# neka-nat/probreg

Measured on AMD Instinct MI355X. Metric: EM iterations/sec (RigidCPD, N=M=100k fp32), higher is better.
Workload: dtype f32; 1 GPU; C1 RigidCPD fp32 synthetic N=M=100000 D=3 w=0; window=EM iterations 0..2332 of the registration (state reset after the warm-up steps), collective=none, m=100000, n_local=100000, n_global=100000

## Files before the change

include/probreg_hip.h:

```cpp
#ifndef PROBREG_HIP_H
#define PROBREG_HIP_H

#include <stdint.h>

#ifdef __cplusplus
extern "C" {
#endif

typedef enum prg_status {
    PRG_OK = 0,
    PRG_ERR_INVALID = -1,
    PRG_ERR_HIP = -2,
    PRG_ERR_STATE = -3,
    PRG_ERR_NOMEM = -4
} prg_status;

typedef enum prg_tf_kind {
    PRG_TF_RIGID = 0,
    PRG_TF_AFFINE = 1,
    PRG_TF_NONRIGID = 2
} prg_tf_kind;

const char* prg_last_error(void);
int prg_version(void);
int prg_device_count(int* count);

#define PRG_NMOMENTS 32
#define PRG_NPARAMS 32

typedef struct prg_cpd prg_cpd;

int prg_cpd_create(prg_cpd** out, int device, void* hip_stream);
int prg_cpd_destroy(prg_cpd* h);

int prg_spatial_order(const float* points_hd, int64_t n, int dim, int on_device, int* perm_host);
int prg_cpd_set_options(prg_cpd* h, int sort_source, int sort_target, int cull);

int prg_cpd_set_dense_engine(prg_cpd* h, int mode, double bound);
int prg_cpd_last_estep_engine(prg_cpd* h, int* engine);
int prg_cpd_engine_bounds(int64_t m, int64_t n_local, double* col_bound, double* row_bound);
int prg_cpd_set_sparse_engine(prg_cpd* h, int mode);
int prg_cpd_last_estep_engines(prg_cpd* h, int* col_engine, int* row_engine);
int prg_cpd_last_estep_lean(prg_cpd* h, int* lean);
int prg_cpd_set_lean_factor(prg_cpd* h, double factor);
int prg_cpd_set_stream_mode(prg_cpd* h, int on);

int prg_cpd_set_source(prg_cpd* h, const float* source_hd, int64_t m, int dim);

int prg_cpd_set_target(prg_cpd* h, const float* target_hd, int64_t n_local, int dim, int64_t n_global);

int prg_cpd_bind_moments(prg_cpd* h, double* moments_dev);
int prg_cpd_moments_ptr(prg_cpd* h, double** moments_dev);
int prg_cpd_params_ptr(prg_cpd* h, double** params_dev);

#define PRG_COMM_ID_BYTES 128
typedef struct prg_comm prg_comm;
int prg_comm_available(int* rccl_version);
int prg_comm_unique_id(unsigned char* id_out);
int prg_comm_create(prg_comm** out, const unsigned char* id, int rank, int nranks, int device);
int prg_comm_adopt(prg_comm** out, void* nccl_comm, int device);
int prg_comm_info(prg_comm* c, int* rank, int* nranks, int64_t* all_reduces_issued);
int prg_comm_destroy(prg_comm* c);
int prg_comm_all_reduce_f64(prg_comm* c, double* buf_dev, int64_t count, void* hip_stream);
int prg_cpd_set_comm(prg_cpd* h, prg_comm* comm);
int prg_cpd_iterate(prg_cpd* h, int kind, int update_scale, double w, int n_iter);
int prg_cpd_set_moments_only(prg_cpd* h, int mode);
int prg_cpd_last_estep_fused(prg_cpd* h, int* fused);
int prg_cpd_set_fused_factor(prg_cpd* h, double factor);
int prg_cpd_set_resid_sweep(prg_cpd* h, int on);

int prg_cpd_init_sums(prg_cpd* h);
int prg_cpd_init_params(prg_cpd* h, const double* init_params_host);

int prg_cpd_estep(prg_cpd* h, double w);

int prg_cpd_estep_timed(prg_cpd* h, double w, float* ms_out);

int prg_cpd_pair_counts(prg_cpd* h, double* col_pairs, double* row_pairs);

int prg_cpd_mstep(prg_cpd* h, int kind, int update_scale);

int prg_cpd_get_params(prg_cpd* h, double* params_host);
int prg_cpd_set_params(prg_cpd* h, const double* params_host);
int prg_cpd_get_moments(prg_cpd* h, double* moments_host);

int prg_cpd_get_estep(prg_cpd* h, double* pt1_hd, double* p1_hd, double* px_hd);
int prg_cpd_get_tsource(prg_cpd* h, float* tsource_hd);

int prg_cpd_moments_from_estep(prg_cpd* h, const double* pt1_hd, const double* p1_hd, const double* px_hd);

int prg_cpd_set_tuning(prg_cpd* h, int r_col, int seg_col, int r_row, int seg_row);

int prg_cpd_nonrigid_build_g(prg_cpd* h, double beta);
int prg_cpd_nonrigid_set_solver(prg_cpd* h, int mode, int max_rank, double tol);
int prg_cpd_nonrigid_rank(prg_cpd* h, int* rank);
int prg_cpd_nonrigid_get_g(prg_cpd* h, float* g_hd);
int prg_cpd_nonrigid_set_w(prg_cpd* h, const double* w_hd);
int prg_cpd_nonrigid_get_w(prg_cpd* h, double* w_hd);
int prg_cpd_nonrigid_apply(prg_cpd* h, double* t_hd);
int prg_cpd_nonrigid_set_priors(prg_cpd* h, const double* p1_tilde_hd, const double* px_tilde_hd, double alpha);
int prg_cpd_rowacc_ptr(prg_cpd* h, double** rowacc_dev, int64_t* count);
int prg_cpd_mstep_nonrigid(prg_cpd* h, double lmd);

int prg_cpd_set_source_weights(prg_cpd* h, const double* log_weights_hd, double uniform_ratio);
int prg_cpd_bcpd_build_g(prg_cpd* h, double c);
int prg_cpd_bcpd_solve(prg_cpd* h, double lmd, double cfac, const double* nu_hd, const double* resid_hd,
                       double* vhat_hd, double* sigma_diag_hd);

int prg_gauss_transform_direct(int device, void* hip_stream, const double* source_hd, int64_t s,
                               const double* target_hd, int64_t t, int dim, const double* weights_hd,
                               int n_weight_rows, double h, double* out_hd);
int prg_gauss_transform_direct_f64(int device, void* hip_stream, const double* source_hd, int64_t s,
                               const double* target_hd, int64_t t, int dim, const double* weights_hd,
                               int n_weight_rows, double h, double* out_hd);

int prg_squared_kernel_sum(int device, void* hip_stream, const float* x_hd, int64_t m,
                           const float* y_hd, int64_t n, int dim, double* out_host);
int prg_rbf_kernel(int device, void* hip_stream, const float* x_hd, int64_t m, const float* y_hd,
                   int64_t n, int dim, double beta, float* out_hd);
int prg_inverse_multiquadric_kernel(int device, void* hip_stream, const float* x_hd, int64_t m, const float* y_hd,
                                    int64_t n, int dim, double c, float* out_hd);
int prg_nn_mean_distance(int device, void* hip_stream, const float* a_hd, int64_t m, const float* b_hd, int64_t n,
                         int dim, double* out_host);

typedef struct prg_ph prg_ph;
int prg_lattice_set_splat_mode(int mode);
int prg_ph_create(prg_ph** out, int device, void* hip_stream);
int prg_ph_destroy(prg_ph* h);
int prg_ph_init(prg_ph* h, const float* points_hd, int64_t n, int dim, int with_blur);
int prg_ph_lattice_size(prg_ph* h, int* size);
int prg_ph_filter(prg_ph* h, const float* values_hd, int channels, float* out_hd);

typedef struct prg_filterreg prg_filterreg;
int prg_fr_create(prg_filterreg** out, int device, void* hip_stream);
int prg_fr_destroy(prg_filterreg* h);
int prg_fr_set_source(prg_filterreg* h, const double* source_hd, int64_t m, int dim);
int prg_fr_set_target(prg_filterreg* h, const double* target_hd, int64_t n, int dim);
int prg_fr_set_state(prg_filterreg* h, const double* rot9, const double* t3, double sigma2);
int prg_fr_estep(prg_filterreg* h, double alpha, int* lattice_size, int* with_blur);
int prg_fr_get_estep(prg_filterreg* h, float* m0_hd, float* m1_hd, float* m2_hd);
int prg_fr_mstep(prg_filterreg* h, double w, int update_sigma2, double min_sigma2, double* out_host);
int prg_fr_get_state(prg_filterreg* h, double* out_host);

int prg_fr_set_target_normals(prg_filterreg* h, const double* normals_hd);
int prg_fr_get_nx(prg_filterreg* h, float* nx_hd);
int prg_fr_mstep_pt2pl(prg_filterreg* h, double w, int update_sigma2, double min_sigma2, double* out_host);

int prg_fr_mstep_from_arrays(int device, void* hip_stream, const double* t_source_hd, int64_t m, int dim,
                             int64_t n_target, const float* m0_hd, const float* m1_hd, const float* m2_hd,
                             const float* nx_hd, const double* rot9, const double* t3, double sigma2, double w,
                             double* out_host);

int prg_kabsch_weighted(int device, void* hip_stream, const float* model_hd, const float* target_hd,
                        const float* weight_hd, int64_t n, int dim, double* rot_host, double* t_host);

typedef struct prg_gmmtree prg_gmmtree;
int prg_gmm_create(prg_gmmtree** out, int device, void* hip_stream);
int prg_gmm_destroy(prg_gmmtree* h);
int prg_gmm_build(prg_gmmtree* h, const double* points_hd, int64_t n, int tree_level, const int64_t* init_idx_host,
                  double lambda_s, double lambda_d, int max_iter, int* iters_host, double* q_host, double* dq_host);
int prg_gmm_set_nodes(prg_gmmtree* h, const double* nodes_host, int tree_level);
int prg_gmm_get_nodes(prg_gmmtree* h, double* nodes_host);
int prg_gmm_set_target(prg_gmmtree* h, const double* target_hd, int64_t n);
int prg_gmm_reg_estep(prg_gmmtree* h, const double* rot9, const double* t3, double scale, double lambda_c,
                      double* m01_host, double* m2_host);

typedef struct prg_gmmfit prg_gmmfit;
int prg_gmmfit_create(prg_gmmfit** out, int device, void* hip_stream);
int prg_gmmfit_destroy(prg_gmmfit* h);
int prg_gmmfit_set_data(prg_gmmfit* h, const double* data_hd, int64_t n, int dim);
int prg_gmmfit_seed(prg_gmmfit* h, int k, const double* uniforms_host, int n_trials);
int prg_gmmfit_get_seeds(prg_gmmfit* h, int* index_host);
int prg_gmmfit_lloyd(prg_gmmfit* h, int max_iter, double tol, int* n_iter_host);
int prg_gmmfit_init_from_labels(prg_gmmfit* h, double reg_covar);
int prg_gmmfit_set_params(prg_gmmfit* h, int k, const double* weights_host, const double* means_host,
                          const double* precisions_host);
int prg_gmmfit_em(prg_gmmfit* h, double tol, int max_iter, double reg_covar, int* n_iter_host, int* converged_host,
                  double* lower_bounds_host);
int prg_gmmfit_get_params(prg_gmmfit* h, double* weights_host, double* means_host, double* covariances_host);

#ifdef __cplusplus
}
#endif
#endif
```

probreg_amd/_lib.py:

```python
import ctypes
import os

_HERE = os.path.dirname(os.path.abspath(__file__))
LIB_PATH = os.environ.get("PROBREG_HIP_LIB") or os.path.join(_HERE, "csrc", "libprobreg_hip.so")

PRG_OK = 0
PRG_ERR_INVALID = -1
PRG_ERR_HIP = -2
PRG_ERR_STATE = -3
PRG_ERR_NOMEM = -4

PRG_TF_RIGID = 0
PRG_TF_AFFINE = 1
PRG_TF_NONRIGID = 2

PRG_NMOMENTS = 32
PRG_NPARAMS = 32
PRG_COMM_ID_BYTES = 128


class ProbregHipError(RuntimeError):
    """A libprobreg_hip call failed (HIP runtime error or call-order violation)."""


def _load():
    try:
        import torch
    except Exception:
        pass
    if not os.path.isfile(LIB_PATH):
        raise ImportError(
            "probreg_amd: %s not found. Build it with `python __graft_entry__.py build` "
            "(or `make -C probreg_amd/csrc`); there is no CPU fallback." % LIB_PATH
        )
    try:
        return ctypes.CDLL(LIB_PATH)
    except OSError as e:
        raise ImportError("probreg_amd: cannot load %s: %s" % (LIB_PATH, e))


lib = _load()

_c = ctypes
_vp, _i, _i64, _d = _c.c_void_p, _c.c_int, _c.c_int64, _c.c_double
_pp = _c.POINTER(_c.c_void_p)

SIGNATURES = {
    "prg_version": [],
    "prg_device_count": [_c.POINTER(_i)],
    "prg_cpd_create": [_pp, _i, _vp],
    "prg_cpd_destroy": [_vp],
    "prg_spatial_order": [_vp, _i64, _i, _i, _vp],
    "prg_cpd_set_options": [_vp, _i, _i, _i],
    "prg_cpd_set_dense_engine": [_vp, _i, _d],
    "prg_cpd_last_estep_engine": [_vp, _c.POINTER(_i)],
    "prg_cpd_set_sparse_engine": [_vp, _i],
    "prg_cpd_engine_bounds": [_i64, _i64, _c.POINTER(_d), _c.POINTER(_d)],
    "prg_cpd_last_estep_lean": [_vp, _c.POINTER(_i)],
    "prg_cpd_set_lean_factor": [_vp, _d],
    "prg_cpd_set_stream_mode": [_vp, _i],
    "prg_cpd_last_estep_engines": [_vp, _c.POINTER(_i), _c.POINTER(_i)],
    "prg_cpd_set_source": [_vp, _vp, _i64, _i],
    "prg_cpd_set_target": [_vp, _vp, _i64, _i, _i64],
    "prg_cpd_bind_moments": [_vp, _vp],
    "prg_cpd_moments_ptr": [_vp, _pp],
    "prg_cpd_params_ptr": [_vp, _pp],
    "prg_comm_available": [_c.POINTER(_i)],
    "prg_comm_unique_id": [_vp],
    "prg_comm_create": [_pp, _vp, _i, _i, _i],
    "prg_comm_adopt": [_pp, _vp, _i],
    "prg_comm_info": [_vp, _c.POINTER(_i), _c.POINTER(_i), _c.POINTER(_i64)],
    "prg_comm_destroy": [_vp],
    "prg_comm_all_reduce_f64": [_vp, _vp, _i64, _vp],
    "prg_cpd_set_comm": [_vp, _vp],
    "prg_cpd_iterate": [_vp, _i, _i, _d, _i],
    "prg_cpd_set_moments_only": [_vp, _i],
    "prg_cpd_last_estep_fused": [_vp, _c.POINTER(_i)],
    "prg_cpd_set_fused_factor": [_vp, _d],
    "prg_cpd_set_resid_sweep": [_vp, _i],
    "prg_cpd_init_sums": [_vp],
    "prg_cpd_init_params": [_vp, _vp],
    "prg_cpd_estep": [_vp, _d],
    "prg_cpd_estep_timed": [_vp, _d, _vp],
    "prg_cpd_pair_counts": [_vp, _c.POINTER(_d), _c.POINTER(_d)],
    "prg_cpd_mstep": [_vp, _i, _i],
    "prg_cpd_get_params": [_vp, _vp],
    "prg_cpd_set_params": [_vp, _vp],
    "prg_cpd_get_moments": [_vp, _vp],
    "prg_cpd_get_estep": [_vp, _vp, _vp, _vp],
    "prg_cpd_get_tsource": [_vp, _vp],
    "prg_cpd_moments_from_estep": [_vp, _vp, _vp, _vp],
    "prg_cpd_set_tuning": [_vp, _i, _i, _i, _i],
    "prg_cpd_nonrigid_build_g": [_vp, _d],
    "prg_cpd_nonrigid_set_solver": [_vp, _i, _i, _d],
    "prg_cpd_nonrigid_rank": [_vp, _c.POINTER(_i)],
    "prg_cpd_nonrigid_get_g": [_vp, _vp],
    "prg_cpd_nonrigid_set_w": [_vp, _vp],
    "prg_cpd_nonrigid_get_w": [_vp, _vp],
    "prg_cpd_nonrigid_apply": [_vp, _vp],
    "prg_cpd_nonrigid_set_priors": [_vp, _vp, _vp, _d],
    "prg_cpd_rowacc_ptr": [_vp, _pp, _c.POINTER(_i64)],
    "prg_cpd_mstep_nonrigid": [_vp, _d],
    "prg_cpd_set_source_weights": [_vp, _vp, _d],
    "prg_cpd_bcpd_build_g": [_vp, _d],
    "prg_cpd_bcpd_solve": [_vp, _d, _d, _vp, _vp, _vp, _vp],
    "prg_gauss_transform_direct": [_i, _vp, _vp, _i64, _vp, _i64, _i, _vp, _i, _d, _vp],
    "prg_gauss_transform_direct_f64": [_i, _vp, _vp, _i64, _vp, _i64, _i, _vp, _i, _d, _vp],
    "prg_squared_kernel_sum": [_i, _vp, _vp, _i64, _vp, _i64, _i, _c.POINTER(_d)],
    "prg_rbf_kernel": [_i, _vp, _vp, _i64, _vp, _i64, _i, _d, _vp],
    "prg_inverse_multiquadric_kernel": [_i, _vp, _vp, _i64, _vp, _i64, _i, _d, _vp],
    "prg_nn_mean_distance": [_i, _vp, _vp, _i64, _vp, _i64, _i, _c.POINTER(_d)],
    "prg_lattice_set_splat_mode": [_i],
    "prg_ph_create": [_pp, _i, _vp],
    "prg_ph_destroy": [_vp],
    "prg_ph_init": [_vp, _vp, _i64, _i, _i],
    "prg_ph_lattice_size": [_vp, _c.POINTER(_i)],
    "prg_ph_filter": [_vp, _vp, _i, _vp],
    "prg_fr_create": [_pp, _i, _vp],
    "prg_fr_destroy": [_vp],
    "prg_fr_set_source": [_vp, _vp, _i64, _i],
    "prg_fr_set_target": [_vp, _vp, _i64, _i],
    "prg_fr_set_state": [_vp, _vp, _vp, _d],
    "prg_fr_estep": [_vp, _d, _c.POINTER(_i), _c.POINTER(_i)],
    "prg_fr_get_estep": [_vp, _vp, _vp, _vp],
    "prg_fr_mstep": [_vp, _d, _i, _d, _vp],
    "prg_fr_get_state": [_vp, _vp],
    "prg_fr_set_target_normals": [_vp, _vp],
    "prg_fr_get_nx": [_vp, _vp],
    "prg_fr_mstep_pt2pl": [_vp, _d, _i, _d, _vp],
    "prg_fr_mstep_from_arrays": [_i, _vp, _vp, _i64, _i, _i64, _vp, _vp, _vp, _vp, _vp, _vp, _d, _d, _vp],
    "prg_kabsch_weighted": [_i, _vp, _vp, _vp, _vp, _i64, _i, _vp, _vp],
    "prg_gmm_create": [_pp, _i, _vp],
    "prg_gmm_destroy": [_vp],
    "prg_gmm_build": [_vp, _vp, _i64, _i, _vp, _d, _d, _i, _vp, _vp, _vp],
    "prg_gmm_set_nodes": [_vp, _vp, _i],
    "prg_gmm_get_nodes": [_vp, _vp],
    "prg_gmm_set_target": [_vp, _vp, _i64],
    "prg_gmm_reg_estep": [_vp, _vp, _vp, _d, _d, _vp, _vp],
    "prg_gmmfit_create": [_pp, _i, _vp],
    "prg_gmmfit_destroy": [_vp],
    "prg_gmmfit_set_data": [_vp, _vp, _i64, _i],
    "prg_gmmfit_seed": [_vp, _i, _vp, _i],
    "prg_gmmfit_get_seeds": [_vp, _vp],
    "prg_gmmfit_lloyd": [_vp, _i, _d, _c.POINTER(_i)],
    "prg_gmmfit_init_from_labels": [_vp, _d],
    "prg_gmmfit_set_params": [_vp, _i, _vp, _vp, _vp],
    "prg_gmmfit_em": [_vp, _d, _i, _d, _c.POINTER(_i), _c.POINTER(_i), _vp],
    "prg_gmmfit_get_params": [_vp, _vp, _vp, _vp],
}

for _name, _args in SIGNATURES.items():
    _fn = getattr(lib, _name)
    _fn.argtypes = _args
    _fn.restype = _i
lib.prg_last_error.argtypes = []
lib.prg_last_error.restype = _c.c_char_p


def last_error():
    msg = lib.prg_last_error()
    return msg.decode("utf-8", "replace") if msg else ""


def check(status):
    if status == PRG_OK:
        return
    msg = last_error()
    if status == PRG_ERR_INVALID:
        raise ValueError(msg)
    if status == PRG_ERR_NOMEM:
        raise MemoryError(msg)
    raise ProbregHipError("libprobreg_hip status %d: %s" % (status, msg))


def device_count():
    n = _i(0)
    st = lib.prg_device_count(_c.byref(n))
    if st != PRG_OK:
        return 0
    return int(n.value)


def require_gpu():
    n = device_count()
    if n <= 0:
        raise ProbregHipError(
            "probreg_amd needs an AMD GPU (gfx950): hipGetDeviceCount reported none (%s). "
            "There is no CPU fallback." % last_error()
        )
    return n


def ptr(a):
    if a is None:
        return None
    if hasattr(a, "data_ptr"):
        return _vp(a.data_ptr())
    return _vp(a.ctypes.data)
```

probreg_amd/csrc/cpd.hip:

```cpp
#include <math.h>

#include <algorithm>
#include <cmath>
#include <cstdlib>
#include <cstring>
#include <vector>

#include "cpd_estep.h"
#include "cpd_sweeps.h"
#include "morton.h"
#include "small_linalg.h"

namespace {
using prg::block_reduce_store;
using prg::ensure_mompart;
using prg::grid1;
using prg::kBlock;
using prg::kMomComp;
using prg::row_moment_terms;

constexpr double kEps32 = 1.1920928955078125e-07;

__global__ __launch_bounds__(kBlock) void k_pack_cloud(const float* __restrict__ in, int64_t n, int dim,
                                                       float4* __restrict__ out, int64_t cap, float pad,
// ... 98 lines not shown
                                                                const double* __restrict__ px, int dim, int64_t m,
                                                                int64_t n, const float4* __restrict__ src4,
                                                                const float4* __restrict__ tgt4,
                                                                const int* __restrict__ perm_src,
                                                                const int* __restrict__ perm_tgt,
                                                                double* __restrict__ mompart) {
    const int64_t i = (int64_t)blockIdx.x * kBlock + threadIdx.x;
    double a[kMomComp];
#pragma unroll
    for (int c = 0; c < kMomComp; ++c) a[c] = 0.0;
    if (i < m) {
        const float4 yf = src4[i];
        const double y[3] = {yf.x, yf.y, yf.z};
        const int64_t j = perm_src ? perm_src[i] : i;
        double pxi[3] = {px[j * dim], px[j * dim + 1], dim > 2 ? px[j * dim + 2] : 0.0};
        row_moment_terms(a, p1[j], pxi, y);
    }
    if (i < n) {
        const float4 xf = tgt4[i];
        const int64_t j = perm_tgt ? perm_tgt[i] : i;
        a[22] = pt1[j] * ((double)xf.x * xf.x + (double)xf.y * xf.y + (double)xf.z * xf.z);
    }
    block_reduce_store(a, mompart);
}

__global__ __launch_bounds__(kBlock) void k_rowacc_from_arrays(const double* __restrict__ pt1,
                                                               const double* __restrict__ p1,
                                                               const double* __restrict__ px, int dim, int64_t m,
                                                               int64_t n, int64_t mcap,
                                                               const int* __restrict__ perm_src,
                                                               const int* __restrict__ perm_tgt,
                                                               double* __restrict__ rowacc, float* __restrict__ pt1f) {
    const int64_t i = (int64_t)blockIdx.x * kBlock + threadIdx.x;
    if (i < n) pt1f[i] = (float)pt1[perm_tgt ? perm_tgt[i] : i];
    if (i >= m) return;
    const int64_t j = perm_src ? perm_src[i] : i;
    rowacc[i] = p1[j];
    rowacc[mcap + i] = px[j * dim];
    rowacc[2 * mcap + i] = px[j * dim + 1];
    rowacc[3 * mcap + i] = dim > 2 ? px[j * dim + 2] : 0.0;
}

__global__ void k_mstep(const double* __restrict__ mom, double* __restrict__ params, int kind, int update_scale,
                        int dim) {
    if (threadIdx.x != 0 || blockIdx.x != 0) return;
    const int d = dim;
    const double S0 = mom[0];
    double mu_x[3], mu_y[3], A[3][3], YPY[3][3];
#pragma unroll
    for (int i = 0; i < 3; ++i) {
        mu_x[i] = mom[1 + i] / S0;
        mu_y[i] = mom[4 + i] / S0;
    }
#pragma unroll
    for (int i = 0; i < 3; ++i)
#pragma unroll
        for (int j = 0; j < 3; ++j) A[i][j] = mom[7 + 3 * i + j] - mom[1 + i] * mu_y[j];
    const double syy[3][3] = {{mom[16], mom[17], mom[18]}, {mom[17], mom[19], mom[20]}, {mom[18], mom[20], mom[21]}};
    double tr_yp1y = 0.0, mux2 = 0.0;
#pragma unroll
    for (int i = 0; i < 3; ++i) {
#pragma unroll
        for (int j = 0; j < 3; ++j) YPY[i][j] = syy[i][j] - S0 * mu_y[i] * mu_y[j];
        tr_yp1y += YPY[i][i];
        mux2 += mu_x[i] * mu_x[i];
    }
    const double tr_xp1x = mom[22] - S0 * mux2;
    double L[3][3], t[3];
    double scale = 1.0, sigma2, q;
    if (kind == PRG_TF_RIGID) {
        double U[3][3], V[3][3], sv[3];
        prg::jacobi_svd(A, d, U, V, sv);
        const double dd = prg::det3(U, d) * prg::det3(V, d);
        double c[3];
#pragma unroll
        for (int k = 0; k < 3; ++k) {
            bool is_min = k < d;
#pragma unroll
            for (int j = 0; j < 3; ++j)
                if (j < d && j != k && (sv[j] < sv[k] || (sv[j] == sv[k] && j < k))) is_min = false;
            c[k] = is_min ? dd : 1.0;
        }
        double tr_atr = 0.0;
#pragma unroll
        for (int i = 0; i < 3; ++i)
#pragma unroll
            for (int j = 0; j < 3; ++j) {
                double r = 0;
#pragma unroll
                for (int k = 0; k < 3; ++k) r += c[k] * U[i][k] * V[j][k];
                L[i][j] = r;
                tr_atr += (i < d && j < d) ? A[i][j] * r : 0.0;
            }
        scale = update_scale ? tr_atr / tr_yp1y : 1.0;
#pragma unroll
        for (int i = 0; i < 3; ++i) {
            double r = 0;
#pragma unroll
            for (int j = 0; j < 3; ++j) r += L[i][j] * mu_y[j];
            t[i] = (i < d) ? mu_x[i] - scale * r : 0.0;
        }
        if (update_scale)
            sigma2 = (tr_xp1x - scale * tr_atr) / (S0 * d);
        else
            sigma2 = (tr_xp1x + tr_yp1y - scale * tr_atr) / (S0 * d);
        sigma2 = fmax(sigma2, kEps32);
        q = (tr_xp1x - 2.0 * scale * tr_atr + scale * scale * tr_yp1y) / (2.0 * sigma2);
        q += d * S0 * 0.5 * log(sigma2);
    } else {
        double Mx[3][6];
#pragma unroll
        for (int i = 0; i < 3; ++i)
#pragma unroll
            for (int j = 0; j < 3; ++j) {
                const bool in = i < d && j < d;
                Mx[i][j] = in ? YPY[j][i] : ((i == j) ? 1.0 : 0.0);
                Mx[i][3 + j] = in ? A[j][i] : 0.0;
            }
        double ypy_scale = 0.0;
#pragma unroll
        for (int i = 0; i < 3; ++i)
#pragma unroll
            for (int j = 0; j < 3; ++j) ypy_scale = fmax(ypy_scale, (i < d && j < d) ? fabs(YPY[i][j]) : 0.0);
#pragma unroll
        for (int c = 0; c < 3; ++c) {
#pragma unroll
            for (int r = c + 1; r < 3; ++r) {
                if (fabs(Mx[r][c]) > fabs(Mx[c][c])) {
#pragma unroll
                    for (int j = 0; j < 6; ++j) { const double tmp = Mx[c][j]; Mx[c][j] = Mx[r][j]; Mx[r][j] = tmp; }
                }
            }
            if (c < d && !(fabs(Mx[c][c]) > 1e-12 * ypy_scale)) Mx[c][c] = 0.0;
#pragma unroll
            for (int r = c + 1; r < 3; ++r) {
                const double f = Mx[r][c] / Mx[c][c];
#pragma unroll
                for (int j = 0; j < 6; ++j) Mx[r][j] -= (j >= c) ? f * Mx[c][j] : 0.0;
            }
        }
        double Xs[3][3];
#pragma unroll
        for (int col = 0; col < 3; ++col)
#pragma unroll
            for (int r = 2; r >= 0; --r) {
                double v = Mx[r][3 + col];
#pragma unroll
                for (int j = 0; j < 3; ++j) v -= (j > r) ? Mx[r][j] * Xs[j][col] : 0.0;
                Xs[r][col] = v / Mx[r][r];
            }
        double tr_ab = 0.0;
#pragma unroll
        for (int i = 0; i < 3; ++i) {
            double r = 0;
#pragma unroll
            for (int j = 0; j < 3; ++j) {
                const bool in = i < d && j < d;
                L[i][j] = in ? Xs[j][i] : ((i == j) ? 1.0 : 0.0);
                r += in ? L[i][j] * mu_y[j] : 0.0;
                tr_ab += in ? A[i][j] * L[i][j] : 0.0;
            }
            t[i] = (i < d) ? mu_x[i] - r : 0.0;
        }
        sigma2 = (tr_xp1x - tr_ab) / (S0 * d);
        sigma2 = fmax(sigma2, kEps32);
        q = (tr_xp1x - 2.0 * tr_ab + tr_ab) / (2.0 * sigma2) + d * S0 * 0.5 * log(sigma2);
    }
    for (int i = 0; i < 3; ++i) {
        for (int j = 0; j < 3; ++j) params[3 * i + j] = L[i][j];
        params[9 + i] = t[i];
    }
    params[12] = scale;
    params[13] = sigma2;
    params[14] = q;
    params[15] = S0;
    params[16] += 1.0;
}

__global__ __launch_bounds__(kBlock) void k_float_to_double(const float* __restrict__ in, double* __restrict__ out,
                                                            int64_t n, const int* __restrict__ perm) {
    int64_t i = (int64_t)blockIdx.x * kBlock + threadIdx.x;
    if (i < n) out[perm ? perm[i] : i] = in[i];
}
__global__ __launch_bounds__(kBlock) void k_scatter_double(const double* __restrict__ in, double* __restrict__ out,
                                                           int64_t n, const int* __restrict__ perm) {
    int64_t i = (int64_t)blockIdx.x * kBlock + threadIdx.x;
    if (i < n) out[perm ? perm[i] : i] = in[i];
}
__global__ __launch_bounds__(kBlock) void k_gather_weights(const double* __restrict__ lw, int64_t m,
                                                           const int* __restrict__ perm, float* __restrict__ out) {
    int64_t i = (int64_t)blockIdx.x * kBlock + threadIdx.x;
    if (i < m) out[i] = (float)lw[perm ? perm[i] : i];
}
__global__ __launch_bounds__(kBlock) void k_pack_px(const double* __restrict__ rowacc, int64_t mcap, int64_t m,
                                                    int dim, double* __restrict__ out, const int* __restrict__ perm) {
    int64_t i = (int64_t)blockIdx.x * kBlock + threadIdx.x;
    if (i >= m) return;
    const int64_t j = perm ? perm[i] : i;
    for (int k = 0; k < dim; ++k) out[j * dim + k] = rowacc[(int64_t)(1 + k) * mcap + i];
}
__global__ __launch_bounds__(kBlock) void k_unpack_points(const float4* __restrict__ in, int64_t m, int dim,
                                                          float* __restrict__ out, const int* __restrict__ perm) {
    int64_t i = (int64_t)blockIdx.x * kBlock + threadIdx.x;
    if (i >= m) return;
    const float4 v = in[i];
    const int64_t j = perm ? perm[i] : i;
    out[j * dim] = v.x;
    out[j * dim + 1] = v.y;
    if (dim > 2) out[j * dim + 2] = v.z;
}

static void free_queue(SweepQueue& q) {
    for (void* p : {(void*)q.masks, (void*)q.chunk, (void*)q.units, (void*)q.ctrl, (void*)q.ucount})
        if (p) (void)hipFree(p);
    q = SweepQueue();
}

int free_plan_buffers(prg_cpd* h) {
    free_queue(h->qcol);
    free_queue(h->qrow);
    void** const owned[] = {(void**)&h->src4, (void**)&h->z4, (void**)&h->tgt4, (void**)&h->pt1, (void**)&h->colpart, (void**)&h->rowpart,
                            (void**)&h->rowacc, (void**)&h->mompart, &h->stage, (void**)&h->perm_src, (void**)&h->perm_tgt, (void**)&h->zmeta,
                            (void**)&h->tmeta, (void**)&h->colmin, (void**)&h->motion, (void**)&h->srcw, (void**)&h->wgcount, (void**)&h->rorig,
                            (void**)&h->corig, (void**)&h->zchunk, (void**)&h->tchunk};
    for (void** p : owned) {
        if (*p) (void)hipFree(*p);
        *p = nullptr;
    }
    h->wg_cap = 0;
    h->stage_bytes = 0;
    return PRG_OK;
}

int cap_for(int64_t n) { return (int)prg::round_up(n + 64 * prg::kSuper + 1024, 1024); }

int morton_permutation(prg_cpd* h, const float* pts_hd, int64_t n, int dim, int** perm_dev, double* ext2 = nullptr,
                       float* box = nullptr) {
    std::vector<float> host((size_t)n * dim);
    PRG_HIP(hipMemcpy(host.data(), pts_hd, host.size() * sizeof(float), hipMemcpyDefault));
    if (ext2) {
        *ext2 = 0.0;
        for (int k = 0; k < 3; ++k) {
            float lo = INFINITY, hi = -INFINITY;
            for (int64_t i = 0; i < n && k < dim; ++i) {
                lo = std::min(lo, host[(size_t)i * dim + k]);
                hi = std::max(hi, host[(size_t)i * dim + k]);
            }
            if (k >= dim) lo = hi = 0.f;
            *ext2 += (double)(hi - lo) * (double)(hi - lo);
            if (box) {
                box[k] = lo;
                box[3 + k] = hi;
            }
        }
    }
    if (*perm_dev) (void)hipFree(*perm_dev);
    *perm_dev = nullptr;
    PRG_HIP(hipMalloc((void**)perm_dev, (size_t)n * sizeof(int)));
    const std::string& order = prg::cpd_env().spatial_order;
    if (order != "morton" && order != "kd_host") {
        PRG_TRY(prg::ensure_stage(h, (size_t)n * dim * sizeof(float)));
        PRG_HIP(hipMemcpyAsync(h->stage, host.data(), host.size() * sizeof(float), hipMemcpyHostToDevice, h->stream));
        return prg::device_kd_order((const float*)h->stage, n, dim, *perm_dev, h->stream);
    }
    const std::vector<int> perm = order == "morton" ? prg::morton_order(host.data(), n, dim) : prg::kd_order(host.data(), n, dim);
    PRG_HIP(hipMemcpy(*perm_dev, perm.data(), (size_t)n * sizeof(int), hipMemcpyHostToDevice));
    return PRG_OK;
}

template <typename T>
int ensure_exact(T** p, size_t count) {
    if (*p) (void)hipFree(*p);
    *p = nullptr;
    PRG_HIP(hipMalloc((void**)p, count * sizeof(T)));
    return PRG_OK;
}

}

namespace prg {
int ensure_stage(prg_cpd* h, size_t bytes) {
    if (h->stage && h->stage_bytes >= bytes) return PRG_OK;
    if (h->stage) {
        PRG_HIP(hipStreamSynchronize(h->stream));
        (void)hipFree(h->stage);
    }
    h->stage = nullptr;
    h->stage_bytes = 0;
    PRG_HIP(hipMalloc(&h->stage, bytes));
    h->stage_bytes = bytes;
    return PRG_OK;
}

const CpdEnv& cpd_env() {
    static const CpdEnv env = [] {
        CpdEnv e;
        auto num = [](const char* name, double absent) { const char* v = getenv(name); return v ? atof(v) : absent; };
        auto is_zero = [](const char* name) { const char* v = getenv(name); return v && atoi(v) == 0; };
        e.mfma_seg = getenv("PRG_MFMA_SEG") ? atoi(getenv("PRG_MFMA_SEG")) : 0;
        e.fine_grid_off = is_zero("PRG_MFMA_FINE_GRID");
        e.r_col = num("PRG_ENGINE_RCOL", 0.0);
        e.r_row = num("PRG_ENGINE_RROW", 0.0);
        e.fused_rcol_scale = num("PRG_FUSED_RCOL_SCALE", -1.0);
        e.lean_factor = num("PRG_LEAN_FACTOR", -1.0);
        e.fused_factor = num("PRG_FUSED_FACTOR", -1.0);
        e.owner_off = is_zero("PRG_OWNER_SWEEP");
        e.debug_engine = getenv("PRG_DEBUG_ENGINE") != nullptr;
        if (const char* v = getenv("PRG_SPATIAL_ORDER")) e.spatial_order = v;
        return e;
    }();
    return env;
}

int ensure_engine_state(prg_cpd* h) {
    if (h->eng_host) return PRG_OK;
    PRG_HIP(hipHostMalloc((void**)&h->eng_host, sizeof(EngineDecision), hipHostMallocMapped | hipHostMallocCoherent));
    memset(h->eng_host, 0, sizeof(EngineDecision));
    PRG_HIP(hipHostGetDevicePointer((void**)&h->eng_host_dev, h->eng_host, 0));
    const size_t bytes = sizeof(EngineDecision) + 2 * sizeof(unsigned long long) + 4 * sizeof(double);
    PRG_HIP(hipMalloc((void**)&h->eng_dev, bytes));
    PRG_HIP(hipMemsetAsync(h->eng_dev, 0, bytes, h->stream));
    h->eng_work = reinterpret_cast<unsigned long long*>(h->eng_dev + 1);
    h->tsum_local = reinterpret_cast<double*>(h->eng_work + 2);
    return PRG_OK;
}
}

extern "C" {

int prg_cpd_create(prg_cpd** out, int device, void* hip_stream) {
    PRG_REQUIRE(out != nullptr, PRG_ERR_INVALID, "prg_cpd_create: out is NULL");
    int count = 0;
    PRG_HIP(hipGetDeviceCount(&count));
    PRG_REQUIRE(device >= 0 && device < count, PRG_ERR_INVALID, "prg_cpd_create: device %d out of range (%d devices)",
                device, count);
    prg::DeviceGuard g(device);
    PRG_REQUIRE(g.ok, PRG_ERR_HIP, "prg_cpd_create: hipSetDevice(%d) failed", device);
    prg_cpd* h = new (std::nothrow) prg_cpd();
    PRG_REQUIRE(h != nullptr, PRG_ERR_NOMEM, "prg_cpd_create: out of host memory");
    h->device = device;
    h->stream = (hipStream_t)hip_stream;
    if (const char* eng = getenv("PRG_DENSE_ENGINE")) h->dense_engine = std::max(0, std::min(2, atoi(eng)));
    if (const char* eng = getenv("PRG_SPARSE_ENGINE")) h->sparse_engine = std::max(0, std::min(2, atoi(eng)));
    if (const char* eng = getenv("PRG_RESID_SWEEP")) h->resid_sweep = atoi(eng) != 0;
    hipError_t e = hipMalloc((void**)&h->state, (PRG_NMOMENTS + PRG_NPARAMS) * sizeof(double));
    if (e != hipSuccess) {
        delete h;
        prg::set_error("prg_cpd_create: hipMalloc failed: %s", hipGetErrorString(e));
        return PRG_ERR_HIP;
    }
    h->moments = h->state;
    h->params = h->state + PRG_NMOMENTS;
    k_zero_doubles<<<1, 64, 0, h->stream>>>(h->state, PRG_NMOMENTS + PRG_NPARAMS);
    *out = h;
    return PRG_OK;
}

int prg_cpd_destroy(prg_cpd* h) {
    if (!h) return PRG_OK;
    prg::DeviceGuard g(h->device);
    (void)hipStreamSynchronize(h->stream);
    free_plan_buffers(h);
    prg::nonrigid_free(h);
    if (h->state) (void)hipFree(h->state);
    if (h->pinned) (void)hipHostFree(h->pinned);
    if (h->eng_host) (void)hipHostFree(h->eng_host);
    if (h->eng_dev) (void)hipFree(h->eng_dev);
    delete h;
    return PRG_OK;
}

int prg_cpd_set_source(prg_cpd* h, const float* source_hd, int64_t m, int dim) {
    PRG_REQUIRE(h && source_hd, PRG_ERR_INVALID, "prg_cpd_set_source: NULL argument");
    PRG_REQUIRE(m > 0 && (dim == 2 || dim == 3), PRG_ERR_INVALID,
                "prg_cpd_set_source: need m > 0 and dim in {2,3} (got m=%lld dim=%d)", (long long)m, dim);
    PRG_REQUIRE(!h->have_target || h->D == dim, PRG_ERR_INVALID,
                "prg_cpd_set_source: dim %d does not match target dim %d", dim, h->D);
    prg::DeviceGuard g(h->device);
    PRG_HIP(hipStreamSynchronize(h->stream));
    const int64_t cap = cap_for(m);
    if (cap != h->Mcap) {
        if (h->src4) (void)hipFree(h->src4);
        if (h->z4) (void)hipFree(h->z4);
        if (h->rowacc) (void)hipFree(h->rowacc);
        h->src4 = h->z4 = nullptr;
        h->rowacc = nullptr;
        PRG_HIP(hipMalloc((void**)&h->src4, cap * sizeof(float4)));
        PRG_HIP(hipMalloc((void**)&h->z4, cap * sizeof(float4)));
        PRG_HIP(hipMalloc((void**)&h->rowacc, 4 * cap * sizeof(double)));
    }
    if (cap != h->Mcap || !h->zmeta) {
        PRG_TRY(ensure_exact(&h->zmeta, (size_t)(cap / prg::kGroup) * 8));
        if (!h->motion) {
            PRG_TRY(ensure_exact(&h->motion, 16));
            PRG_HIP(hipMemsetAsync(h->motion, 0, 16 * sizeof(unsigned), h->stream));
        }
        PRG_TRY(ensure_exact(&h->rorig, (size_t)(cap / prg::kMfmaWgPoints) + 4));
        PRG_TRY(ensure_exact(&h->zchunk, (size_t)(cap / prg::kSuper) * 8));
    }
    h->M = m;
    h->D = dim;
    h->Mcap = cap;
    if (h->opt_sort_src) {
        PRG_TRY(morton_permutation(h, source_hd, m, dim, &h->perm_src, &h->sext2));
    } else if (h->perm_src) {
        (void)hipFree(h->perm_src);
        h->perm_src = nullptr;
    }
    PRG_TRY(prg::ensure_stage(h, (size_t)m * dim * sizeof(float)));
    PRG_HIP(hipMemcpyAsync(h->stage, source_hd, (size_t)m * dim * sizeof(float), hipMemcpyDefault, h->stream));
    k_pack_cloud<<<grid1(cap), kBlock, 0, h->stream>>>((const float*)h->stage, m, dim, h->src4, cap, prg::kSrcPad,
                                                       0.f, h->perm_src);
    k_pack_cloud<<<grid1(cap), kBlock, 0, h->stream>>>((const float*)h->stage, m, dim, h->z4, cap, prg::kSrcPad, 0.f,
                                                       h->perm_src);
    k_group_meta<<<grid1(cap / prg::kGroup), kBlock, 0, h->stream>>>(h->z4, cap / prg::kGroup, h->zmeta);
    PRG_HIP(hipGetLastError());
    PRG_HIP(hipStreamSynchronize(h->stream));
    h->have_colmin = false;
    h->have_source = true;
    h->have_estep = false;
    prg::nonrigid_free(h);
    if (h->srcw) (void)hipFree(h->srcw);
    h->srcw = nullptr;
    h->uniform_ratio = 0.0;
    return PRG_OK;
}

int prg_cpd_set_source_weights(prg_cpd* h, const double* log_weights_hd, double uniform_ratio) {
    PRG_REQUIRE(h && h->have_source, PRG_ERR_STATE, "prg_cpd_set_source_weights: source not set");
    PRG_REQUIRE(uniform_ratio >= 0.0, PRG_ERR_INVALID, "prg_cpd_set_source_weights: uniform_ratio must be >= 0");
    prg::DeviceGuard g(h->device);
    h->uniform_ratio = uniform_ratio;
    if (!log_weights_hd) {
        PRG_HIP(hipStreamSynchronize(h->stream));
        if (h->srcw) (void)hipFree(h->srcw);
        h->srcw = nullptr;
        return PRG_OK;
    }
    hipPointerAttribute_t attr;
    const bool on_host = hipPointerGetAttributes(&attr, log_weights_hd) != hipSuccess || attr.type != hipMemoryTypeDevice;
    (void)hipGetLastError();
    if (on_host)
        for (int64_t i = 0; i < h->M; ++i)
            PRG_REQUIRE(log_weights_hd[i] <= 0.0, PRG_ERR_INVALID,
                        "prg_cpd_set_source_weights: log-weight %lld is %g, must be <= 0 (and not NaN)", (long long)i,
                        log_weights_hd[i]);
    if (!h->srcw) PRG_HIP(hipMalloc((void**)&h->srcw, (size_t)h->Mcap * sizeof(float)));
    PRG_TRY(prg::ensure_stage(h, (size_t)h->M * sizeof(double)));
    PRG_HIP(hipMemcpyAsync(h->stage, log_weights_hd, (size_t)h->M * sizeof(double), hipMemcpyDefault, h->stream));
    k_gather_weights<<<grid1(h->M), kBlock, 0, h->stream>>>((const double*)h->stage, h->M, h->perm_src, h->srcw);
    PRG_HIP(hipGetLastError());
    PRG_HIP(hipStreamSynchronize(h->stream));
    h->have_colmin = false;
    return PRG_OK;
}

int prg_cpd_set_target(prg_cpd* h, const float* target_hd, int64_t n_local, int dim, int64_t n_global) {
    PRG_REQUIRE(h && target_hd, PRG_ERR_INVALID, "prg_cpd_set_target: NULL argument");
    PRG_REQUIRE(n_local > 0 && n_global >= n_local && (dim == 2 || dim == 3), PRG_ERR_INVALID,
                "prg_cpd_set_target: need 0 < n_local <= n_global and dim in {2,3}");
    PRG_REQUIRE(!h->have_source || h->D == dim, PRG_ERR_INVALID,
                "prg_cpd_set_target: dim %d does not match source dim %d", dim, h->D);
    prg::DeviceGuard g(h->device);
    PRG_HIP(hipStreamSynchronize(h->stream));
    if (h->tsum_local) PRG_HIP(hipMemsetAsync(h->tsum_local, 0, 4 * sizeof(double), h->stream));
    const int64_t cap = cap_for(n_local);
    if (cap != h->Ncap) {
        if (h->tgt4) (void)hipFree(h->tgt4);
        if (h->pt1) (void)hipFree(h->pt1);
        h->tgt4 = nullptr;
        h->pt1 = nullptr;
        PRG_HIP(hipMalloc((void**)&h->tgt4, cap * sizeof(float4)));
        PRG_HIP(hipMalloc((void**)&h->pt1, cap * sizeof(float)));
    }
    if (cap != h->Ncap || !h->tmeta) {
        PRG_TRY(ensure_exact(&h->tmeta, (size_t)(cap / prg::kGroup) * 8));
        PRG_TRY(ensure_exact(&h->tchunk, (size_t)(cap / prg::kSuper) * 8));
        PRG_TRY(ensure_exact(&h->corig, (size_t)(cap / prg::kMfmaWgPoints) + 4));
        PRG_TRY(ensure_exact(&h->colmin, (size_t)cap + (size_t)cap / prg::kGroup));
        PRG_HIP(hipMemsetAsync(h->colmin, 0, ((size_t)cap + (size_t)cap / prg::kGroup) * sizeof(float), h->stream));
    }
    if (!h->motion) {
        PRG_TRY(ensure_exact(&h->motion, 16));
        PRG_HIP(hipMemsetAsync(h->motion, 0, 16 * sizeof(unsigned), h->stream));
    }
    h->N = n_local;
    h->Nglobal = n_global;
    h->D = dim;
    h->Ncap = cap;
    if (h->opt_sort_tgt) {
        PRG_TRY(morton_permutation(h, target_hd, n_local, dim, &h->perm_tgt, &h->text2, h->tbox));
    } else if (h->perm_tgt) {
        (void)hipFree(h->perm_tgt);
        h->perm_tgt = nullptr;
    }
    PRG_TRY(prg::ensure_stage(h, (size_t)n_local * dim * sizeof(float)));
    PRG_HIP(hipMemcpyAsync(h->stage, target_hd, (size_t)n_local * dim * sizeof(float), hipMemcpyDefault, h->stream));
    k_pack_cloud<<<grid1(cap), kBlock, 0, h->stream>>>((const float*)h->stage, n_local, dim, h->tgt4, cap,
                                                       prg::kTgtPad, 0.f, h->perm_tgt);
    k_group_meta<<<grid1(cap / prg::kGroup), kBlock, 0, h->stream>>>(h->tgt4, cap / prg::kGroup, h->tmeta);
    PRG_HIP(hipGetLastError());
    PRG_HIP(hipStreamSynchronize(h->stream));
    h->have_colmin = false;
    h->have_target = true;
    h->have_estep = false;
    return PRG_OK;
}

int prg_cpd_bind_moments(prg_cpd* h, double* moments_dev) {
    PRG_REQUIRE(h, PRG_ERR_INVALID, "prg_cpd_bind_moments: NULL handle");
    h->moments = moments_dev ? moments_dev : h->state;
    return PRG_OK;
}

int prg_cpd_moments_ptr(prg_cpd* h, double** moments_dev) {
    PRG_REQUIRE(h && moments_dev, PRG_ERR_INVALID, "prg_cpd_moments_ptr: NULL argument");
    *moments_dev = h->moments;
    return PRG_OK;
}

int prg_cpd_params_ptr(prg_cpd* h, double** params_dev) {
    PRG_REQUIRE(h && params_dev, PRG_ERR_INVALID, "prg_cpd_params_ptr: NULL argument");
    *params_dev = h->params;
    return PRG_OK;
}

int prg_cpd_set_tuning(prg_cpd* h, int r_col, int seg_col, int r_row, int seg_row) {
    PRG_REQUIRE(h, PRG_ERR_INVALID, "prg_cpd_set_tuning: NULL handle");
    auto ok_r = [](int r) { return r == 0 || r == 2 || r == 4 || r == -2 || r == -4; };
    PRG_REQUIRE(ok_r(r_col) && ok_r(r_row), PRG_ERR_INVALID,
                "prg_cpd_set_tuning: points per lane must be 0 (auto), 2, 4 (packed) or -2, -4 (scalar form)");
    PRG_REQUIRE(seg_col >= 0 && seg_col <= 1024 && seg_row >= 0 && seg_row <= 256, PRG_ERR_INVALID,
                "prg_cpd_set_tuning: segment counts must be in [0, 1024] (column pass) / [0, 256] (row pass)");
    h->r_col = r_col;
    h->seg_col = seg_col;
    h->r_row = r_row;
    h->seg_row = seg_row;
    return PRG_OK;
}

int prg_cpd_set_dense_engine(prg_cpd* h, int mode, double bound) {
    PRG_REQUIRE(h, PRG_ERR_INVALID, "prg_cpd_set_dense_engine: NULL handle");
    PRG_REQUIRE(mode >= 0 && mode <= 2, PRG_ERR_INVALID, "prg_cpd_set_dense_engine: mode must be 0, 1 or 2");
    PRG_REQUIRE(bound >= 0.0, PRG_ERR_INVALID, "prg_cpd_set_dense_engine: bound must be >= 0 (0 keeps the default)");
    h->dense_engine = mode;
    if (bound > 0.0) h->dense_bound = bound;
    EngineSwitch fresh;
    fresh.pred_fused = h->eng.pred_fused;
    fresh.grid_fine = h->eng.grid_fine;
    h->eng = fresh;
    return PRG_OK;
}

int prg_cpd_last_estep_engine(prg_cpd* h, int* engine) {
    PRG_REQUIRE(h && engine, PRG_ERR_INVALID, "prg_cpd_last_estep_engine: NULL argument");
    *engine = h->last_estep_mfma ? 1 : 0;
    return PRG_OK;
}

int prg_cpd_set_sparse_engine(prg_cpd* h, int mode) {
    PRG_REQUIRE(h, PRG_ERR_INVALID, "prg_cpd_set_sparse_engine: NULL handle");
    PRG_REQUIRE(mode >= 0 && mode <= 3, PRG_ERR_INVALID, "prg_cpd_set_sparse_engine: mode must be 0 (grid of culled waves), 1 (default: owner sweep for single-sweep "
                "iterations, work queue for the two-sweep E-steps of large clouds), 2 (work queue always) or 3 (round 5's default: queue for large clouds, no owner sweep)");
    h->sparse_engine = mode;
    return PRG_OK;
}

int prg_cpd_last_estep_engines(prg_cpd* h, int* col_engine, int* row_engine) {
    PRG_REQUIRE(h && col_engine && row_engine, PRG_ERR_INVALID, "prg_cpd_last_estep_engines: NULL argument");
    *col_engine = h->last_estep_mfma ? 1 : 0;
    *row_engine = h->last_estep_row_mfma ? 1 : 0;
    return PRG_OK;
}

int prg_cpd_last_estep_lean(prg_cpd* h, int* lean) {
    PRG_REQUIRE(h && lean, PRG_ERR_INVALID, "prg_cpd_last_estep_lean: NULL argument");
    *lean = h->last_estep_row_lean ? 1 : 0;
    return PRG_OK;
}

int prg_cpd_set_moments_only(prg_cpd* h, int mode) {
    PRG_REQUIRE(h, PRG_ERR_INVALID, "prg_cpd_set_moments_only: NULL handle");
    PRG_REQUIRE(mode >= 0 && mode <= 2, PRG_ERR_INVALID, "prg_cpd_set_moments_only: mode must be 0, 1 or 2");
    h->moments_only = mode == 1;
    h->fused_in_iterate = mode != 2;
    return PRG_OK;
}

int prg_cpd_set_resid_sweep(prg_cpd* h, int on) {
    PRG_REQUIRE(h, PRG_ERR_INVALID, "prg_cpd_set_resid_sweep: NULL handle");
    h->resid_sweep = on != 0;
    return PRG_OK;
}

int prg_cpd_set_fused_factor(prg_cpd* h, double factor) {
    PRG_REQUIRE(h && factor >= 0.0, PRG_ERR_INVALID, "prg_cpd_set_fused_factor: need a handle and a factor >= 0");
    h->fused_factor = factor;
    return PRG_OK;
}

int prg_cpd_last_estep_fused(prg_cpd* h, int* fused) {
    PRG_REQUIRE(h && fused, PRG_ERR_INVALID, "prg_cpd_last_estep_fused: NULL argument");
    *fused = h->last_estep_fused ? 1 : 0;
    return PRG_OK;
}

int prg_cpd_set_stream_mode(prg_cpd* h, int on) {
    PRG_REQUIRE(h, PRG_ERR_INVALID, "prg_cpd_set_stream_mode: NULL handle");
    h->mfma_stream = on != 0;
    return PRG_OK;
}

int prg_cpd_set_lean_factor(prg_cpd* h, double factor) {
    PRG_REQUIRE(h, PRG_ERR_INVALID, "prg_cpd_set_lean_factor: NULL handle");
    h->lean_factor = factor;
    return PRG_OK;
}

int prg_cpd_set_options(prg_cpd* h, int sort_source, int sort_target, int cull) {
    PRG_REQUIRE(h, PRG_ERR_INVALID, "prg_cpd_set_options: NULL handle");
    PRG_REQUIRE(!h->have_source && !h->have_target, PRG_ERR_STATE,
                "prg_cpd_set_options: must be called before the clouds are uploaded");
    h->opt_sort_src = sort_source != 0;
    h->opt_sort_tgt = sort_target != 0;
    h->opt_cull = cull != 0;
    return PRG_OK;
}

int prg_cpd_init_sums(prg_cpd* h) {
    PRG_REQUIRE(h && h->have_target, PRG_ERR_STATE, "prg_cpd_init_sums: target not set");
    prg::DeviceGuard g(h->device);
    PRG_TRY(ensure_mompart(h));
    const int nblk = (int)prg::ceil_div(h->N, kBlock);
    k_zero_doubles<<<1, 64, 0, h->stream>>>(h->moments, PRG_NMOMENTS);
    k_cloud_sums<<<nblk, kBlock, 0, h->stream>>>(h->tgt4, h->N, h->mompart);
    prg::reduce_partials(h, h->mompart, nblk, 4, h->moments, 24);
    PRG_HIP(hipGetLastError());
    PRG_TRY(prg::ensure_engine_state(h));
    PRG_HIP(hipMemcpyAsync(h->tsum_local, h->moments + 24, 4 * sizeof(double), hipMemcpyDeviceToDevice, h->stream));
    if (h->comm) PRG_TRY(prg::comm_all_reduce_f64(h->comm, h->moments, PRG_NMOMENTS, h->stream));
    return PRG_OK;
}

int prg_cpd_set_comm(prg_cpd* h, prg_comm* comm) {
    PRG_REQUIRE(h, PRG_ERR_INVALID, "prg_cpd_set_comm: NULL handle");
    PRG_REQUIRE(!comm || comm->device == h->device, PRG_ERR_INVALID, "prg_cpd_set_comm: the communicator lives on device %d, the plan on %d",
                comm ? comm->device : -1, h->device);
    h->comm = comm;
    return PRG_OK;
}

static bool is_rotation(const double* lin) {
    for (int i = 0; i < 3; ++i)
        for (int j = 0; j < 3; ++j) {
            double d = 0.0;
            for (int k = 0; k < 3; ++k) d += lin[3 * k + i] * lin[3 * k + j];
            if (!(fabs(d - (i == j ? 1.0 : 0.0)) <= 1.0e-12)) return false;
        }
    return true;
}

int prg_cpd_init_params(prg_cpd* h, const double* init_params_host) {
    PRG_REQUIRE(h && h->have_source && h->have_target, PRG_ERR_STATE, "prg_cpd_init_params: clouds not set");
    prg::DeviceGuard g(h->device);
    PRG_TRY(ensure_mompart(h));
    const int nblk = (int)prg::ceil_div(h->M, kBlock);
    double* srcsum = h->mompart + (h->mompart_elems - 64);
    double* init_dev = nullptr;
    if (init_params_host) {
        init_dev = srcsum + 8;
        PRG_HIP(hipMemcpyAsync(init_dev, init_params_host, 16 * sizeof(double), hipMemcpyHostToDevice, h->stream));
    }
    k_cloud_sums<<<nblk, kBlock, 0, h->stream>>>(h->src4, h->M, h->mompart);
    prg::reduce_partials(h, h->mompart, nblk, 4, srcsum, 0);
    k_init_params<<<1, 64, 0, h->stream>>>(h->moments, srcsum, h->params, (double)h->M, (double)h->Nglobal, h->D,
                                           init_dev);
    PRG_HIP(hipGetLastError());
    if (init_params_host) PRG_HIP(hipStreamSynchronize(h->stream));
    h->have_colmin = false;
    h->eng = EngineSwitch();
    h->init_rot_orthonormal = !init_params_host || is_rotation(init_params_host);
    return PRG_OK;
}


int prg_cpd_engine_bounds(int64_t m, int64_t n_local, double* col_bound, double* row_bound) {
    PRG_REQUIRE(m > 0 && n_local > 0 && col_bound && row_bound, PRG_ERR_INVALID, "prg_cpd_engine_bounds: need m, n_local > 0 and two outputs");
    *col_bound = prg::engine_col_bound(m, n_local);
    *row_bound = prg::engine_row_bound(m, n_local);
    return PRG_OK;
}

int prg_cpd_estep(prg_cpd* h, double w) { return prg::estep_impl(h, w, nullptr); }

int prg_cpd_estep_timed(prg_cpd* h, double w, float* ms_out) {
    PRG_REQUIRE(h && ms_out, PRG_ERR_INVALID, "prg_cpd_estep_timed: NULL argument");
    prg::DeviceGuard g(h->device);
    hipEvent_t ev[6];
    for (int i = 0; i < 6; ++i) PRG_HIP(hipEventCreate(&ev[i]));
    int st = prg::estep_impl(h, w, ev);
    if (st == PRG_OK) {
        hipError_t e = hipEventSynchronize(ev[5]);
        if (e != hipSuccess) {
            prg::set_error("prg_cpd_estep_timed: hipEventSynchronize failed: %s", hipGetErrorString(e));
            st = PRG_ERR_HIP;
        }
    }
    if (st == PRG_OK) {
        for (int i = 0; i < 5; ++i) (void)hipEventElapsedTime(&ms_out[i], ev[i], ev[i + 1]);
        (void)hipEventElapsedTime(&ms_out[5], ev[0], ev[5]);
    }
    for (int i = 0; i < 6; ++i) (void)hipEventDestroy(ev[i]);
    return st;
}

int prg_cpd_pair_counts(prg_cpd* h, double* col_pairs, double* row_pairs) {
    PRG_REQUIRE(h && h->have_estep && col_pairs && row_pairs, PRG_ERR_STATE, "prg_cpd_pair_counts: no E-step has been run");
    prg::DeviceGuard g(h->device);
    *col_pairs = h->dense_pairs_col;
    *row_pairs = h->dense_pairs_row;
    for (int pass = 0; pass < 2; ++pass) {
        const SweepQueue& q = pass ? h->qrow : h->qcol;
        if ((pass ? h->wg_row : h->wg_col) != -1) continue;
        int nu[2] = {0, 0};
        PRG_HIP(hipMemcpyAsync(nu, q.ctrl + 8, 2 * sizeof(int), hipMemcpyDeviceToHost, h->stream));
        PRG_HIP(hipStreamSynchronize(h->stream));
        double sum = 0.0;
        for (int part = 0; part < 2; ++part) {
            if (nu[part] <= 0) continue;
            std::vector<unsigned> host((size_t)nu[part]);
            PRG_HIP(hipMemcpyAsync(host.data(), q.ucount + (part ? q.cap_soft : 0), (size_t)nu[part] * sizeof(unsigned),
                                   hipMemcpyDeviceToHost, h->stream));
            PRG_HIP(hipStreamSynchronize(h->stream));
            for (int i = 0; i < nu[part]; ++i) sum += host[(size_t)i];
        }
        *(pass ? row_pairs : col_pairs) = sum * 128.0 * prg::kGroup;
    }
    if (h->wg_col > 0 || h->wg_row > 0) {
        std::vector<unsigned> host((size_t)h->wg_cap * 2);
        PRG_HIP(hipMemcpyAsync(host.data(), h->wgcount, host.size() * sizeof(unsigned), hipMemcpyDeviceToHost, h->stream));
        PRG_HIP(hipStreamSynchronize(h->stream));
        if (h->wg_col > 0) {
            double s = 0.0;
            for (int64_t i = 0; i < h->wg_col; ++i) s += host[(size_t)i];
            *col_pairs = s * h->wg_col_pairs;
        }
        if (h->wg_row > 0) {
            double s = 0.0;
            for (int64_t i = 0; i < h->wg_row; ++i) s += host[(size_t)(h->wg_cap + i)];
            *row_pairs = s * h->wg_row_pairs;
        }
    }
    const double all_pairs = (double)h->M * (double)h->N;
    *col_pairs = std::min(*col_pairs, all_pairs);
    *row_pairs = std::min(*row_pairs, all_pairs);
    return PRG_OK;
}

int prg_cpd_mstep(prg_cpd* h, int kind, int update_scale) {
    PRG_REQUIRE(h && h->have_source, PRG_ERR_STATE, "prg_cpd_mstep: source not set");
    PRG_REQUIRE(kind == PRG_TF_RIGID || kind == PRG_TF_AFFINE, PRG_ERR_INVALID,
                "prg_cpd_mstep: kind must be PRG_TF_RIGID or PRG_TF_AFFINE (use prg_cpd_mstep_nonrigid)");
    PRG_REQUIRE(kind == PRG_TF_RIGID || !(h->have_estep && h->last_estep_fused), PRG_ERR_STATE,
                "prg_cpd_mstep: the last E-step ran as the single sweep of a rigid iteration (prg_cpd_set_moments_only(1)): its "
                "moments do not hold Y^T diag(p1) Y, which the affine M-step needs");
    prg::DeviceGuard g(h->device);
    k_mstep<<<1, 64, 0, h->stream>>>(h->moments, h->params, kind, update_scale, h->D);
    PRG_HIP(hipGetLastError());
    h->init_rot_orthonormal = kind == PRG_TF_RIGID;
    return PRG_OK;
}

int prg_cpd_iterate(prg_cpd* h, int kind, int update_scale, double w, int n_iter) {
    PRG_REQUIRE(h && h->have_source && h->have_target, PRG_ERR_STATE, "prg_cpd_iterate: clouds not set");
    PRG_REQUIRE(kind == PRG_TF_RIGID || kind == PRG_TF_AFFINE, PRG_ERR_INVALID,
                "prg_cpd_iterate: kind must be PRG_TF_RIGID or PRG_TF_AFFINE");
    PRG_REQUIRE(n_iter >= 0, PRG_ERR_INVALID, "prg_cpd_iterate: n_iter must be >= 0");
    prg::DeviceGuard g(h->device);
    const bool keep = h->moments_only;
    if (kind == PRG_TF_RIGID && h->fused_in_iterate) h->moments_only = true;
    if (kind != PRG_TF_RIGID) h->moments_only = false;
    int st = PRG_OK;
    for (int it = 0; it < n_iter && st == PRG_OK; ++it) {
        st = prg::estep_impl(h, w, nullptr);
        if (st == PRG_OK) {
            k_mstep<<<1, 64, 0, h->stream>>>(h->moments, h->params, kind, update_scale, h->D);
            h->init_rot_orthonormal = kind == PRG_TF_RIGID;
        }
    }
    h->moments_only = keep;
    PRG_TRY(st);
    PRG_HIP(hipGetLastError());
    return PRG_OK;
}

int prg_cpd_get_params(prg_cpd* h, double* params_host) {
    PRG_REQUIRE(h && params_host, PRG_ERR_INVALID, "prg_cpd_get_params: NULL argument");
    prg::DeviceGuard g(h->device);
    if (!h->pinned) PRG_HIP(hipHostMalloc((void**)&h->pinned, 64 * sizeof(double), hipHostMallocDefault));
    PRG_HIP(hipMemcpyAsync(h->pinned, h->params, PRG_NPARAMS * sizeof(double), hipMemcpyDeviceToHost, h->stream));
    int* host_info = reinterpret_cast<int*>(h->pinned + 48);
    *host_info = 0;
    if (h->nr_info) PRG_HIP(hipMemcpyAsync(host_info, h->nr_info, sizeof(int), hipMemcpyDeviceToHost, h->stream));
    PRG_HIP(hipStreamSynchronize(h->stream));
    for (int i = 0; i < PRG_NPARAMS; ++i) params_host[i] = h->pinned[i];
    if (*host_info != 0) {
        const int pivot = *host_info - 1;
        PRG_HIP(hipMemsetAsync(h->nr_info, 0, sizeof(int), h->stream));
        prg::set_error("prg_cpd_mstep_nonrigid: the reduced system is not positive definite at pivot %d (sigma2 or lmd <= 0?)", pivot);
        return PRG_ERR_STATE;
    }
    return PRG_OK;
}

int prg_cpd_set_params(prg_cpd* h, const double* params_host) {
    PRG_REQUIRE(h && params_host, PRG_ERR_INVALID, "prg_cpd_set_params: NULL argument");
    prg::DeviceGuard g(h->device);
    PRG_HIP(hipMemcpyAsync(h->params, params_host, PRG_NPARAMS * sizeof(double), hipMemcpyHostToDevice, h->stream));
    PRG_HIP(hipStreamSynchronize(h->stream));
    h->init_rot_orthonormal = is_rotation(params_host);
    return PRG_OK;
}

int prg_cpd_get_moments(prg_cpd* h, double* moments_host) {
    PRG_REQUIRE(h && moments_host, PRG_ERR_INVALID, "prg_cpd_get_moments: NULL argument");
    prg::DeviceGuard g(h->device);
    PRG_HIP(hipMemcpyAsync(moments_host, h->moments, PRG_NMOMENTS * sizeof(double), hipMemcpyDeviceToHost,
                           h->stream));
    PRG_HIP(hipStreamSynchronize(h->stream));
    return PRG_OK;
}

int prg_cpd_get_estep(prg_cpd* h, double* pt1_hd, double* p1_hd, double* px_hd) {
    PRG_REQUIRE(h && h->have_estep, PRG_ERR_STATE, "prg_cpd_get_estep: no E-step has been run");
    PRG_REQUIRE(h->rowacc_valid || (!p1_hd && !px_hd), PRG_ERR_STATE,
                "prg_cpd_get_estep: the last E-step ran as the fused single sweep of a rigid iteration (prg_cpd_iterate / "
                "prg_cpd_set_moments_only): it leaves MOMENTS and pt1, no per-point p1 / px");
    prg::DeviceGuard g(h->device);
    const size_t need = (size_t)(h->N > h->M * h->D ? h->N : h->M * h->D) * sizeof(double);
    PRG_TRY(prg::ensure_stage(h, need));
    if (pt1_hd) {
        k_float_to_double<<<grid1(h->N), kBlock, 0, h->stream>>>(h->pt1, (double*)h->stage, h->N, h->perm_tgt);
        PRG_HIP(hipMemcpyAsync(pt1_hd, h->stage, h->N * sizeof(double), hipMemcpyDefault, h->stream));
        PRG_HIP(hipStreamSynchronize(h->stream));
    }
    if (p1_hd) {
        k_scatter_double<<<grid1(h->M), kBlock, 0, h->stream>>>(h->rowacc, (double*)h->stage, h->M, h->perm_src);
        PRG_HIP(hipMemcpyAsync(p1_hd, h->stage, h->M * sizeof(double), hipMemcpyDefault, h->stream));
        PRG_HIP(hipStreamSynchronize(h->stream));
    }
    if (px_hd) {
        k_pack_px<<<grid1(h->M), kBlock, 0, h->stream>>>(h->rowacc, h->Mcap, h->M, h->D, (double*)h->stage, h->perm_src);
        PRG_HIP(hipMemcpyAsync(px_hd, h->stage, h->M * h->D * sizeof(double), hipMemcpyDefault, h->stream));
        PRG_HIP(hipStreamSynchronize(h->stream));
    }
    PRG_HIP(hipGetLastError());
    return PRG_OK;
}

int prg_cpd_get_tsource(prg_cpd* h, float* tsource_hd) {
    PRG_REQUIRE(h && h->have_source && tsource_hd, PRG_ERR_STATE, "prg_cpd_get_tsource: source not set");
    prg::DeviceGuard g(h->device);
    PRG_TRY(prg::ensure_stage(h, (size_t)h->M * h->D * sizeof(float)));
    k_unpack_points<<<grid1(h->M), kBlock, 0, h->stream>>>(h->z4, h->M, h->D, (float*)h->stage, h->perm_src);
    PRG_HIP(hipMemcpyAsync(tsource_hd, h->stage, h->M * h->D * sizeof(float), hipMemcpyDefault, h->stream));
    PRG_HIP(hipStreamSynchronize(h->stream));
    return PRG_OK;
}

int prg_cpd_moments_from_estep(prg_cpd* h, const double* pt1_hd, const double* p1_hd, const double* px_hd) {
    PRG_REQUIRE(h && h->have_source && h->have_target, PRG_ERR_STATE, "prg_cpd_moments_from_estep: clouds not set");
    PRG_REQUIRE(pt1_hd && p1_hd && px_hd, PRG_ERR_INVALID, "prg_cpd_moments_from_estep: NULL array");
    prg::DeviceGuard g(h->device);
    const size_t nb_pt1 = (size_t)h->N * sizeof(double), nb_p1 = (size_t)h->M * sizeof(double),
                 nb_px = (size_t)h->M * h->D * sizeof(double);
    PRG_TRY(prg::ensure_stage(h, nb_pt1 + nb_p1 + nb_px));
    PRG_TRY(ensure_mompart(h));
    double* d_pt1 = (double*)h->stage;
    double* d_p1 = d_pt1 + h->N;
    double* d_px = d_p1 + h->M;
    PRG_HIP(hipMemcpyAsync(d_pt1, pt1_hd, nb_pt1, hipMemcpyDefault, h->stream));
    PRG_HIP(hipMemcpyAsync(d_p1, p1_hd, nb_p1, hipMemcpyDefault, h->stream));
    PRG_HIP(hipMemcpyAsync(d_px, px_hd, nb_px, hipMemcpyDefault, h->stream));
    const int nblk = prg::mom_blocks(*h);
    k_moments_from_arrays<<<nblk, kBlock, 0, h->stream>>>(d_pt1, d_p1, d_px, h->D, h->M, h->N, h->src4, h->tgt4,
                                                          h->perm_src, h->perm_tgt, h->mompart);
    prg::reduce_partials(h, h->mompart, nblk, kMomComp, h->moments, 0);
    k_rowacc_from_arrays<<<nblk, kBlock, 0, h->stream>>>(d_pt1, d_p1, d_px, h->D, h->M, h->N, h->Mcap, h->perm_src,
                                                         h->perm_tgt, h->rowacc, h->pt1);
    PRG_HIP(hipGetLastError());
    PRG_HIP(hipStreamSynchronize(h->stream));
    h->have_estep = true;
    h->last_estep_fused = false;
    h->rowacc_valid = true;
    return PRG_OK;
}

}
```

probreg_amd/csrc/cpd_estep.h:

```cpp
#pragma once
#include <algorithm>

#include "cpd_plan.h"
#include "prg_device.h"

struct EstepLayout {
    int ra, rb, RA, RB;
    bool use_cull;
    int SA, segA, PA;
    int SB, segB, PB;
    bool mfma_possible;
    int seg_col_fine, seg_row_fine;
    int PAm, PBm;
    bool use_queue;
    bool allow_fused;
    bool allow_resid;
    bool use_owner;
    int PO;
    int64_t colpart_elems, rowpart_elems, wgcount_elems, mompart_elems;
};

namespace prg {
constexpr int kBlock = 256;
constexpr int kMomComp = 24;
inline dim3 grid1(int64_t n) { return dim3((unsigned)ceil_div(n, kBlock)); }

int estep_layout(const prg_cpd& h, EstepLayout* L);
int estep_impl(prg_cpd* h, double w, hipEvent_t* ev);
double engine_col_bound(int64_t m, int64_t n_local);
double engine_row_bound(int64_t m, int64_t n_local, bool lean = true);
int ensure_engine_state(prg_cpd* h);

inline int mom_blocks(const prg_cpd& h) { return (int)ceil_div(std::max(h.M, h.N), kBlock); }
inline int64_t mompart_elems(const prg_cpd& h) { return (int64_t)mom_blocks(h) * (kMomComp + 2) + 64; }
int ensure_mompart(prg_cpd* h);
void reduce_partials(prg_cpd* h, const double* part, int nblk, int ncomp, double* out, int off);

__device__ __forceinline__ void block_reduce_store(double (&a)[kMomComp], double* __restrict__ mompart) {
    __shared__ double sh[4][kMomComp];
    const int lane = threadIdx.x & 63, wv = threadIdx.x >> 6;
#pragma unroll
    for (int c = 0; c < kMomComp; ++c) {
        const double s = wave_sum(a[c]);
        if (lane == 0) sh[wv][c] = s;
    }
    __syncthreads();
    if (threadIdx.x < kMomComp)
        mompart[(int64_t)blockIdx.x * kMomComp + threadIdx.x] =
            sh[0][threadIdx.x] + sh[1][threadIdx.x] + sh[2][threadIdx.x] + sh[3][threadIdx.x];
}

__device__ __forceinline__ void row_moment_terms(double (&a)[kMomComp], double p1, const double (&px)[3],
                                                 const double (&y)[3]) {
    a[0] = p1;
#pragma unroll
    for (int i = 0; i < 3; ++i) {
        a[1 + i] = px[i];
        a[4 + i] = p1 * y[i];
#pragma unroll
        for (int j = 0; j < 3; ++j) a[7 + 3 * i + j] = px[i] * y[j];
    }
    a[16] = p1 * y[0] * y[0];
    a[17] = p1 * y[0] * y[1];
    a[18] = p1 * y[0] * y[2];
    a[19] = p1 * y[1] * y[1];
    a[20] = p1 * y[1] * y[2];
    a[21] = p1 * y[2] * y[2];
}
}
```

probreg_amd/csrc/cpd_estep.hip:

```cpp
#include <math.h>

#include <algorithm>
#include <cmath>

#include "cpd_estep.h"
#include "cpd_sweeps.h"

namespace {
using prg::block_reduce_store;
using prg::grid1;
using prg::kBlock;
using prg::kMomComp;
using prg::row_moment_terms;

constexpr double kLog2e = 1.4426950408889634;

constexpr int kRedBlock = 1024;
__global__ __launch_bounds__(kRedBlock) void k_reduce_partials(const double* __restrict__ part, int nblk, int ncomp,
                                                               double* __restrict__ out, int off) {
    __shared__ double sh[32][33];
    const int c = threadIdx.x & 31, slice = threadIdx.x >> 5;
    double s = 0.0;
    if (c < ncomp)
        for (int b = slice; b < nblk; b += 32) s += part[(int64_t)b * ncomp + c];
// ... 445 lines not shown
    } else {
        const double tot = den + c;
        b = (float)(-log2(tot));
        pd = den / tot;
        p = (float)pd;
        qn = pd / A;
    }
    float cmin = 0.f;
    double a[kMomComp];
#pragma unroll
    for (int k = 0; k < kMomComp; ++k) a[k] = 0.0;
    if (valid) {
        reinterpret_cast<float*>(tgt4 + i)[3] = b;
        pt1[i] = p;
        colmin[i] = gmin;
        cmin = gmin;
        const float4 xf = tgt4[i];
        const double x[3] = {xf.x, xf.y, xf.z};
        double pz[3], xu = 0.0, xx = 0.0;
#pragma unroll
        for (int k = 0; k < 3; ++k) {
            pz[k] = pd * x[k] - qn * U[k];
            xu += x[k] * U[k];
            xx += x[k] * x[k];
        }
        a[0] = pd;
#pragma unroll
        for (int r = 0; r < 3; ++r) {
            a[1 + r] = pd * x[r];
            a[4 + r] = pz[r];
#pragma unroll
            for (int k = 0; k < 3; ++k) a[7 + 3 * r + k] = x[r] * pz[k];
        }
        a[16] = pd * xx + qn * (R - 2.0 * xu);
        a[22] = pd * xx;
    } else {
        b = 0.f;
    }
    block_reduce_store(a, mompart);
    {
        const float gm = half_max(cmin);
        if ((threadIdx.x & 31) == 0) colmin_g[(int64_t)blockIdx.x * (kBlock / 32) + (threadIdx.x >> 5)] = gm;
        __shared__ float wg_max[kBlock / 32];
        if ((threadIdx.x & 31) == 0) wg_max[threadIdx.x >> 5] = gm;
        __syncthreads();
        if (threadIdx.x == 0) {
            float mx = wg_max[0];
#pragma unroll
            for (int k = 1; k < kBlock / 32; ++k) mx = fmaxf(mx, wg_max[k]);
            if (mx > 0.f) atomicMax(stat + 4 + slot, __float_as_uint(mx));
        }
    }
    if (gmeta) block_group_meta(0.f, 0.f, 0.f, b, b, false, gmeta);
}

__global__ __launch_bounds__(kRedBlock) void k_fused_final(const double* __restrict__ part, int nblk,
                                                           const double* __restrict__ params, double* __restrict__ moments) {
    __shared__ double sh[32][33];
    __shared__ double m[32];
    const int c = threadIdx.x & 31, slice = threadIdx.x >> 5;
    double sum = 0.0;
    if (c < kMomComp)
        for (int b = slice; b < nblk; b += 32) sum += part[(int64_t)b * kMomComp + c];
    sh[slice][c] = sum;
    __syncthreads();
    if (threadIdx.x < 32) {
        double t = 0.0;
#pragma unroll
        for (int k = 0; k < 32; ++k) t += sh[k][threadIdx.x];
        m[threadIdx.x] = t;
    }
    __syncthreads();
    if (threadIdx.x != 0) return;
    const double S0 = m[0], s = params[12];
    const double t[3] = {params[9], params[10], params[11]};
    double tsz = 0.0, tt = 0.0;
    moments[0] = S0;
#pragma unroll
    for (int i = 0; i < 3; ++i) {
        moments[1 + i] = m[1 + i];
        tsz += t[i] * m[4 + i];
        tt += t[i] * t[i];
    }
#pragma unroll
    for (int j = 0; j < 3; ++j) {
        double sy = 0.0;
#pragma unroll
        for (int k = 0; k < 3; ++k) sy += params[3 * k + j] * (m[4 + k] - S0 * t[k]);
        moments[4 + j] = sy / s;
    }
#pragma unroll
    for (int i = 0; i < 3; ++i)
#pragma unroll
        for (int j = 0; j < 3; ++j) {
            double v = 0.0;
#pragma unroll
            for (int k = 0; k < 3; ++k) v += (m[7 + 3 * i + k] - m[1 + i] * t[k]) * params[3 * k + j];
            moments[7 + 3 * i + j] = v / s;
        }
    moments[16] = (m[16] - 2.0 * tsz + S0 * tt) / (s * s);
#pragma unroll
    for (int k = 17; k < 22; ++k) moments[k] = 0.0;
    moments[22] = m[22];
    moments[23] = 0.0;
}

__global__ __launch_bounds__(kBlock) void k_row_moments(const float* __restrict__ rowpart, int nseg, int64_t mcap,
                                                        int64_t m, const float4* __restrict__ src4,
                                                        const float4* __restrict__ z4, double* __restrict__ rowacc,
                                                        double* __restrict__ mompart,
                                                        const unsigned char* __restrict__ rowflag,
                                                        const float4* __restrict__ rorig, const QueueView qv, int lean) {
    if (qv.chunk) queue_reset(qv);
    const bool has_e = !lean;
    double a[kMomComp];
#pragma unroll
    for (int c = 0; c < kMomComp; ++c) a[c] = 0.0;
    const int lane = threadIdx.x & 63;
    for (int64_t i = (int64_t)blockIdx.x * kBlock + threadIdx.x; i - lane < m; i += (int64_t)gridDim.x * kBlock) {
        const bool valid = i < m;
        double p1 = 0, u[3] = {0, 0, 0}, e = 0;
        if (qv.chunk) {
            const int2* __restrict__ cb = qv.chunk + (i >> 7) * qv.nchunk;
            for (int c0 = 0; c0 < qv.nchunk; c0 += 64) {
                const int2 mine = c0 + lane < qv.nchunk ? cb[c0 + lane] : make_int2(0, 0);
                const int lim = qv.nchunk - c0 < 64 ? qv.nchunk - c0 : 64;
                int c = -1, left = 0, next = 0;
                auto next_slot = [&]() -> int {
                    while (left == 0) {
                        if (++c >= lim) return -1;
                        next = __builtin_amdgcn_readlane(mine.x, c);
                        left = __builtin_amdgcn_readlane(mine.y, c);
                    }
                    --left;
                    return next++;
                };
                for (;;) {
                    int sl[4];
#pragma unroll
                    for (int q = 0; q < 4; ++q) sl[q] = next_slot();
                    if (sl[0] < 0) break;
                    float v[4][5];
#pragma unroll
                    for (int q = 0; q < 4; ++q) {
                        const float* __restrict__ o = rowpart + (int64_t)(sl[q] < 0 ? sl[0] : sl[q]) * 640 + (i & 127);
#pragma unroll
                        for (int k = 0; k < 5; ++k) v[q][k] = o[128 * k];
                    }
#pragma unroll
                    for (int q = 0; q < 4; ++q) {
                        if (sl[q] < 0) continue;
                        p1 += (double)v[q][0];
                        u[0] += (double)v[q][1];
                        u[1] += (double)v[q][2];
                        u[2] += (double)v[q][3];
                        e += (double)v[q][4];
                    }
                    if (sl[3] < 0) break;
                }
            }
        }
        uint64_t live = qv.chunk ? 0ull : (nseg >= 64 ? ~0ull : ((1ull << nseg) - 1ull));
        if (rowflag && !qv.chunk) {
            const int wb = __builtin_amdgcn_readfirstlane((int)(i >> 7));
            const uint4* __restrict__ f = reinterpret_cast<const uint4*>(rowflag + (int64_t)wb * 64);
            uint64_t bits = 0;
#pragma unroll
            for (int q = 0; q < 4; ++q) {
                const uint4 v = f[q];
                const uint32_t w4[4] = {v.x, v.y, v.z, v.w};
#pragma unroll
                for (int k = 0; k < 4; ++k)
#pragma unroll
                    for (int bb = 0; bb < 4; ++bb)
                        bits |= (uint64_t)((w4[k] >> (8 * bb)) & 1u) << (q * 16 + k * 4 + bb);
            }
            live &= bits;
        }
        while (live) {
            const int s = __builtin_ctzll(live);
            live &= live - 1;
            const int s2 = live ? __builtin_ctzll(live) : s;
            const double k2 = live ? 1.0 : 0.0;
            live &= live - 1;
            const float* __restrict__ o = rowpart + (int64_t)s * 5 * mcap + i;
            const float* __restrict__ o2 = rowpart + (int64_t)s2 * 5 * mcap + i;
            const float v0 = o[0], v1 = o[mcap], v2 = o[2 * mcap], v3 = o[3 * mcap], v4 = has_e ? o[4 * mcap] : 0.f;
            const float w0 = o2[0], w1 = o2[mcap], w2 = o2[2 * mcap], w3 = o2[3 * mcap], w4 = has_e ? o2[4 * mcap] : 0.f;
            p1 += (double)v0 + k2 * (double)w0;
            u[0] += (double)v1 + k2 * (double)w1;
            u[1] += (double)v2 + k2 * (double)w2;
            u[2] += (double)v3 + k2 * (double)w3;
            e += (double)v4 + k2 * (double)w4;
        }
        const float4 zf = rorig ? rorig[i / prg::kMfmaWgPoints] : z4[i], yf = src4[i];
        const double z[3] = {zf.x, zf.y, zf.z};
        const double y[3] = {yf.x, yf.y, yf.z};
        double px[3];
#pragma unroll
        for (int k = 0; k < 3; ++k) px[k] = u[k] + p1 * z[k];
        double t[kMomComp];
#pragma unroll
        for (int c = 0; c < kMomComp; ++c) t[c] = 0.0;
        row_moment_terms(t, p1, px, y);
        t[22] = has_e ? p1 * (z[0] * z[0] + z[1] * z[1] + z[2] * z[2]) + 2.0 * (z[0] * u[0] + z[1] * u[1] + z[2] * u[2]) + e : 0.0;
        if (valid) {
#pragma unroll
            for (int c = 0; c < kMomComp; ++c) a[c] += t[c];
            rowacc[i] = p1;
            rowacc[mcap + i] = px[0];
            rowacc[2 * mcap + i] = px[1];
            rowacc[3 * mcap + i] = px[2];
        }
    }
    block_reduce_store(a, mompart);
}

__global__ __launch_bounds__(kBlock) void k_xpx_columns(const double* __restrict__ xpart, int nblk, double* __restrict__ moments) {
    __shared__ double sh[kBlock / 64][2];
    double x = 0.0, p = 0.0;
    for (int b = threadIdx.x; b < nblk; b += kBlock) {
        x += xpart[2 * (int64_t)b];
        p += xpart[2 * (int64_t)b + 1];
    }
    const double wx = wave_sum(x), wp = wave_sum(p);
    if ((threadIdx.x & 63) == 0) {
        sh[threadIdx.x >> 6][0] = wx;
        sh[threadIdx.x >> 6][1] = wp;
    }
    __syncthreads();
    if (threadIdx.x == 0) {
        double tx = 0.0, tp = 0.0;
#pragma unroll
        for (int k = 0; k < kBlock / 64; ++k) {
            tx += sh[k][0];
            tp += sh[k][1];
        }
        moments[22] = tp > 0.0 ? tx * (moments[0] / tp) : tx;
    }
}

static QueueView queue_view(const SweepQueue& q, bool active) {
    QueueView v;
    v.chunk = active ? q.chunk : nullptr;
    v.nchunk = q.nchunk;
    v.ctrl = q.ctrl;
    v.pop_start = prg::kQueueWorkgroups * (prg::kSweepBlock / 64);
    v.cap_soft = q.cap_soft;
    return v;
}

template <typename T>
int ensure_buffer(T** p, int64_t* have, int64_t need) {
    if (*p && *have >= need) return PRG_OK;
    if (*p) (void)hipFree(*p);
    *p = nullptr;
    *have = 0;
    PRG_HIP(hipMalloc((void**)p, (size_t)need * sizeof(T)));
    *have = need;
    return PRG_OK;
}

int auto_segments(int64_t nblk_x, int64_t stream_len, int quantum, int cap) {
    int64_t target = std::max<int64_t>(prg::ceil_div(12544, std::max<int64_t>(nblk_x, 1)),
                                       std::min<int64_t>(stream_len / 2048, 64));
    target = std::min<int64_t>(std::max<int64_t>(target, 1), cap);
    const int64_t seg = prg::round_up(prg::ceil_div(stream_len, target), quantum);
    return (int)prg::ceil_div(stream_len, seg);
}

int cull_segments(int64_t lane_points, int64_t stream_len, int64_t cap) {
    int64_t s = std::min<int64_t>(prg::ceil_div(stream_len, 512), cap);
    if (s * prg::ceil_div(lane_points, 128) < 65536) s = std::min<int64_t>(prg::ceil_div(stream_len, 256), cap);
    return (int)std::max<int64_t>(s, 1);
}

int mfma_fine_segments(int64_t owned, int64_t streamed, int max_planes) {
    const CpdEnv& env = prg::cpd_env();
    if (env.mfma_seg || env.fine_grid_off) return env.mfma_seg;
    const int64_t blocks = prg::ceil_div(owned, prg::kMfmaWgPoints), chunks = prg::ceil_div(streamed, 256);
    int64_t want = prg::ceil_div(3 * 768 + 256, blocks);
    want = std::min<int64_t>(std::min<int64_t>(want, chunks / 4), max_planes);
    return want > prg::mfma_planes(owned, streamed, 0) ? (int)want : 0;
}

int64_t resid_plane_elems(const prg_cpd& h, int planes, int block_cols) {
    return (int64_t)3 * planes * h.Ncap + (prg::ceil_div(h.N, block_cols) * planes + 64) / 8 + 8;
}

double engine_leave_below(int64_t owned, int64_t streamed, double tau, double delta, double c_v) {
    const int seg = prg::cpd_env().mfma_seg;
    const int cps_i = seg ? prg::mfma_chunks_per_seg(owned, streamed, seg) : prg::mfma_chunks_per_seg_model(owned, streamed);
    const double cps = (double)cps_i;
    const double wgs = (double)prg::ceil_div(owned, prg::kMfmaWgPoints) * (double)prg::ceil_div(prg::ceil_div(streamed, 256), cps_i);
    const double late = std::max(0.0, 1.0 - 768.0 / wgs) * tau / (768.0 * 512.0 * 256.0);
    return std::max(0.0, cps * tau + delta) / (c_v - late) / (double)owned;
}

double fused_lower_bound_scale(bool allow_resid) {
    const double env = prg::cpd_env().fused_rcol_scale;
    return env > 0.0 ? env : allow_resid ? 1.0 : 0.5;
}

constexpr double kLeanFactor = 64.0;

int first_queue_unit(double bound, int64_t owned, int64_t streamed) {
    const double groups = std::min(bound, (double)streamed) * (double)owned / (128.0 * prg::kGroup);
    int q = 32;
    while (groups / q > 0.75 * prg::kQueueMaxUnits && q < 256) q *= 2;
    return q;
}

double m_over_n(const prg_cpd* h) { return h->uniform_ratio > 0.0 ? h->uniform_ratio : (double)h->M / (double)h->Nglobal; }

}

namespace prg {
double engine_col_bound(int64_t m, int64_t n_local) { return engine_leave_below(n_local, m, 12.0e-6, -15.0e-6, 0.200e-12); }
double engine_row_bound(int64_t m, int64_t n_local, bool lean) {
    return lean ? engine_leave_below(m, n_local, 14.5e-6, -20.0e-6, 0.250e-12) : engine_leave_below(m, n_local, 19.2e-6, 8.0e-6, 0.233e-12);
}

int ensure_mompart(prg_cpd* h) { return ensure_buffer(&h->mompart, &h->mompart_elems, mompart_elems(*h)); }

void reduce_partials(prg_cpd* h, const double* part, int nblk, int ncomp, double* out, int off) {
    k_reduce_partials<<<1, kRedBlock, 0, h->stream>>>(part, nblk, ncomp, out, off);
}

int estep_layout(const prg_cpd& h, EstepLayout* out) {
    const CpdEnv& env = cpd_env();
    EstepLayout L;
    L.ra = h.r_col ? h.r_col : 2;
    L.rb = h.r_row ? h.r_row : 2;
    L.RA = L.ra < 0 ? -L.ra : L.ra;
    L.RB = L.rb < 0 ? -L.rb : L.rb;
    L.use_cull = h.opt_cull && h.perm_src && h.perm_tgt && h.r_col == 0 && h.r_row == 0;
    const int quantum = L.use_cull ? kSuper : 8;
    if (L.use_cull) {
        L.SA = h.seg_col ? h.seg_col : cull_segments(h.N, h.M, 1024);
        L.SB = h.seg_row ? h.seg_row : cull_segments(h.M, h.N, 256);
    } else {
        L.SA = h.seg_col ? h.seg_col : auto_segments(ceil_div(h.N, kBlock * L.RA), h.M, quantum, 256);
        L.SB = h.seg_row ? h.seg_row : auto_segments(ceil_div(h.M, kBlock * L.RB), h.N, quantum, 64);
    }
    auto seg_of = [quantum](int64_t len, int s) { return (int)round_up(ceil_div(len, s), quantum); };
    L.segA = seg_of(h.M, L.SA);
    L.segB = seg_of(h.N, L.SB);
    L.SA = (int)ceil_div(h.M, L.segA);
    L.SB = (int)ceil_div(h.N, L.segB);
    while (L.SA > 1 && (int64_t)L.SA * L.segA + kOverRead > h.Mcap) --L.SA, L.segA = seg_of(h.M, L.SA);
    while (L.SB > 1 && (int64_t)L.SB * L.segB + kOverRead > h.Ncap) --L.SB, L.segB = seg_of(h.N, L.SB);
    PRG_REQUIRE((int64_t)L.SA * L.segA + kOverRead <= h.Mcap && (int64_t)L.SB * L.segB + kOverRead <= h.Ncap,
                PRG_ERR_STATE, "prg_cpd_estep: internal segmenting failure");
    L.PA = L.use_cull ? (int)ceil_div(L.SA, 4) : L.SA;
    L.PB = L.use_cull ? (int)ceil_div(L.SB, 4) : L.SB;
    PRG_REQUIRE(!L.use_cull || L.PB <= 64, PRG_ERR_INVALID, "prg_cpd_estep: at most 256 row-pass segments with culling");

    L.mfma_possible = L.use_cull && h.dense_engine > 0 && !h.srcw && (h.dense_engine >= 2 || (h.M >= 8192 && h.N >= 8192));
    L.seg_col_fine = L.mfma_possible ? mfma_fine_segments(h.N, h.M, 256) : 0;
    L.seg_row_fine = L.mfma_possible ? mfma_fine_segments(h.M, h.N, 64) : 0;
    const int col_grid_planes = L.mfma_possible ? std::max(mfma_planes(h.N, h.M, env.mfma_seg), mfma_planes(h.N, h.M, L.seg_col_fine)) : 0;
    const int row_grid_planes = L.mfma_possible ? std::max(mfma_planes(h.M, h.N, env.mfma_seg), mfma_planes(h.M, h.N, L.seg_row_fine)) : 0;
    L.PAm = L.mfma_possible ? std::max(col_grid_planes, mfma_stream_planes(h.N, h.M)) : 0;
    L.PBm = L.mfma_possible ? std::max(row_grid_planes, mfma_stream_planes(h.M, h.N)) : 0;
    L.use_queue = L.use_cull && (h.sparse_engine == 2 || ((h.sparse_engine == 1 || h.sparse_engine == 3) && h.M >= 32768 && h.N >= 32768));
    const bool single_ok = h.moments_only && !h.nonrigid && !h.bcpd && h.init_rot_orthonormal;
    L.allow_fused = L.mfma_possible && single_ok;
    L.allow_resid = L.use_cull && h.resid_sweep && single_ok && !h.srcw;
    L.use_owner = L.allow_resid && h.sparse_engine == 1 && !env.owner_off;
    L.PO = L.use_owner ? owner_planes(h.N, h.M) : 0;

    const int64_t col_grid = (int64_t)L.PA * h.Ncap;
    const int64_t col_mfma = (int64_t)L.PAm * h.Ncap;
    const int64_t col_queue = L.use_queue ? queue_max_units(h.N, h.M) * 128 : 0;
    const int64_t col_fused = L.allow_fused ? (int64_t)3 * col_grid_planes * h.Ncap : 0;
    const int64_t col_resid = !L.allow_resid ? 0 : L.use_owner ? resid_plane_elems(h, L.PO, 64)
                              : L.use_queue ? 3 * col_queue : resid_plane_elems(h, L.PA, 128);
    L.colpart_elems = std::max({col_grid, col_mfma, col_queue, col_fused, col_resid});
    const int64_t row_planes = (int64_t)std::max(L.PB, L.PBm) * 5 * h.Mcap + (h.Mcap >> 7) * 16;
    const int64_t row_queue = L.use_queue ? queue_max_units(h.M, h.N) * 640 : 0;
    L.rowpart_elems = std::max(row_planes, row_queue);
    L.wgcount_elems = !L.use_cull ? 0 : std::max({ceil_div(h.N, 128) * L.PA, ceil_div(h.N, 64) * L.PO, ceil_div(h.M, 128) * L.PB,
                                                  ceil_div(h.N, kMfmaWgPoints) * L.PAm, ceil_div(h.M, kMfmaWgPoints) * L.PBm});
    L.mompart_elems = mompart_elems(h);
    *out = L;
    return PRG_OK;
}
}

namespace {
int ensure_estep_buffers(prg_cpd* h, const EstepLayout& L) {
    PRG_TRY(ensure_buffer(&h->colpart, &h->colpart_elems, L.colpart_elems));
    PRG_TRY(ensure_buffer(&h->rowpart, &h->rowpart_elems, L.rowpart_elems));
    PRG_TRY(ensure_buffer(&h->mompart, &h->mompart_elems, L.mompart_elems));
    if (L.use_queue) PRG_TRY(prg::prepare_queues(h));
    if (L.wgcount_elems > h->wg_cap) {
        if (h->wgcount) {
            PRG_HIP(hipStreamSynchronize(h->stream));
            (void)hipFree(h->wgcount);
        }
        h->wgcount = nullptr;
        h->wg_cap = 0;
        PRG_HIP(hipMalloc((void**)&h->wgcount, (size_t)L.wgcount_elems * 2 * sizeof(unsigned)));
        h->wg_cap = L.wgcount_elems;
    }
    return PRG_OK;
}

int transform_source(prg_cpd* h, int slot) {
    const double* disp = h->bcpd ? h->W : nullptr;
    if (h->nonrigid) PRG_TRY(prg::nonrigid_displacement(h, &disp));
    k_transform_linear<<<(unsigned)prg::ceil_div(h->M, kBlock), kBlock, 0, h->stream>>>(
        h->src4, h->z4, h->M, h->params, h->motion, slot, h->zmeta, h->srcw, disp, h->zchunk);
    return PRG_OK;
}

struct EstepEngines {
    bool use_mfma = false, row_mfma = false;
    bool first = false;
    bool fine = false;
    bool row_lean = false;
    bool fused = false;
    bool col_launched = false;
};

void fill_engine_args(prg_cpd* h, const EstepLayout& L, int slot, EngineArgs* out) {
    const CpdEnv& env = prg::cpd_env();
    EngineArgs ea;
    ea.ext2 = std::max(h->sext2, h->text2);
    ea.r_col_bound = env.r_col > 0.0 ? env.r_col : h->dense_bound > 0.0 ? h->dense_bound : prg::engine_col_bound(h->M, h->N);
    ea.r_col_bound_fused = ea.r_col_bound * fused_lower_bound_scale(L.allow_resid);
    ea.r_row_bound = env.r_row > 0.0 ? env.r_row : prg::engine_row_bound(h->M, h->N, true);
    ea.r_row_bound_full = env.r_row > 0.0 ? env.r_row : prg::engine_row_bound(h->M, h->N, false);
    ea.streamed_col = (double)h->M;
    ea.streamed_row = (double)h->N;
    h->q_first_col = first_queue_unit(ea.r_col_bound, h->N, h->M);
    h->q_first_row = first_queue_unit(ea.r_row_bound, h->M, h->N);
    ea.owned_col = (double)h->N;
    ea.owned_row = (double)h->M;
    ea.work = h->eng_work;
    ea.tsum = h->tsum_local;
    ea.dim = h->D;
    ea.lean_factor = h->lean_factor >= 0.0 ? h->lean_factor : env.lean_factor >= 0.0 ? env.lean_factor : kLeanFactor;
    ea.fused_allowed = L.allow_fused ? 1 : 0;
    ea.resid_allowed = L.allow_resid ? 1 : 0;
    ea.fused_factor = env.fused_factor >= 0.0 ? env.fused_factor : h->fused_factor;
    ea.reset = h->eng.reset ? 1 : 0;
    for (int k = 0; k < 6; ++k) ea.tbox[k] = h->tbox[k];
    ea.slot = slot;
    ea.have_colmin = h->have_colmin ? 1 : 0;
    ea.forced = h->dense_engine >= 2 ? 1 : 0;
    ea.seq = (unsigned)h->estep_count;
    ea.dev = h->eng_dev;
    ea.host = h->eng_host_dev;
    *out = ea;
}

int decide_engines(prg_cpd* h, const EstepLayout& L, int slot, bool cull_seed, hipEvent_t* ev, EstepEngines* out) {
    EstepEngines d;
    *out = d;
    if (!L.mfma_possible || h->eng.mfma_off) {
        if (ev) PRG_HIP(hipEventRecord(ev[1], h->stream));
        return PRG_OK;
    }
    PRG_TRY(prg::ensure_engine_state(h));
    EngineArgs ea;
    fill_engine_args(h, L, slot, &ea);
    h->eng.reset = false;
    prg::launch_chunk_meta_bbox(h, &ea);
    if (ev) PRG_HIP(hipEventRecord(ev[1], h->stream));
    auto seg_col = [&]() { return h->eng.grid_fine && L.seg_col_fine ? L.seg_col_fine : prg::cpd_env().mfma_seg; };
    const bool pred = h->eng.pred_col != 0, pred_fused = L.allow_fused && h->eng.pred_fused != 0;
    const bool vector_grid = !L.use_queue && !L.use_owner;
    if (pred_fused)
        prg::launch_fused_mfma(h, seg_col(), !h->have_colmin, false, h->eng_dev);
    else if (pred)
        prg::launch_colpass_mfma(h, seg_col(), !h->have_colmin, false, h->eng_dev, h->mfma_stream && h->eng.pred_fine == 0 && !h->eng.grid_fine);
    else if (vector_grid)
        prg::launch_colpass_cull(h, L.SA, L.segA, cull_seed, h->eng_dev, L.allow_resid);
    PRG_HIP(hipGetLastError());
    volatile EngineDecision* mb = h->eng_host;
    hipError_t werr;
    const bool got = prg::wait_mailbox(&mb->seq, ea.seq, h->stream, &werr);
    PRG_HIP(werr);
    PRG_REQUIRE(got, PRG_ERR_HIP, "prg_cpd_estep: the engine decision never reached the host");
    d.use_mfma = mb->col != 0;
    d.first = mb->first != 0;
    d.row_mfma = mb->row != 0;
    d.fine = mb->fine != 0;
    d.row_lean = d.row_mfma && mb->lean != 0;
    d.fused = L.allow_fused && mb->fused != 0;
    if (!mb->dense) h->eng.mfma_off = true;
    h->eng.grid_fine = !d.first && (double)mb->r_col < 0.9 * (double)h->M;
    if (prg::cpd_env().debug_engine)
        fprintf(stderr, "[engine] sigma2 %.4e nk*ext2 %.1f pairs per owned point col %.0f (bound %.0f) row %.0f (bound %.0f) motion %.3e cmax %.3e nk*width %.1f "
                        "nk*far2 %.1f have_colmin %d -> col %d (first %d, launched ahead: %s) row %d fine %d\n",
                (double)mb->sigma2, (double)mb->nk_ext2, (double)mb->r_col, ea.r_col_bound, (double)mb->r_row, ea.r_row_bound,
                (double)mb->motion, (double)mb->cmax,
                (double)mb->nk_width, (double)mb->nk_far2, (int)h->have_colmin, (int)d.use_mfma, (int)d.first,
                pred == d.use_mfma ? "yes" : "NO", (int)d.row_mfma, (int)d.fine);
    if (pred_fused)
        d.col_launched = d.fused;
    else if (pred)
        d.col_launched = d.use_mfma && !d.fused;
    else
        d.col_launched = !d.use_mfma && vector_grid;
    h->eng.pred_col = d.use_mfma ? 1 : 0;
    h->eng.pred_fine = d.fine ? 1 : 0;
    h->eng.pred_fused = d.fused ? 1 : 0;
    if (!d.col_launched && d.fused) {
        prg::launch_fused_mfma(h, seg_col(), d.first, d.fine, h->eng_dev);
        d.col_launched = true;
    } else if (!d.col_launched && d.use_mfma) {
        prg::launch_colpass_mfma(h, seg_col(), d.first, d.fine, h->eng_dev, h->mfma_stream && !d.fine && !h->eng.grid_fine);
        d.col_launched = true;
    }
    *out = d;
    return PRG_OK;
}

struct ColumnPass {
    bool owner = false, queue = false;
};
int column_pass(prg_cpd* h, const EstepLayout& L, const EstepEngines& d, bool resid, bool cull_seed, ColumnPass* out) {
    ColumnPass cp;
    cp.owner = !d.col_launched && resid && L.use_owner;
    cp.queue = !d.col_launched && L.use_queue && !cp.owner;
    if (d.col_launched) {
    } else if (cp.owner)
        prg::launch_colpass_owner(h, cull_seed, L.PO);
    else if (cp.queue)
        PRG_TRY(prg::launch_colpass_queue(h, cull_seed, h->qcol_live ? 0 : h->q_first_col, resid));
    else if (L.use_cull)
        prg::launch_colpass_cull(h, L.SA, L.segA, cull_seed, nullptr, resid);
    else if (L.ra < 0)
        prg::launch_colpass_scalar(h, L.RA, L.SA, L.segA);
    else
        prg::launch_colpass_packed(h, L.RA, L.SA, L.segA);
    *out = cp;
    return PRG_OK;
}

int finish_estep(prg_cpd* h, double w, bool col_queue, bool row_queue, bool rowacc_valid) {
    PRG_HIP(hipGetLastError());
    if (h->comm) {
        PRG_TRY(prg::comm_all_reduce_f64(h->comm, h->moments, kMomComp, h->stream));
        if (h->nonrigid && rowacc_valid) PRG_TRY(prg::comm_all_reduce_f64(h->comm, h->rowacc, 4 * h->Mcap, h->stream));
    }
    h->qcol_live = col_queue;
    h->qrow_live = row_queue;
    h->have_estep = true;
    h->rowacc_valid = rowacc_valid;
    h->have_colmin = true;
    h->last_w = w;
    return PRG_OK;
}

int single_sweep_tail(prg_cpd* h, const EstepLayout& L, const EstepEngines& d, const ColumnPass& cp, bool resid, double w, int slot,
                      hipEvent_t* ev) {
    const int nblk = (int)prg::ceil_div(h->N, kBlock);
    float* const colmin_g = h->colmin + h->Ncap;
    const float* part = reinterpret_cast<const float*>(h->colpart);
    if (!resid) {
        k_colfinal_fused<<<nblk, kBlock, 0, h->stream>>>(h->tgt4, part, h->mfma_col_planes, h->Ncap, h->N, h->pt1, h->params, w, m_over_n(h),
                                                         h->D, h->colmin, colmin_g, h->tmeta, d.first ? 2 : 1, h->motion, slot, h->corig,
                                                         h->mompart);
    } else if (cp.queue) {
        k_colfinal_resid<true><<<nblk, kBlock, 0, h->stream>>>(h->tgt4, part, 0, h->Ncap, h->N, h->pt1, h->params, w, m_over_n(h), h->D,
                                                               h->colmin, colmin_g, h->tmeta, h->motion, slot, nullptr,
                                                               queue_view(h->qcol, true), h->mompart, 7);
    } else {
        const int planes = cp.owner ? L.PO : L.PA;
        k_colfinal_resid<false><<<nblk, kBlock, 0, h->stream>>>(h->tgt4, part, planes, h->Ncap, h->N, h->pt1, h->params, w, m_over_n(h), h->D,
                                                                h->colmin, colmin_g, h->tmeta, h->motion, slot, prg::resid_flags(h, planes),
                                                                queue_view(h->qcol, false), h->mompart,
                                                                cp.owner && prg::owner_cols_per_lane() == 1 ? 6 : 7);
    }
    if (ev) {
        PRG_HIP(hipEventRecord(ev[3], h->stream));
        PRG_HIP(hipEventRecord(ev[4], h->stream));
    }
    k_fused_final<<<1, kRedBlock, 0, h->stream>>>(h->mompart, nblk, h->params, h->moments);
    if (ev) PRG_HIP(hipEventRecord(ev[5], h->stream));
    h->wg_row = 0;
    h->dense_pairs_row = 0.0;
    return finish_estep(h, w, cp.queue, false, false);
}

int two_sweep_tail(prg_cpd* h, const EstepLayout& L, const EstepEngines& d, const ColumnPass& cp, double w, int slot, hipEvent_t* ev) {
    const int mfma_seg = prg::cpd_env().mfma_seg;
    double* xpart = h->mompart + (int64_t)prg::mom_blocks(*h) * kMomComp;
    k_colfinal<<<grid1(h->N), kBlock, 0, h->stream>>>(h->tgt4, h->colpart, d.use_mfma ? h->mfma_col_planes : L.PA, h->Ncap, h->N, h->pt1, h->params, w,
                                                      m_over_n(h), h->D, h->colmin, h->colmin + h->Ncap,
                                                      L.use_cull ? h->tmeta : nullptr, d.use_mfma ? (d.first ? 2 : 1) : 0, h->motion, slot,
                                                      queue_view(h->qcol, cp.queue), d.row_lean ? xpart : nullptr);
    if (ev) PRG_HIP(hipEventRecord(ev[3], h->stream));
    const bool row_queue = !d.row_mfma && L.use_queue;
    if (d.row_mfma)
        prg::launch_rowpass_mfma(h, h->eng.grid_fine && L.seg_row_fine ? L.seg_row_fine : mfma_seg, d.fine, d.row_lean, h->mfma_stream && !d.fine && !h->eng.grid_fine);
    else if (row_queue)
        PRG_TRY(prg::launch_rowpass_queue(h, h->qrow_live ? 0 : h->q_first_row));
    else if (L.use_cull)
        prg::launch_rowpass_cull(h, L.SB, L.segB);
    else if (L.rb < 0)
        prg::launch_rowpass_scalar(h, L.RB, L.SB, L.segB);
    else
        prg::launch_rowpass_packed(h, L.RB, L.SB, L.segB);
    if (ev) PRG_HIP(hipEventRecord(ev[4], h->stream));
    const int nblk = (int)std::min<int64_t>(prg::ceil_div(h->M, kBlock), 1024);
    const int row_planes = d.row_mfma ? h->mfma_row_planes : L.PB;
    k_row_moments<<<nblk, kBlock, 0, h->stream>>>(h->rowpart, row_planes, h->Mcap, h->M, h->src4, h->z4, h->rowacc,
                                                  h->mompart,
                                                  L.use_cull ? reinterpret_cast<const unsigned char*>(h->rowpart + (int64_t)row_planes * 5 * h->Mcap)
                                                             : nullptr,
                                                  d.row_mfma ? h->rorig : nullptr, queue_view(h->qrow, row_queue), d.row_lean ? 1 : 0);
    k_reduce_partials<<<1, kRedBlock, 0, h->stream>>>(h->mompart, nblk, kMomComp, h->moments, 0);
    if (d.row_lean) k_xpx_columns<<<1, kBlock, 0, h->stream>>>(xpart, (int)prg::ceil_div(h->N, kBlock), h->moments);
    if (ev) PRG_HIP(hipEventRecord(ev[5], h->stream));
    return finish_estep(h, w, cp.queue, row_queue, true);
}

}

int prg::estep_impl(prg_cpd* h, double w, hipEvent_t* ev) {
    PRG_REQUIRE(h && h->have_source && h->have_target, PRG_ERR_STATE, "prg_cpd_estep: clouds not set");
    PRG_REQUIRE(w >= 0.0 && w < 1.0, PRG_ERR_INVALID, "prg_cpd_estep: w must be in [0, 1) (got %g)", w);
    prg::DeviceGuard g(h->device);
    EstepLayout L;
    PRG_TRY(estep_layout(*h, &L));
    PRG_TRY(ensure_estep_buffers(h, L));

    if (ev) PRG_HIP(hipEventRecord(ev[0], h->stream));
    const int slot = (int)(h->estep_count & 1);
    ++h->estep_count;
    PRG_TRY(transform_source(h, slot));
    const bool cull_seed = h->have_colmin && !h->srcw;
    h->wg_col_pairs = h->wg_row_pairs = 128.0 * prg::kGroup;
    EstepEngines d;
    PRG_TRY(decide_engines(h, L, slot, cull_seed, ev, &d));
    const bool resid = L.allow_resid && !d.use_mfma;
    const bool single = d.fused || resid;
    h->last_estep_mfma = d.use_mfma;
    h->last_estep_fused = single;
    h->last_estep_row_mfma = d.row_mfma && !single;
    h->last_estep_row_lean = d.row_lean && !single;
    ColumnPass cp;
    PRG_TRY(column_pass(h, L, d, resid, cull_seed, &cp));
    if (ev) PRG_HIP(hipEventRecord(ev[2], h->stream));
    return single ? single_sweep_tail(h, L, d, cp, resid, w, slot, ev) : two_sweep_tail(h, L, d, cp, w, slot, ev);
}
```

probreg_amd/csrc/cpd_plan.h:

```cpp
#pragma once
#include <vector>

#include "prg_common.h"

struct EngineDecision {
    unsigned seq;
    int col;
    int first;
    int row;
    int fine;
    int dense;
    float sigma2, motion, cmax, nk_ext2, nk_width, nk_far2;
    float r_col, r_row;
    int row_off;
    int lean;
    int fused;
    int pad_;
};
static_assert(sizeof(EngineDecision) % 8 == 0, "the engine state behind EngineDecision needs 8-byte alignment");
struct EngineArgs {
    double ext2;
    double r_col_bound, r_row_bound;
    double r_col_bound_fused;
    double r_row_bound_full;
    double owned_col, owned_row;
    double streamed_col, streamed_row;
    const double* tsum;
    double lean_factor;
    double fused_factor;
    int dim;
    unsigned long long* work;
    float tbox[6];
    int slot, have_colmin, forced, reset;
    int fused_allowed;
    int resid_allowed;
    unsigned seq;
    EngineDecision* dev;
    EngineDecision* host;
};

struct EngineSwitch {
    bool reset = true;
    bool mfma_off = false;
    int pred_col = 1;
    int pred_fine = 0;
    int pred_fused = 0;
    bool grid_fine = false;
};

struct CpdEnv {
    int mfma_seg = 0;
    bool fine_grid_off = false;
    double r_col = 0.0, r_row = 0.0;
    double fused_rcol_scale = -1.0;
    double lean_factor = -1.0, fused_factor = -1.0;
    bool owner_off = false;
    bool debug_engine = false;
    std::string spatial_order;
};

struct SweepQueue {
    unsigned long long* masks = nullptr;
    int2* chunk = nullptr;
    int2* units = nullptr;
    int* ctrl = nullptr;
    unsigned* ucount = nullptr;
    int64_t cap_blocks = 0, cap_units = 0;
    int cap_chunk = 0;
    int64_t nblocks = 0;
    int nchunk = 0, cap_soft = 0;
};

struct prg_comm {
    void* nccl = nullptr;
    int rank = 0, nranks = 1, device = 0;
    bool owned = true;
    int64_t calls = 0;
};

struct prg_cpd {
    int device = 0;
    hipStream_t stream = nullptr;

    int64_t M = 0, N = 0, Nglobal = 0;
    int D = 0;
    int64_t Mcap = 0, Ncap = 0;

    float4* src4 = nullptr;
    float4* z4 = nullptr;
    float4* tgt4 = nullptr;
    float* pt1 = nullptr;

    float2* colpart = nullptr;
    int64_t colpart_elems = 0;
    float* rowpart = nullptr;
    int64_t rowpart_elems = 0;
    double* rowacc = nullptr;
    double* mompart = nullptr;
    int64_t mompart_elems = 0;

    double* state = nullptr;
    double* moments = nullptr;
    double* params = nullptr;

    int r_col = 0, seg_col = 0, r_row = 0, seg_row = 0;

    bool opt_sort_src = true, opt_sort_tgt = true, opt_cull = true;
    int* perm_src = nullptr;
    int* perm_tgt = nullptr;
    float* zmeta = nullptr;
    float* tmeta = nullptr;
    float* colmin = nullptr;
    unsigned* motion = nullptr;
    bool have_colmin = false;
    float4* rorig = nullptr;
    float4* corig = nullptr;
    bool fused_in_iterate = true;
    bool moments_only = false;
    bool init_rot_orthonormal = true;
    bool resid_sweep = true;
    bool last_estep_fused = false;
    bool rowacc_valid = false;
    float* zchunk = nullptr;
    float* tchunk = nullptr;
    int dense_engine = 1;
    double dense_bound = 0.0;
    double* tsum_local = nullptr;
    unsigned long long* eng_work = nullptr;
    int q_first_col = 32, q_first_row = 32;
    EngineSwitch eng;
    EngineDecision* eng_dev = nullptr;
    EngineDecision* eng_host = nullptr;
    EngineDecision* eng_host_dev = nullptr;
    bool mfma_stream = true;
    int mfma_col_planes = 0, mfma_row_planes = 0;
    bool last_estep_row_lean = false;
    double fused_factor = 256.0;
    double lean_factor = -1.0;
    bool last_estep_mfma = false, last_estep_row_mfma = false;
    double text2 = 0.0, sext2 = 0.0;
    float tbox[6] = {0, 0, 0, 0, 0, 0};
    SweepQueue qcol, qrow;
    int sparse_engine = 1;
    bool qcol_live = false, qrow_live = false;
    unsigned* wgcount = nullptr;
    int64_t wg_cap = 0, wg_col = 0, wg_row = 0;
    double wg_col_pairs = 128.0 * 32.0, wg_row_pairs = 128.0 * 32.0;
    double dense_pairs_col = 0.0, dense_pairs_row = 0.0;
    uint64_t estep_count = 0;

    void* stage = nullptr;
    size_t stage_bytes = 0;

    float* G = nullptr;
    double* W = nullptr;
    double* F = nullptr;
    int64_t f_ld = 0;
    int f_rank = 0, f_cap = 0;
    int nr_solver = 1;
    int nr_max_rank = 0;
    double nr_tol = 1.0e-11;
    double beta = 0.0;
    bool nonrigid = false;
    double* nr_work = nullptr;
    bool gw_valid = false;
    size_t nr_work_bytes = 0;
    double* nr_solve = nullptr;
    size_t nr_solve_bytes = 0;
    int* nr_info = nullptr;
    double* nr_prior = nullptr;
    double nr_alpha = 0.0;
    hipStream_t nr_stream2 = nullptr;
    std::vector<hipEvent_t> nr_events;

    float* srcw = nullptr;
    double uniform_ratio = 0.0;
    bool bcpd = false;

    double* pinned = nullptr;

    bool have_source = false, have_target = false, have_estep = false;
    double last_w = 0.0;

    prg_comm* comm = nullptr;
};

namespace prg {
struct UniqueId { char bytes[PRG_COMM_ID_BYTES]; };
int comm_all_reduce_f64(prg_comm* c, double* buf_dev, int64_t count, hipStream_t st);
int ensure_stage(prg_cpd* h, size_t bytes);
const CpdEnv& cpd_env();
int device_kd_order(const float* pts_dev, int64_t n, int dim, int* perm_dev, hipStream_t st, int leaf = 32);
int nonrigid_displacement(prg_cpd* h, const double** gw_out);
int nonrigid_gw(prg_cpd* h, const double* w3, double* out3);
int nonrigid_free(prg_cpd* h);
int build_kernel_matrix(prg_cpd* h, int kind, double param);
int lowrank_ft3(prg_cpd* h, const double* x3, double* out);
int lowrank_apply(prg_cpd* h, const double* v, double* out3);
}
```

probreg_amd/csrc/cpd_sweeps.h:

```cpp
#pragma once
#include "cpd_plan.h"

namespace prg {
constexpr int kSweepBlock = 256;
constexpr int kColChunk = 8;
constexpr int kRowChunk = 4;
constexpr int kOverRead = 8;

__device__ __forceinline__ float col_offset(float kk, float dmin) {
    const float p = -(kk * dmin);
    return p > 0.f ? __uint_as_float(__float_as_uint(p) - 1u) : 0.f;
}

constexpr int kMfmaOwn = 8;
constexpr int kMfmaWgPoints = 4 * 16 * kMfmaOwn;
__device__ __forceinline__ float col_seed_offset(float kk, float cm, float mo) {
    const float r = __fsqrt_rn(cm);
    const float rl = fmaxf(__fsub_rn(r, mo), 0.f), rh = __fadd_rn(r, mo);
    const float lo = __fmul_rn(rl, rl), hi = __fmul_rn(rh, rh);
    const float nk = -kk;
    const float g = __fmul_rn(nk, __fsub_rn(hi, lo));
    return __fadd_rn(__fmul_rn(nk, lo), fmaxf(__fsub_rn(g, 80.f), 0.f));
}
void launch_colpass_mfma(prg_cpd* h, int S, bool first, bool fine, const EngineDecision* guard, bool stream);
int mfma_stream_planes(int64_t owned_points, int64_t streamed_points);
void launch_chunk_meta_bbox(prg_cpd* h, const EngineArgs* eng);
void launch_fused_mfma(prg_cpd* h, int S, bool first, bool fine, const EngineDecision* guard);
void launch_rowpass_mfma(prg_cpd* h, int S, bool fine, bool lean, bool stream);
int mfma_planes(int64_t owned_points, int64_t streamed_points, int S);
int mfma_chunks_per_seg(int64_t owned_points, int64_t streamed_points, int S);
int mfma_chunks_per_seg_model(int64_t owned_points, int64_t streamed_points);

constexpr int kOwnerWaves = 8;
constexpr int kOwnerMaxPlanes = 32;
constexpr int kOwnerColsPerLane = 1;
int owner_cols_per_lane();
int owner_planes(int64_t owned_points, int64_t streamed_points);
void launch_colpass_owner(prg_cpd* h, bool use_seed, int planes);

constexpr int kQueueChunkGroups = 512;
constexpr int kQueueTargetUnits = 16384;
constexpr int kQueueMaxUnits = 98304;
constexpr int kQueueWorkgroups = 2048;
int launch_colpass_queue(prg_cpd* h, bool use_seed, int q_init, bool resid = false);
int launch_rowpass_queue(prg_cpd* h, int q_init);
int64_t queue_max_units(int64_t owned_points, int64_t streamed_points);
int prepare_queues(prg_cpd* h);

#ifndef PRG_CULL_EXP
#define PRG_CULL_EXP 48
#endif
constexpr float kCullExp = (float)PRG_CULL_EXP;
constexpr int kGroup = 32;
constexpr int kSuper = 256;
void launch_colpass_cull(prg_cpd* h, int S, int seg_len, bool use_seed, const EngineDecision* guard = nullptr, bool resid = false);
inline unsigned char* resid_flags(const prg_cpd* h, int planes) {
    return reinterpret_cast<unsigned char*>(reinterpret_cast<float*>(h->colpart) + (int64_t)planes * 6 * h->Ncap);
}
void launch_rowpass_cull(prg_cpd* h, int S, int seg_len);
void launch_colpass_packed(prg_cpd* h, int R, int S, int seg_len);
void launch_rowpass_packed(prg_cpd* h, int R, int S, int seg_len);
void launch_colpass_scalar(prg_cpd* h, int R, int S, int seg_len);
void launch_rowpass_scalar(prg_cpd* h, int R, int S, int seg_len);
}
```

probreg_amd/csrc/cpd_sweeps_mfma.hip:

```cpp
#include <math.h>

#include <algorithm>
#include <map>
#include <mutex>
#include <vector>

#include "cpd_sweeps.h"

namespace {

typedef float f32x4 __attribute__((ext_vector_type(4)));
typedef float f32x2 __attribute__((ext_vector_type(2)));
typedef __bf16 bf16x8 __attribute__((ext_vector_type(8)));

constexpr double kLog2e = 1.4426950408889634;
constexpr int kBlock = prg::kSweepBlock;
constexpr int kOwn = prg::kMfmaOwn;
constexpr int kWgPoints = 4 * 16 * kOwn;
constexpr int kChunk = 256;
constexpr int kChunkTiles = kChunk / 16;
constexpr int kTileBytes = 1024 + 5 * 64;
constexpr int kTileFloats = kTileBytes / 4;

__device__ __forceinline__ float exp2r(float a) { return __builtin_amdgcn_exp2f(a); }
__device__ __forceinline__ float xor_sum(float v) {
    v += __shfl_xor(v, 16, 64);
    v += __shfl_xor(v, 32, 64);
    return v;
}
__device__ __forceinline__ float xor_max(float v) {
    v = fmaxf(v, __shfl_xor(v, 16, 64));
    v = fmaxf(v, __shfl_xor(v, 32, 64));
    return v;
}

struct alignas(32) BoxMeta { float lo[3]; float hi[3]; float aux; float pad; };

__device__ __forceinline__ float box_gap2(const float (&alo)[3], const float (&ahi)[3], const BoxMeta& g) {
    float d2 = 0.f;
#pragma unroll
    for (int k = 0; k < 3; ++k) {
        const float gap = fmaxf(fmaxf(alo[k] - g.hi[k], g.lo[k] - ahi[k]), 0.f);
        d2 = fmaf(gap, gap, d2);
    }
    return d2;
}

__device__ __forceinline__ bool wg_box(const BoxMeta* __restrict__ gmeta, int64_t first_point, int64_t n_points, int lane,
                                       float (&lo)[3], float (&hi)[3]) {
    const int64_t g = first_point / 32 + (lane & 15);
    const bool valid = (g + 1) * 32 <= n_points;
    const BoxMeta m = gmeta[g];
#pragma unroll
    for (int k = 0; k < 3; ++k) {
        lo[k] = valid ? m.lo[k] : INFINITY;
        hi[k] = valid ? m.hi[k] : -INFINITY;
#pragma unroll
        for (int sh = 1; sh < 16; sh <<= 1) {
            lo[k] = fminf(lo[k], __shfl_xor(lo[k], sh, 64));
            hi[k] = fmaxf(hi[k], __shfl_xor(hi[k], sh, 64));
        }
    }
    return hi[0] >= lo[0];
}

struct WaveBox { float lo[3]; float hi[3]; };
__device__ __forceinline__ bool wave_box(const BoxMeta* __restrict__ gmeta, int64_t first_point, int64_t n_points, int lane,
                                         WaveBox& w) {
    const BoxMeta m = gmeta[first_point / 32 + (lane & 3)];
#pragma unroll
    for (int k = 0; k < 3; ++k) {
        float l = m.lo[k], h = m.hi[k];
        l = fminf(l, __shfl_xor(l, 1, 64));
        l = fminf(l, __shfl_xor(l, 2, 64));
        h = fmaxf(h, __shfl_xor(h, 1, 64));
        h = fmaxf(h, __shfl_xor(h, 2, 64));
        w.lo[k] = __uint_as_float(__builtin_amdgcn_readfirstlane(__float_as_uint(l)));
        w.hi[k] = __uint_as_float(__builtin_amdgcn_readfirstlane(__float_as_uint(h)));
    }
    return first_point + 16 * kOwn <= n_points;
}

__device__ __forceinline__ unsigned tiles_of_groups(unsigned g) {
    g = (g | (g << 4)) & 0x0F0Fu;
    g = (g | (g << 2)) & 0x3333u;
    g = (g | (g << 1)) & 0x5555u;
    return g | (g << 1);
}

struct Split3 { __bf16 h, m, l; };
__device__ __forceinline__ Split3 split3(float a) {
    Split3 s;
    s.h = (__bf16)a;
    const float r1 = a - (float)s.h;
    s.m = (__bf16)r1;
    s.l = (__bf16)(r1 - (float)s.m);
    return s;
}
__device__ __forceinline__ bf16x8 slots_streamed(const Split3 s) {
    const __bf16 z = (__bf16)0.f;
    return (bf16x8){s.h, s.h, s.m, s.h, s.l, s.m, z, z};
}
__device__ __forceinline__ bf16x8 slots_owned(const Split3 s) {
    const __bf16 z = (__bf16)0.f;
    return (bf16x8){s.h, s.m, s.h, s.l, s.h, s.m, z, z};
}

__device__ __forceinline__ void stage_point(float* __restrict__ buf, int p, const float4 v, const float4 o, float kk,
                                            bool lean = false) {
    const float dx = v.x - o.x, dy = v.y - o.y, dz = v.z - o.z;
    const float sq = fmaf(dz, dz, fmaf(dy, dy, dx * dx));
    float* tile = buf + (p >> 4) * kTileFloats;
    bf16x8* a = reinterpret_cast<bf16x8*>(tile);
    const int j = p & 15;
    const __bf16 one = (__bf16)1.f, z = (__bf16)0.f;
    a[0 * 16 + j] = slots_streamed(split3(dx));
    a[1 * 16 + j] = slots_streamed(split3(dy));
    a[2 * 16 + j] = slots_streamed(split3(dz));
    a[3 * 16 + j] = (bf16x8){one, one, one, z, z, z, z, z};
    float* f = tile + 256;
    f[j] = fmaf(kk, sq, v.w);
    *reinterpret_cast<float2*>(f + 16 + 2 * j) = make_float2(dx, dy);
    *reinterpret_cast<float2*>(f + 48 + 2 * j) = make_float2(dz, lean ? 1.f : sq);
}

__device__ __forceinline__ bf16x8 owned_operand(int k, float kk, float dx, float dy, float dz, float cst) {
    const float m2 = -2.f * kk;
    if (k == 0) return slots_owned(split3(m2 * dx));
    if (k == 1) return slots_owned(split3(m2 * dy));
    if (k == 2) return slots_owned(split3(m2 * dz));
    const Split3 c = split3(cst);
    const __bf16 z = (__bf16)0.f;
    return (bf16x8){c.h, c.m, c.l, z, z, z, z, z};
}

struct WorkItem { int blk; int c0; int nc; int plane; bool ends_block; };
struct StreamCut { int g; int pmax; unsigned base; unsigned rem; };
__device__ __forceinline__ unsigned sk_start(unsigned w, const StreamCut sc) { return w * sc.base + (w < sc.rem ? w : sc.rem); }
__device__ __forceinline__ WorkItem sk_item(unsigned u, unsigned u_end, unsigned w, unsigned nchunks, const StreamCut sc) {
    WorkItem it;
    const unsigned blk = u / nchunks, c0 = u - blk * nchunks;
    const unsigned left = nchunks - c0, want = u_end - u;
    it.blk = (int)blk;
    it.c0 = (int)c0;
    it.nc = (int)(want < left ? want : left);
    it.ends_block = c0 + (unsigned)it.nc == nchunks;
    const unsigned x = blk * nchunks, big = sc.rem * (sc.base + 1u);
    const unsigned wf = x < big ? x / (sc.base + 1u) : sc.rem + (x - big) / sc.base;
    it.plane = (int)(w - wf);
    return it;
}

template <bool FUSED>
__global__ __launch_bounds__(kBlock) __attribute__((amdgpu_waves_per_eu(3, FUSED ? 3 : 10))) void k_colpass_mfma(
                                                         const float4* __restrict__ tgt4, const float4* __restrict__ z4,
                                                         const BoxMeta* __restrict__ tmeta,
                                                         const BoxMeta* __restrict__ zmeta,
                                                         const BoxMeta* __restrict__ zchunk,
                                                         const float* __restrict__ colmin_prev,
                                                         const float* __restrict__ colmin_g,
                                                         const unsigned* __restrict__ motion, int chunks_per_seg,
                                                         int64_t m_total, int64_t n_total,
                                                         const double* __restrict__ params,
                                                         float2* __restrict__ colpart, int64_t ncap,
                                                         unsigned* __restrict__ wgcount, unsigned long long* __restrict__ work,
                                                         int first, int fine,
                                                         const EngineDecision* __restrict__ guard, const StreamCut sk,
                                                         float4* __restrict__ corig) {
    __shared__ __attribute__((aligned(16))) float stage[2][kChunkTiles * kTileFloats];
    __shared__ unsigned wave_tiles[kBlock / 64];
    if (guard) {
        const bool fused_wanted = guard->col == 1 && guard->fused == 1;
        if (FUSED ? !fused_wanted : (guard->col != 1 || fused_wanted)) return;
        fine = guard->fine;
    }
    const int lane = threadIdx.x & 63, wv = __builtin_amdgcn_readfirstlane((int)(threadIdx.x >> 6));
    const float kk = (float)(-kLog2e / (2.0 * params[13]));
    const float mo = __uint_as_float(*motion);
    const int nchunks = (int)((m_total + kChunk - 1) / kChunk), nblocks = (int)((n_total + kWgPoints - 1) / kWgPoints);
    const int sk_g = FUSED ? 0 : sk.g, sk_pmax = sk.pmax;
    unsigned unit = sk_g ? sk_start(blockIdx.x, sk) : 0u;
    const unsigned unit_end = sk_g ? sk_start(blockIdx.x + 1u, sk) : 0u;
    for (;;) {
    WorkItem item;
    if (sk_g) {
        item = sk_item(unit, unit_end, blockIdx.x, (unsigned)nchunks, sk);
    } else {
        item.blk = (int)blockIdx.x;
        item.c0 = (int)blockIdx.y * chunks_per_seg;
        item.nc = (item.c0 + chunks_per_seg < nchunks ? item.c0 + chunks_per_seg : nchunks) - item.c0;
        item.plane = blockIdx.y;
        item.ends_block = false;
    }
    const int64_t n0wg = (int64_t)item.blk * kWgPoints, n0 = n0wg + wv * (16 * kOwn);
    float lo[3], hi[3];
    float4 o;
    float thr = INFINITY;
    float thr_w = INFINITY;
    WaveBox wb;
    bool wave_cull = wave_box(tmeta, n0, n_total, lane, wb) && !first && fine;
    if (n0wg + kWgPoints <= n_total && wg_box(tmeta, n0wg, n_total, lane, lo, hi)) {
        o = make_float4(0.5f * (lo[0] + hi[0]), 0.5f * (lo[1] + hi[1]), 0.5f * (lo[2] + hi[2]), 0.f);
        if (!first) {
            float cm = colmin_g[n0wg / 32 + (lane & 15)];
            float cw = __shfl(cm, 4 * wv + (lane & 3), 64);
            cw = fmaxf(cw, __shfl_xor(cw, 1, 64));
            cw = fmaxf(cw, __shfl_xor(cw, 2, 64));
#pragma unroll
            for (int sh = 1; sh < 16; sh <<= 1) cm = fmaxf(cm, __shfl_xor(cm, sh, 64));
            const float r = sqrtf(cm) + mo, rw = sqrtf(cw) + mo;
            thr = r * r * 1.00001f + (-prg::kCullExp) / kk;
            thr_w = rw * rw * 1.00001f + (-prg::kCullExp) / kk;
        }
    } else {
        o = tgt4[n0wg];
        o.w = 0.f;
        wave_cull = false;
#pragma unroll
        for (int q = 0; q < 3; ++q) { lo[q] = -INFINITY; hi[q] = INFINITY; }
    }
    const int k = lane >> 4, j = lane & 15;
    bf16x8 bx[kOwn];
    float s[kOwn], tm[kOwn], off[FUSED ? 1 : kOwn];
    f32x2 uxy[FUSED ? kOwn : 1], uze[FUSED ? kOwn : 1];
#pragma unroll
    for (int t = 0; t < kOwn; ++t) {
        const float4 x = tgt4[n0 + 16 * t + j];
        const float xx = x.x - o.x, xy = x.y - o.y, xz = x.z - o.z;
        const float xsq = fmaf(xz, xz, fmaf(xy, xy, xx * xx));
        const float offt = first ? 0.f : prg::col_seed_offset(kk, colmin_prev[n0 + 16 * t + j], mo);
        if (!FUSED) off[t] = offt;
        bx[t] = owned_operand(k, kk, xx, xy, xz, fmaf(kk, xsq, offt));
        s[t] = 0.f;
        tm[t] = -INFINITY;
        if (FUSED) uxy[t] = uze[t] = (f32x2){0.f, 0.f};
    }
    unsigned tiles_done = 0;
    const int64_t c0 = item.c0;
    const int nc = item.nc;
    const BoxMeta cm = zchunk[c0 + (lane < nc ? lane : nc - 1)];
    unsigned long long mask = __ballot(lane < nc && !(box_gap2(lo, hi, cm) > thr));
    if (mask) {
        int cur = __builtin_ctzll(mask);
        mask &= mask - 1;
        float4 ra = z4[(c0 + cur) * kChunk + threadIdx.x];
        ra.w = 0.f;
        BoxMeta gm = zmeta[wave_cull ? (c0 + cur) * 8 + (lane & 7) : 0];
        stage_point(stage[0], threadIdx.x, ra, o, kk);
        __syncthreads();
        for (int bsel = 0;; bsel ^= 1) {
            const float* __restrict__ buf = stage[bsel];
            unsigned tmask = 0xFFFFu;
            if (wave_cull)
                tmask = tiles_of_groups((unsigned)__ballot(lane < 8 && !(box_gap2(wb.lo, wb.hi, gm) > thr_w)) & 0xFFu);
            const int nxt = mask ? __builtin_ctzll(mask) : -1;
            mask &= mask - 1;
            if (nxt >= 0) {
                ra = z4[(c0 + nxt) * kChunk + threadIdx.x];
                ra.w = 0.f;
                if (wave_cull) gm = zmeta[(c0 + nxt) * 8 + (lane & 7)];
            }
            tiles_done += __popc(tmask);
            auto tile_step = [&](f32x4& d, const float* __restrict__ tb, const bf16x8 a1, const f32x4 cz, const bf16x8 a1n,
                                 const f32x4 czn) {
                f32x2 xy0, xy1, xy2, xy3, zs0, zs1, zs2, zs3;
                if (FUSED) {
                    const f32x4 a01 = *reinterpret_cast<const f32x4*>(tb + 272 + 8 * k), a23 = *reinterpret_cast<const f32x4*>(tb + 276 + 8 * k),
                                b01 = *reinterpret_cast<const f32x4*>(tb + 304 + 8 * k), b23 = *reinterpret_cast<const f32x4*>(tb + 308 + 8 * k);
                    xy0 = (f32x2){a01[0], a01[1]}; xy1 = (f32x2){a01[2], a01[3]}; xy2 = (f32x2){a23[0], a23[1]}; xy3 = (f32x2){a23[2], a23[3]};
                    zs0 = (f32x2){b01[0], b01[1]}; zs1 = (f32x2){b01[2], b01[3]}; zs2 = (f32x2){b23[0], b23[1]}; zs3 = (f32x2){b23[2], b23[3]};
                }
#pragma unroll
                for (int u = 0; u < kOwn; ++u) {
                    const f32x4 dn = u + 1 < kOwn ? __builtin_amdgcn_mfma_f32_16x16x32_bf16(a1, bx[u + 1], cz, 0, 0, 0)
                                                  : __builtin_amdgcn_mfma_f32_16x16x32_bf16(a1n, bx[0], czn, 0, 0, 0);
                    tm[u] = fmaxf(fmaxf(tm[u], d[0]), d[1]);
                    tm[u] = fmaxf(fmaxf(tm[u], d[2]), d[3]);
                    const float q0 = exp2r(d[0]), q1 = exp2r(d[1]), q2 = exp2r(d[2]), q3 = exp2r(d[3]);
                    s[u] += (q0 + q1) + (q2 + q3);
                    if (FUSED) {
                        const f32x2 s0 = {q0, q0}, s1 = {q1, q1}, s2 = {q2, q2}, s3 = {q3, q3};
                        uxy[u] = __builtin_elementwise_fma(s3, xy3, __builtin_elementwise_fma(s2, xy2, __builtin_elementwise_fma(s1, xy1, __builtin_elementwise_fma(s0, xy0, uxy[u]))));
                        uze[u] = __builtin_elementwise_fma(s3, zs3, __builtin_elementwise_fma(s2, zs2, __builtin_elementwise_fma(s1, zs1, __builtin_elementwise_fma(s0, zs0, uze[u]))));
                    }
                    d = dn;
                }
            };
            if (tmask == 0xFFFFu) {
                bf16x8 a1 = reinterpret_cast<const bf16x8*>(buf)[lane];
                f32x4 cz = *reinterpret_cast<const f32x4*>(buf + 256 + 4 * k);
                f32x4 d = __builtin_amdgcn_mfma_f32_16x16x32_bf16(a1, bx[0], cz, 0, 0, 0);
                for (int t = 0; t < kChunkTiles; ++t) {
                    const float* __restrict__ tn = buf + (t + 1 < kChunkTiles ? t + 1 : t) * kTileFloats;
                    const bf16x8 a1n = reinterpret_cast<const bf16x8*>(tn)[lane];
                    const f32x4 czn = *reinterpret_cast<const f32x4*>(tn + 256 + 4 * k);
                    tile_step(d, buf + t * kTileFloats, a1, cz, a1n, czn);
                    a1 = a1n;
                    cz = czn;
                }
            } else if (tmask) {
                int t = __builtin_ctz(tmask);
                tmask &= tmask - 1;
                bf16x8 a1 = reinterpret_cast<const bf16x8*>(buf + t * kTileFloats)[lane];
                f32x4 cz = *reinterpret_cast<const f32x4*>(buf + t * kTileFloats + 256 + 4 * k);
                f32x4 d = __builtin_amdgcn_mfma_f32_16x16x32_bf16(a1, bx[0], cz, 0, 0, 0);
                for (;;) {
                    const bool more = tmask != 0;
                    const int t2 = more ? __builtin_ctz(tmask) : t;
                    tmask &= tmask - 1;
                    const float* __restrict__ tn = buf + t2 * kTileFloats;
                    const bf16x8 a1n = reinterpret_cast<const bf16x8*>(tn)[lane];
                    const f32x4 czn = *reinterpret_cast<const f32x4*>(tn + 256 + 4 * k);
                    tile_step(d, buf + t * kTileFloats, a1, cz, a1n, czn);
                    if (!more) break;
                    t = t2;
                    a1 = a1n;
                    cz = czn;
                }
            }
            if (nxt >= 0) stage_point(stage[bsel ^ 1], threadIdx.x, ra, o, kk);
            __syncthreads();
            if (nxt < 0) break;
        }
    }
    if (lane == 0) wave_tiles[wv] = tiles_done;
    __syncthreads();
    if (threadIdx.x == 0) {
        const unsigned tiles = wave_tiles[0] + wave_tiles[1] + wave_tiles[2] + wave_tiles[3];
        wgcount[(int64_t)item.plane * nblocks + item.blk] = tiles;
        if (tiles) atomicAdd(work, (unsigned long long)tiles);
    }
    if (FUSED) {
        float* __restrict__ fout = reinterpret_cast<float*>(colpart) + (int64_t)item.plane * 6 * ncap + n0;
#pragma unroll
        for (int u2 = 0; u2 < kOwn; ++u2) {
            const float st = xor_sum(s[u2]), tt = xor_max(tm[u2]);
            const float bxs = xor_sum(uxy[u2][0]), bys = xor_sum(uxy[u2][1]), bzs = xor_sum(uze[u2][0]), es = xor_sum(uze[u2][1]);
            if (lane < 16) {
                const float offt = first ? 0.f : prg::col_seed_offset(kk, colmin_prev[n0 + 16 * u2 + lane], mo);
                float dmin = fmaxf((tt - offt) / kk, 0.f);
                dmin = fmaf(dmin, 2.0e-4f, dmin) + 1.0e-12f;
                fout[16 * u2 + lane] = tt == -INFINITY ? INFINITY : dmin;
                fout[ncap + 16 * u2 + lane] = st;
                fout[2 * ncap + 16 * u2 + lane] = bxs;
                fout[3 * ncap + 16 * u2 + lane] = bys;
                fout[4 * ncap + 16 * u2 + lane] = bzs;
                fout[5 * ncap + 16 * u2 + lane] = es;
            }
        }
        if (item.plane == 0 && threadIdx.x == 0) corig[item.blk] = o;
        break;
    }
    float2* __restrict__ out = colpart + (int64_t)item.plane * ncap + n0;
#pragma unroll
    for (int u2 = 0; u2 < kOwn; ++u2) {
        const float st = xor_sum(s[u2]);
        const float tt = xor_max(tm[u2]);
        if (lane < 16) {
            float dmin = fmaxf((tt - off[u2]) / kk, 0.f);
            dmin = fmaf(dmin, 2.0e-4f, dmin) + 1.0e-12f;
            out[16 * u2 + lane] = make_float2(tt == -INFINITY ? INFINITY : dmin, st);
        }
    }
    if (!sk_g) break;
    if (item.ends_block) {
        for (int q = item.plane + 1; q < sk_pmax; ++q) {
            colpart[(int64_t)q * ncap + n0wg + threadIdx.x] = make_float2(INFINITY, 0.f);
            colpart[(int64_t)q * ncap + n0wg + kBlock + threadIdx.x] = make_float2(INFINITY, 0.f);
            if (threadIdx.x == 0) wgcount[(int64_t)q * nblocks + item.blk] = 0u;
        }
    }
    unit += item.nc;
    if (unit >= unit_end) break;
    __syncthreads();
    }
}

template <bool LEAN, bool STREAM>
__global__ __launch_bounds__(kBlock) __attribute__((amdgpu_waves_per_eu(3, STREAM ? 3 : 10))) void k_rowpass_mfma(const float4* __restrict__ z4, const float4* __restrict__ tgt4,
                                                         const BoxMeta* __restrict__ zmeta,
                                                         const BoxMeta* __restrict__ tmeta,
                                                         const BoxMeta* __restrict__ tchunk, int chunks_per_seg,
                                                         int64_t n_total, int64_t m_total,
                                                         const double* __restrict__ params, float* __restrict__ rowpart,
                                                         int64_t mcap, float4* __restrict__ rorig,
                                                         unsigned char* __restrict__ rowflag,
                                                         unsigned* __restrict__ wgcount, unsigned long long* __restrict__ work,
                                                         int fine, const StreamCut sk) {
    __shared__ __attribute__((aligned(16))) float stage[2][kChunkTiles * kTileFloats];
    __shared__ unsigned wave_tiles[kBlock / 64];
    const int lane = threadIdx.x & 63, wv = __builtin_amdgcn_readfirstlane((int)(threadIdx.x >> 6));
    const float kk = (float)(-kLog2e / (2.0 * params[13]));
    const int nchunks = (int)((n_total + kChunk - 1) / kChunk), nblocks = (int)((m_total + kWgPoints - 1) / kWgPoints);
    const int sk_pmax = sk.pmax;
    unsigned unit = STREAM ? sk_start(blockIdx.x, sk) : 0u;
    const unsigned unit_end = STREAM ? sk_start(blockIdx.x + 1u, sk) : 0u;
    for (;;) {
    WorkItem item;
    if (STREAM) {
        item = sk_item(unit, unit_end, blockIdx.x, (unsigned)nchunks, sk);
    } else {
        item.blk = (int)blockIdx.x;
        item.c0 = (int)blockIdx.y * chunks_per_seg;
        item.nc = (item.c0 + chunks_per_seg < nchunks ? item.c0 + chunks_per_seg : nchunks) - item.c0;
        item.plane = blockIdx.y;
        item.ends_block = false;
    }
    const int64_t m0wg = (int64_t)item.blk * kWgPoints, m0 = m0wg + wv * (16 * kOwn);
    float lo[3], hi[3];
    float4 o;
    WaveBox wb;
    bool wave_cull = wave_box(zmeta, m0, m_total, lane, wb) && fine;
    if (m0wg + kWgPoints <= m_total && wg_box(zmeta, m0wg, m_total, lane, lo, hi)) {
        o = make_float4(0.5f * (lo[0] + hi[0]), 0.5f * (lo[1] + hi[1]), 0.5f * (lo[2] + hi[2]), 0.f);
    } else {
        o = z4[m0wg];
        o.w = 0.f;
        wave_cull = false;
#pragma unroll
        for (int q = 0; q < 3; ++q) { lo[q] = -INFINITY; hi[q] = INFINITY; }
    }
    const int k = lane >> 4, j = lane & 15;
    bf16x8 bz[kOwn];
    f32x2 uxy[kOwn], uze[kOwn], pp[LEAN ? 1 : kOwn];
#pragma unroll
    for (int t = 0; t < kOwn; ++t) {
        const float4 z = z4[m0 + 16 * t + j];
        const float zx = z.x - o.x, zy = z.y - o.y, zz = z.z - o.z;
        bz[t] = owned_operand(k, kk, zx, zy, zz, kk * fmaf(zz, zz, fmaf(zy, zy, zx * zx)));
        uxy[t] = uze[t] = (f32x2){0.f, 0.f};
        if (!LEAN) pp[t] = (f32x2){0.f, 0.f};
    }
    unsigned tiles_done = 0;
    const int64_t c0 = item.c0;
    const int nc = item.nc;
    const BoxMeta cm = tchunk[c0 + (lane < nc ? lane : nc - 1)];
    unsigned long long mask = __ballot(lane < nc && !(fmaf(box_gap2(lo, hi, cm), kk, cm.aux) < -prg::kCullExp));
    if (mask) {
        int cur = __builtin_ctzll(mask);
        mask &= mask - 1;
        float4 ra = tgt4[(c0 + cur) * kChunk + threadIdx.x];
        BoxMeta gm = tmeta[wave_cull ? (c0 + cur) * 8 + (lane & 7) : 0];
        stage_point(stage[0], threadIdx.x, ra, o, kk, LEAN);
        __syncthreads();
        for (int bsel = 0;; bsel ^= 1) {
            const float* __restrict__ buf = stage[bsel];
            unsigned tmask = 0xFFFFu;
            if (wave_cull)
                tmask = tiles_of_groups(
                    (unsigned)__ballot(lane < 8 && !(fmaf(box_gap2(wb.lo, wb.hi, gm), kk, gm.aux) < -prg::kCullExp)) & 0xFFu);
            const int nxt = mask ? __builtin_ctzll(mask) : -1;
            mask &= mask - 1;
            if (nxt >= 0) {
                ra = tgt4[(c0 + nxt) * kChunk + threadIdx.x];
                if (wave_cull) gm = tmeta[(c0 + nxt) * 8 + (lane & 7)];
            }
            tiles_done += __popc(tmask);
            auto tile_step = [&](f32x4& d, const float* __restrict__ tb, const bf16x8 a1, const f32x4 cx, const bf16x8 a1n,
                                 const f32x4 cxn) {
                const f32x4 a01 = *reinterpret_cast<const f32x4*>(tb + 272 + 8 * k), a23 = *reinterpret_cast<const f32x4*>(tb + 276 + 8 * k),
                            b01 = *reinterpret_cast<const f32x4*>(tb + 304 + 8 * k), b23 = *reinterpret_cast<const f32x4*>(tb + 308 + 8 * k);
                const f32x2 xy0 = {a01[0], a01[1]}, xy1 = {a01[2], a01[3]}, xy2 = {a23[0], a23[1]}, xy3 = {a23[2], a23[3]};
                const f32x2 zs0 = {b01[0], b01[1]}, zs1 = {b01[2], b01[3]}, zs2 = {b23[0], b23[1]}, zs3 = {b23[2], b23[3]};
#pragma unroll
                for (int u = 0; u < kOwn; ++u) {
                    const f32x4 dn = u + 1 < kOwn ? __builtin_amdgcn_mfma_f32_16x16x32_bf16(a1, bz[u + 1], cx, 0, 0, 0)
                                                  : __builtin_amdgcn_mfma_f32_16x16x32_bf16(a1n, bz[0], cxn, 0, 0, 0);
                    const float q0 = exp2r(d[0]), q1 = exp2r(d[1]), q2 = exp2r(d[2]), q3 = exp2r(d[3]);
                    const f32x2 s0 = {q0, q0}, s1 = {q1, q1}, s2 = {q2, q2}, s3 = {q3, q3};
                    if (!LEAN) {
                        pp[u] += (f32x2){q0, q1};
                        pp[u] += (f32x2){q2, q3};
                    }
                    uxy[u] = __builtin_elementwise_fma(s3, xy3, __builtin_elementwise_fma(s2, xy2, __builtin_elementwise_fma(s1, xy1, __builtin_elementwise_fma(s0, xy0, uxy[u]))));
                    uze[u] = __builtin_elementwise_fma(s3, zs3, __builtin_elementwise_fma(s2, zs2, __builtin_elementwise_fma(s1, zs1, __builtin_elementwise_fma(s0, zs0, uze[u]))));
                    d = dn;
                }
            };
            if (tmask == 0xFFFFu) {
                bf16x8 a1 = reinterpret_cast<const bf16x8*>(buf)[lane];
                f32x4 cx = *reinterpret_cast<const f32x4*>(buf + 256 + 4 * k);
                f32x4 d = __builtin_amdgcn_mfma_f32_16x16x32_bf16(a1, bz[0], cx, 0, 0, 0);
                for (int t = 0; t < kChunkTiles; ++t) {
                    const float* __restrict__ tn = buf + (t + 1 < kChunkTiles ? t + 1 : t) * kTileFloats;
                    const bf16x8 a1n = reinterpret_cast<const bf16x8*>(tn)[lane];
                    const f32x4 cxn = *reinterpret_cast<const f32x4*>(tn + 256 + 4 * k);
                    tile_step(d, buf + t * kTileFloats, a1, cx, a1n, cxn);
                    a1 = a1n;
                    cx = cxn;
                }
            } else if (tmask) {
                int t = __builtin_ctz(tmask);
                tmask &= tmask - 1;
                bf16x8 a1 = reinterpret_cast<const bf16x8*>(buf + t * kTileFloats)[lane];
                f32x4 cx = *reinterpret_cast<const f32x4*>(buf + t * kTileFloats + 256 + 4 * k);
                f32x4 d = __builtin_amdgcn_mfma_f32_16x16x32_bf16(a1, bz[0], cx, 0, 0, 0);
                for (;;) {
                    const bool more = tmask != 0;
                    const int t2 = more ? __builtin_ctz(tmask) : t;
                    tmask &= tmask - 1;
                    const float* __restrict__ tn = buf + t2 * kTileFloats;
                    const bf16x8 a1n = reinterpret_cast<const bf16x8*>(tn)[lane];
                    const f32x4 cxn = *reinterpret_cast<const f32x4*>(tn + 256 + 4 * k);
                    tile_step(d, buf + t * kTileFloats, a1, cx, a1n, cxn);
                    if (!more) break;
                    t = t2;
                    a1 = a1n;
                    cx = cxn;
                }
            }
            if (nxt >= 0) stage_point(stage[bsel ^ 1], threadIdx.x, ra, o, kk, LEAN);
            __syncthreads();
            if (nxt < 0) break;
        }
    }
    if (lane == 0) wave_tiles[wv] = tiles_done;
    __syncthreads();
    if (threadIdx.x == 0) {
        const unsigned tiles = wave_tiles[0] + wave_tiles[1] + wave_tiles[2] + wave_tiles[3];
        wgcount[(int64_t)item.plane * nblocks + item.blk] = tiles;
        if (tiles) atomicAdd(work, (unsigned long long)tiles);
    }
    const bool touched = tiles_done != 0;
    if (lane == 0) rowflag[((int64_t)item.blk * 4 + wv) * 64 + item.plane] = touched ? 1 : 0;
    if (touched) {
        float* __restrict__ out = rowpart + (int64_t)item.plane * 5 * mcap + m0;
#pragma unroll
        for (int u = 0; u < kOwn; ++u) {
            const float a0 = xor_sum(LEAN ? uze[u][1] : pp[LEAN ? 0 : u][0] + pp[LEAN ? 0 : u][1]), a1s = xor_sum(uxy[u][0]),
                        a2 = xor_sum(uxy[u][1]), a3 = xor_sum(uze[u][0]);
            if (!LEAN) {
                const float a4 = xor_sum(uze[u][1]);
                if (lane < 16) out[4 * mcap + 16 * u + lane] = a4;
            }
            if (lane < 16) {
                out[16 * u + lane] = a0;
                out[mcap + 16 * u + lane] = a1s;
                out[2 * mcap + 16 * u + lane] = a2;
                out[3 * mcap + 16 * u + lane] = a3;
            }
        }
    }
    if (item.c0 == 0 && threadIdx.x == 0) rorig[item.blk] = o;
    if (!STREAM) break;
    if (item.ends_block) {
        for (int q = item.plane + 1 + lane; q < sk_pmax; q += 64) rowflag[((int64_t)item.blk * 4 + wv) * 64 + q] = 0;
        if (threadIdx.x == 0)
            for (int q = item.plane + 1; q < sk_pmax; ++q) wgcount[(int64_t)q * nblocks + item.blk] = 0u;
    }
    unit += item.nc;
    if (unit >= unit_end) break;
    __syncthreads();
    }
}

__global__ __launch_bounds__(kBlock) void k_chunk_meta(const BoxMeta* __restrict__ gmeta, int64_t nchunk,
                                                       BoxMeta* __restrict__ cmeta) {
    const int64_t c = (int64_t)blockIdx.x * kBlock + threadIdx.x;
    if (c >= nchunk) return;
    BoxMeta o = gmeta[c * 8];
#pragma unroll
    for (int g = 1; g < 8; ++g) {
        const BoxMeta m = gmeta[c * 8 + g];
#pragma unroll
        for (int k = 0; k < 3; ++k) {
            o.lo[k] = fminf(o.lo[k], m.lo[k]);
            o.hi[k] = fmaxf(o.hi[k], m.hi[k]);
        }
        o.aux = fmaxf(o.aux, m.aux);
    }
    cmeta[c] = o;
}

__global__ __launch_bounds__(kBlock) void k_chunk_meta_bbox(const BoxMeta* __restrict__ gmeta, int64_t nchunk,
                                                            BoxMeta* __restrict__ cmeta, const float4* __restrict__ pts,
                                                            int64_t m, unsigned* __restrict__ stat,
                                                            const double* __restrict__ params, const EngineArgs eng) {
    __shared__ float sh[kBlock / 64][6];
    float lo[3] = {INFINITY, INFINITY, INFINITY}, hi[3] = {-INFINITY, -INFINITY, -INFINITY};
    for (int64_t c = threadIdx.x; c < nchunk; c += kBlock) {
        BoxMeta o = gmeta[c * 8];
#pragma unroll
        for (int g = 0; g < 8; ++g) {
            const BoxMeta q = gmeta[c * 8 + g];
#pragma unroll
            for (int k = 0; k < 3; ++k) {
                o.lo[k] = fminf(o.lo[k], q.lo[k]);
                o.hi[k] = fmaxf(o.hi[k], q.hi[k]);
            }
            o.aux = fmaxf(o.aux, q.aux);
            if ((c * 8 + g + 1) * 32 <= m) {
#pragma unroll
                for (int k = 0; k < 3; ++k) {
                    lo[k] = fminf(lo[k], q.lo[k]);
                    hi[k] = fmaxf(hi[k], q.hi[k]);
                }
            }
        }
        cmeta[c] = o;
    }
    const int64_t tail = (m / 32) * 32 + threadIdx.x;
    if (threadIdx.x < 32 && tail < m) {
        const float4 p = pts[tail];
        lo[0] = fminf(lo[0], p.x); hi[0] = fmaxf(hi[0], p.x);
        lo[1] = fminf(lo[1], p.y); hi[1] = fmaxf(hi[1], p.y);
        lo[2] = fminf(lo[2], p.z); hi[2] = fmaxf(hi[2], p.z);
    }
#pragma unroll
    for (int k = 0; k < 3; ++k) {
#pragma unroll
        for (int sft = 1; sft <= 32; sft <<= 1) {
            lo[k] = fminf(lo[k], __shfl_xor(lo[k], sft, 64));
            hi[k] = fmaxf(hi[k], __shfl_xor(hi[k], sft, 64));
        }
    }
    if ((threadIdx.x & 63) == 0)
#pragma unroll
        for (int k = 0; k < 3; ++k) {
            sh[threadIdx.x >> 6][k] = lo[k];
            sh[threadIdx.x >> 6][3 + k] = hi[k];
        }
    __syncthreads();
    if (threadIdx.x != 0) return;
    float box[6];
#pragma unroll
    for (int q = 0; q < 6; ++q) {
        float v = sh[0][q];
        for (int w = 1; w < kBlock / 64; ++w) v = q < 3 ? fminf(v, sh[w][q]) : fmaxf(v, sh[w][q]);
        box[q] = v;
        stat[8 + q] = __float_as_uint(v);
    }
    if (!eng.dev) return;
    const double sigma2 = params[13], nk = kLog2e / (2.0 * sigma2);
    const double mo = __uint_as_float(stat[eng.slot]), cmax = __uint_as_float(stat[4 + (eng.slot ^ 1)]), r = sqrt(cmax);
    const double width = r >= mo ? 4.0 * r * mo : (r + mo) * (r + mo);
    const bool ok = sigma2 > 0.0 && isfinite(sigma2);
    const EngineDecision prev = *eng.dev;
    float r_col = eng.reset ? (float)eng.streamed_col : prev.r_col, r_row = eng.reset ? (float)eng.streamed_row : prev.r_row;
    int row_off = eng.reset ? 0 : prev.row_off;
    const unsigned long long tc = eng.work[0], tr = eng.work[1];
    eng.work[0] = 0ull;
    eng.work[1] = 0ull;
    if (tc && !eng.reset) r_col = (float)((double)tc * 2048.0 / eng.owned_col);
    if (tr && !eng.reset) r_row = (float)((double)tr * 2048.0 / eng.owned_row);

    const bool lean_ok = eng.tsum && eng.tsum[3] > 0.0 && sigma2 * (double)eng.dim * eng.lean_factor * eng.owned_col >= eng.tsum[3];
    if (prev.fused && tc && !eng.reset) r_row = (float)((double)r_col * eng.owned_col / eng.owned_row);
    const bool fused_ok = eng.tsum && eng.tsum[3] > 0.0 && sigma2 * (double)eng.dim * eng.fused_factor * eng.owned_col >= eng.tsum[3];
    const bool fused_try = eng.fused_allowed && fused_ok && !row_off;
    bool dense = ok && (eng.forced || r_col >= (fused_try ? eng.r_col_bound_fused : eng.r_col_bound));
    if (dense && !eng.forced && eng.fused_allowed && eng.resid_allowed && !fused_try && !(r_col >= 0.6 * eng.streamed_col)) dense = false;
    if (!fused_try && !(r_row >= (lean_ok ? eng.r_row_bound : eng.r_row_bound_full))) row_off = 1;
    double far2 = 0.0;
#pragma unroll
    for (int k = 0; k < 3; ++k) {
        const double a = fabs((double)eng.tbox[3 + k] - (double)box[k]), b = fabs((double)box[3 + k] - (double)eng.tbox[k]);
        far2 += fmax(a, b) * fmax(a, b);
    }
    const bool first = dense && !eng.have_colmin && isfinite(far2) && nk * far2 < 110.0;
    const bool col = first || (dense && eng.have_colmin && isfinite(cmax) && nk * width < 150.0);
    const bool row = dense && (eng.forced || !row_off);
    const bool lean = row && lean_ok;
    EngineDecision d;
    d.seq = eng.seq;
    d.col = col ? 1 : 0;
    d.first = first ? 1 : 0;
    d.row = row ? 1 : 0;
    d.fine = nk * eng.ext2 > 200.0 * (prg::kCullExp / 127.0) ? 1 : 0;
    d.dense = dense ? 1 : 0;
    d.sigma2 = (float)sigma2; d.motion = (float)mo; d.cmax = (float)cmax;
    d.nk_ext2 = (float)(nk * eng.ext2); d.nk_width = (float)(nk * width); d.nk_far2 = (float)(nk * far2);
    d.r_col = r_col; d.r_row = r_row; d.row_off = row_off; d.lean = lean ? 1 : 0;
    d.fused = eng.fused_allowed && col && row && fused_ok ? 1 : 0;
    *eng.dev = d;
    EngineDecision* hm = eng.host;
    hm->col = d.col; hm->first = d.first; hm->row = d.row; hm->fine = d.fine; hm->dense = d.dense;
    hm->sigma2 = d.sigma2; hm->motion = d.motion; hm->cmax = d.cmax;
    hm->nk_ext2 = d.nk_ext2; hm->nk_width = d.nk_width; hm->nk_far2 = d.nk_far2;
    hm->r_col = d.r_col; hm->r_row = d.r_row; hm->row_off = d.row_off; hm->lean = d.lean; hm->fused = d.fused;
    __threadfence_system();
    __hip_atomic_store(&hm->seq, d.seq, __ATOMIC_RELEASE, __HIP_MEMORY_SCOPE_SYSTEM);
}

}

namespace prg {

static double mfma_dense_makespan(int64_t blocks, int64_t chunks, int64_t cps, double over) {
    const int64_t segs = ceil_div(chunks, cps), rem = chunks - (segs - 1) * cps;
    std::vector<double> slot(768, 0.0);
    auto later = [](double a, double b) { return a > b; };
    double end = 0.0;
    for (int64_t y = 0; y < segs; ++y) {
        const double d = (double)(y + 1 < segs ? cps : rem) + over;
        for (int64_t x = 0; x < blocks; ++x) {
            std::pop_heap(slot.begin(), slot.end(), later);
            const double t = slot.back() + d;
            slot.back() = t;
            std::push_heap(slot.begin(), slot.end(), later);
            end = std::max(end, t);
        }
    }
    return end;
}

int mfma_chunks_per_seg(int64_t owned_points, int64_t streamed_points, int S) {
    const int64_t chunks = ceil_div(streamed_points, kChunk);
    if (S <= 0) {
        const int64_t blocks = ceil_div(owned_points, kWgPoints);
        static std::mutex mu;
        static std::map<std::pair<int64_t, int64_t>, int> memo;
        static const bool old_model = getenv("PRG_MFMA_SEG_MODEL") && atoi(getenv("PRG_MFMA_SEG_MODEL")) == 4;
        std::lock_guard<std::mutex> lock(mu);
        const auto key = std::make_pair(blocks, chunks);
        const auto hit = memo.find(key);
        if (hit != memo.end()) {
            S = hit->second;
        } else {
            double best = 1e30;
            S = 1;
            for (int64_t cand = 4; cand <= 32; ++cand) {
                const int64_t cps = ceil_div(chunks, std::min<int64_t>(cand, chunks));
                if (cps > 64) continue;
                const int64_t segs = ceil_div(chunks, cps);
                const double cost = old_model ? (double)ceil_div(blocks * segs, (int64_t)768) * (double)cps
                                              : mfma_dense_makespan(blocks, chunks, cps, 0.15);
                if (cost < best * 0.999) {
                    best = cost;
                    S = (int)cand;
                }
            }
            memo[key] = S;
        }
    }
    const int64_t cps = ceil_div(chunks, std::min<int64_t>(S, chunks));
    return (int)std::min<int64_t>(cps, 64);
}

int mfma_chunks_per_seg_model(int64_t owned_points, int64_t streamed_points) {
    const int64_t chunks = ceil_div(streamed_points, kChunk), blocks = ceil_div(owned_points, kWgPoints);
    double best = 1e30;
    int64_t best_cps = chunks;
    for (int64_t cand = 4; cand <= 32; ++cand) {
        const int64_t cps = ceil_div(chunks, std::min<int64_t>(cand, chunks));
        const int64_t segs = ceil_div(chunks, cps);
        const double cost = (double)ceil_div(blocks * segs, (int64_t)768) * (double)cps;
        if (cost < best * 0.999) {
            best = cost;
            best_cps = cps;
        }
    }
    return (int)std::min<int64_t>(best_cps, 64);
}

int mfma_planes(int64_t owned_points, int64_t streamed_points, int S) {
    const int cps = mfma_chunks_per_seg(owned_points, streamed_points, S);
    return (int)ceil_div(ceil_div(streamed_points, kChunk), cps);
}

void launch_chunk_meta(prg_cpd* h, const float* gmeta, int64_t cap, float* cmeta) {
    const int64_t nchunk = cap / kChunk;
    k_chunk_meta<<<(unsigned)ceil_div(nchunk, kBlock), kBlock, 0, h->stream>>>(reinterpret_cast<const BoxMeta*>(gmeta), nchunk,
                                                                             reinterpret_cast<BoxMeta*>(cmeta));
}

void launch_chunk_meta_bbox(prg_cpd* h, const EngineArgs* eng) {
    EngineArgs none;
    none.dev = nullptr;
    none.host = nullptr;
    k_chunk_meta_bbox<<<1, kBlock, 0, h->stream>>>(reinterpret_cast<const BoxMeta*>(h->zmeta), h->Mcap / kChunk,
                                                  reinterpret_cast<BoxMeta*>(h->zchunk), h->z4, h->M, h->motion, h->params,
                                                  eng ? *eng : none);
}

constexpr int kStreamSlots = 768;
static int64_t stream_workgroups(int64_t blocks, int64_t chunks) {
    const int64_t units = blocks * chunks;
    return kStreamSlots * ceil_div(units, (int64_t)kStreamSlots * 64);
}
int mfma_stream_planes(int64_t owned_points, int64_t streamed_points) {
    static const bool off = getenv("PRG_MFMA_STREAM") && atoi(getenv("PRG_MFMA_STREAM")) == 0;
    const int64_t blocks = ceil_div(owned_points, kWgPoints), chunks = ceil_div(streamed_points, kChunk);
    if (off || blocks * chunks < 4 * (int64_t)kStreamSlots || blocks * chunks >= (int64_t)1 << 31) return 0;
    static thread_local int64_t last_blocks = -1, last_chunks = -1;
    static thread_local int last_planes = 0;
    if (blocks != last_blocks || chunks != last_chunks) {
        const int64_t units = blocks * chunks, g = stream_workgroups(blocks, chunks), base = units / g, rem = units % g;
        auto holder = [&](int64_t x) { return x < rem * (base + 1) ? x / (base + 1) : rem + (x - rem * (base + 1)) / base; };
        int64_t most = 0;
        for (int64_t b = 0; b < blocks; ++b) most = std::max(most, holder((b + 1) * chunks - 1) - holder(b * chunks) + 1);
        last_blocks = blocks;
        last_chunks = chunks;
        last_planes = (int)most;
    }
    return last_planes <= 48 ? last_planes : 0;
}

static StreamCut stream_cut(int planes, int64_t blocks, int64_t chunks) {
    StreamCut c = {0, 0, 0u, 0u};
    if (planes > 0) {
        const int64_t units = blocks * chunks, g = stream_workgroups(blocks, chunks);
        c.g = (int)g;
        c.pmax = planes;
        c.base = (unsigned)(units / g);
        c.rem = (unsigned)(units % g);
    }
    return c;
}

void launch_colpass_mfma(prg_cpd* h, int S, bool first, bool fine, const EngineDecision* guard, bool stream) {
    const int cps = mfma_chunks_per_seg(h->N, h->M, S);
    const int sp = stream ? mfma_stream_planes(h->N, h->M) : 0;
    const int64_t nblocks = ceil_div(h->N, kWgPoints);
    dim3 grid((unsigned)nblocks, (unsigned)ceil_div(ceil_div(h->M, kChunk), cps));
    h->mfma_col_planes = sp ? sp : (int)grid.y;
    const StreamCut cut = stream_cut(sp, nblocks, ceil_div(h->M, kChunk));
    if (sp) grid = dim3((unsigned)cut.g, 1);
    k_colpass_mfma<false><<<grid, kBlock, 0, h->stream>>>(h->tgt4, h->z4, reinterpret_cast<const BoxMeta*>(h->tmeta),
                                                   reinterpret_cast<const BoxMeta*>(h->zmeta),
                                                   reinterpret_cast<const BoxMeta*>(h->zchunk), h->colmin, h->colmin + h->Ncap,
                                                   h->motion + ((h->estep_count - 1) & 1), cps, h->M, h->N, h->params,
                                                   h->colpart, h->Ncap, h->wgcount, h->eng_work, first ? 1 : 0, fine ? 1 : 0, guard,
                                                   cut, nullptr);
    h->wg_col = nblocks * h->mfma_col_planes;
    h->wg_col_pairs = 128.0 * 16.0;
    h->dense_pairs_col = 0.0;
}

void launch_fused_mfma(prg_cpd* h, int S, bool first, bool fine, const EngineDecision* guard) {
    const int cps = mfma_chunks_per_seg(h->N, h->M, S);
    const int64_t nblocks = ceil_div(h->N, kWgPoints);
    dim3 grid((unsigned)nblocks, (unsigned)ceil_div(ceil_div(h->M, kChunk), cps));
    h->mfma_col_planes = (int)grid.y;
    const StreamCut none = {0, 0, 0u, 0u};
    k_colpass_mfma<true><<<grid, kBlock, 0, h->stream>>>(h->tgt4, h->z4, reinterpret_cast<const BoxMeta*>(h->tmeta),
                                                         reinterpret_cast<const BoxMeta*>(h->zmeta),
                                                         reinterpret_cast<const BoxMeta*>(h->zchunk), h->colmin, h->colmin + h->Ncap,
                                                         h->motion + ((h->estep_count - 1) & 1), cps, h->M, h->N, h->params,
                                                         h->colpart, h->Ncap, h->wgcount, h->eng_work, first ? 1 : 0, fine ? 1 : 0, guard,
                                                         none, h->corig);
    h->wg_col = nblocks * h->mfma_col_planes;
    h->wg_col_pairs = 128.0 * 16.0;
    h->dense_pairs_col = 0.0;
}

void launch_rowpass_mfma(prg_cpd* h, int S, bool fine, bool lean, bool stream) {
    const int cps = mfma_chunks_per_seg(h->M, h->N, S);
    const int sp = stream && lean ? mfma_stream_planes(h->M, h->N) : 0;
    const int64_t nblocks = ceil_div(h->M, kWgPoints);
    dim3 grid((unsigned)nblocks, (unsigned)ceil_div(ceil_div(h->N, kChunk), cps));
    h->mfma_row_planes = sp ? sp : (int)grid.y;
    const StreamCut cut = stream_cut(sp, nblocks, ceil_div(h->N, kChunk));
    if (sp) grid = dim3((unsigned)cut.g, 1);
    unsigned char* rowflag = reinterpret_cast<unsigned char*>(h->rowpart + (int64_t)h->mfma_row_planes * 5 * h->Mcap);
    launch_chunk_meta(h, h->tmeta, h->Ncap, h->tchunk);
    auto kernel = sp ? k_rowpass_mfma<true, true> : lean ? k_rowpass_mfma<true, false> : k_rowpass_mfma<false, false>;
    kernel<<<grid, kBlock, 0, h->stream>>>(h->z4, h->tgt4, reinterpret_cast<const BoxMeta*>(h->zmeta),
                                           reinterpret_cast<const BoxMeta*>(h->tmeta), reinterpret_cast<const BoxMeta*>(h->tchunk), cps,
                                           h->N, h->M, h->params, h->rowpart, h->Mcap, h->rorig, rowflag, h->wgcount + h->wg_cap,
                                           h->eng_work + 1, fine ? 1 : 0, cut);
    h->wg_row = nblocks * h->mfma_row_planes;
    h->wg_row_pairs = 128.0 * 16.0;
    h->dense_pairs_row = 0.0;
}

}
```

probreg_amd/engine.py:

```python
import ctypes

import numpy as np

from . import _lib
from ._lib import check, lib, ptr


def _current_device_and_stream(device=None):
    try:
        import torch

        if torch.cuda.is_available():
            dev = torch.cuda.current_device() if device is None else int(device)
            return dev, int(torch.cuda.current_stream(dev).cuda_stream)
    except ImportError:
        pass
    return (0 if device is None else int(device)), 0


def spatial_order(points, on_device=True):
    import numpy as np

    pts = np.ascontiguousarray(points, dtype=np.float32)
    perm = np.empty(pts.shape[0], dtype=np.int32)
    check(lib.prg_spatial_order(pts.ctypes.data_as(ctypes.c_void_p), int(pts.shape[0]), int(pts.shape[1]), 1 if on_device else 0,
                                perm.ctypes.data_as(ctypes.c_void_p)))
    return perm


def engine_bounds(m, n_local):
    a, b = ctypes.c_double(0.0), ctypes.c_double(0.0)
    check(lib.prg_cpd_engine_bounds(int(m), int(n_local), ctypes.byref(a), ctypes.byref(b)))
    return float(a.value), float(b.value)


class CpdPlan(object):

    def __init__(self, device=None, stream=None):
        _lib.require_gpu()
        dev, st = _current_device_and_stream(device)
        if stream is not None:
            st = int(stream)
        self.device = dev
        self.stream = st
        self._h = ctypes.c_void_p()
        check(lib.prg_cpd_create(ctypes.byref(self._h), dev, ctypes.c_void_p(st)))
        self._moments_tensor = None
        self._comm = None
        self.m = self.n = self.dim = 0

    def close(self):
        if getattr(self, "_h", None) is not None and self._h:
            lib.prg_cpd_destroy(self._h)
            self._h = None

    def __del__(self):
        try:
            self.close()
        except Exception:
            pass

    @staticmethod
    def _f32(a):
        if hasattr(a, "data_ptr"):
            import torch

            assert a.dtype == torch.float32 and a.is_contiguous()
            return a
        return np.ascontiguousarray(a, dtype=np.float32)

    def set_options(self, sort_source=True, sort_target=True, cull=True):
        check(lib.prg_cpd_set_options(self._h, int(sort_source), int(sort_target), int(cull)))

    def set_dense_engine(self, mode=1, bound=0.0):
        check(lib.prg_cpd_set_dense_engine(self._h, int(mode), float(bound)))

    def last_estep_engine(self):
        e = ctypes.c_int(0)
        check(lib.prg_cpd_last_estep_engine(self._h, ctypes.byref(e)))
        return int(e.value)

    def set_sparse_engine(self, mode=1):
        check(lib.prg_cpd_set_sparse_engine(self._h, int(mode)))

    def last_estep_engines(self):
        c, r = ctypes.c_int(0), ctypes.c_int(0)
        check(lib.prg_cpd_last_estep_engines(self._h, ctypes.byref(c), ctypes.byref(r)))
        return int(c.value), int(r.value)

    def last_estep_lean(self):
        v = ctypes.c_int(0)
        check(lib.prg_cpd_last_estep_lean(self._h, ctypes.byref(v)))
        return int(v.value)

    def set_stream_mode(self, on=True):
        check(lib.prg_cpd_set_stream_mode(self._h, 1 if on else 0))

    def set_lean_factor(self, factor=-1.0):
        check(lib.prg_cpd_set_lean_factor(self._h, float(factor)))

    def set_source(self, source):
        a = self._f32(source)
        self.m, self.dim = int(a.shape[0]), int(a.shape[1])
        check(lib.prg_cpd_set_source(self._h, ptr(a), self.m, self.dim))

    def set_target(self, target_local, n_global=None):
        a = self._f32(target_local)
        self.n = int(a.shape[0])
        check(lib.prg_cpd_set_target(self._h, ptr(a), self.n, int(a.shape[1]), int(n_global or self.n)))

    def set_tuning(self, r_col=0, seg_col=0, r_row=0, seg_row=0):
        check(lib.prg_cpd_set_tuning(self._h, r_col, seg_col, r_row, seg_row))

    def set_comm(self, comm):
        check(lib.prg_cpd_set_comm(self._h, comm._h if comm is not None else None))
        old = getattr(self, "_comm", None)
        if old is not None and old is not comm:
            old._detached(self)
        self._comm = comm
        if comm is not None:
            comm._attached(self)

    def iterate(self, kind, update_scale, w, n_iter):
        check(lib.prg_cpd_iterate(self._h, int(kind), 1 if update_scale else 0, float(w), int(n_iter)))

    def set_moments_only(self, mode=1):
        check(lib.prg_cpd_set_moments_only(self._h, int(mode)))

    def set_resid_sweep(self, on=True):
        check(lib.prg_cpd_set_resid_sweep(self._h, 1 if on else 0))

    def set_fused_factor(self, factor=256.0):
        check(lib.prg_cpd_set_fused_factor(self._h, float(factor)))

    def last_estep_fused(self):
        v = ctypes.c_int(0)
        check(lib.prg_cpd_last_estep_fused(self._h, ctypes.byref(v)))
        return int(v.value)

    def moments_tensor(self):
        if self._moments_tensor is None:
            import torch

            t = torch.zeros(_lib.PRG_NMOMENTS, dtype=torch.float64, device="cuda:%d" % self.device)
            check(lib.prg_cpd_bind_moments(self._h, ctypes.c_void_p(t.data_ptr())))
            self._moments_tensor = t
        return self._moments_tensor

    def rowacc_tensor_view(self):
        p = ctypes.c_void_p()
        cnt = ctypes.c_int64()
        check(lib.prg_cpd_rowacc_ptr(self._h, ctypes.byref(p), ctypes.byref(cnt)))
        return p.value, int(cnt.value)

    def init_sums(self):
        check(lib.prg_cpd_init_sums(self._h))

    def init_params(self, init16=None):
        if init16 is None:
            check(lib.prg_cpd_init_params(self._h, None))
        else:
            a = np.ascontiguousarray(init16, dtype=np.float64)
            assert a.size == 16
            check(lib.prg_cpd_init_params(self._h, ptr(a)))

    def estep(self, w=0.0):
        check(lib.prg_cpd_estep(self._h, float(w)))

    def estep_timed(self, w=0.0):
        ms = np.zeros(6, dtype=np.float32)
        check(lib.prg_cpd_estep_timed(self._h, float(w), ptr(ms)))
        names = ("transform", "colpass", "colfinal", "rowpass", "moments", "total")
        return dict(zip(names, [float(v) for v in ms]))

    def pair_counts(self):
        a, b = ctypes.c_double(0.0), ctypes.c_double(0.0)
        check(lib.prg_cpd_pair_counts(self._h, ctypes.byref(a), ctypes.byref(b)))
        return float(a.value), float(b.value)

    def mstep(self, kind, update_scale=True):
        check(lib.prg_cpd_mstep(self._h, int(kind), 1 if update_scale else 0))

    def mstep_nonrigid(self, lmd):
        check(lib.prg_cpd_mstep_nonrigid(self._h, float(lmd)))

    def get_params(self):
        out = np.empty(_lib.PRG_NPARAMS, dtype=np.float64)
        check(lib.prg_cpd_get_params(self._h, ptr(out)))
        return out

    def set_params(self, params):
        a = np.ascontiguousarray(params, dtype=np.float64)
        assert a.size == _lib.PRG_NPARAMS
        check(lib.prg_cpd_set_params(self._h, ptr(a)))

    def get_moments(self):
        out = np.empty(_lib.PRG_NMOMENTS, dtype=np.float64)
        check(lib.prg_cpd_get_moments(self._h, ptr(out)))
        return out

    def get_estep(self):
        pt1 = np.empty(self.n, dtype=np.float64)
        p1 = np.empty(self.m, dtype=np.float64)
        px = np.empty((self.m, self.dim), dtype=np.float64)
        check(lib.prg_cpd_get_estep(self._h, ptr(pt1), ptr(p1), ptr(px)))
        return pt1, p1, px

    def get_estep_pt1(self):
        pt1 = np.empty(self.n, dtype=np.float64)
        check(lib.prg_cpd_get_estep(self._h, ptr(pt1), None, None))
        return pt1

    def get_tsource(self):
        out = np.empty((self.m, self.dim), dtype=np.float32)
        check(lib.prg_cpd_get_tsource(self._h, ptr(out)))
        return out

    def moments_from_estep(self, pt1, p1, px):
        pt1 = np.ascontiguousarray(pt1, dtype=np.float64)
        p1 = np.ascontiguousarray(p1, dtype=np.float64)
        px = np.ascontiguousarray(px, dtype=np.float64)
        assert pt1.shape == (self.n,) and p1.shape == (self.m,) and px.shape == (self.m, self.dim)
        check(lib.prg_cpd_moments_from_estep(self._h, ptr(pt1), ptr(p1), ptr(px)))

    def build_g(self, beta):
        check(lib.prg_cpd_nonrigid_build_g(self._h, float(beta)))

    def set_nonrigid_solver(self, mode=1, max_rank=0, tol=0.0):
        check(lib.prg_cpd_nonrigid_set_solver(self._h, int(mode), int(max_rank), float(tol)))

    def nonrigid_rank(self):
        r = ctypes.c_int(0)
        check(lib.prg_cpd_nonrigid_rank(self._h, ctypes.byref(r)))
        return int(r.value)

    def get_g(self):
        out = np.empty((self.m, self.m), dtype=np.float32)
        check(lib.prg_cpd_nonrigid_get_g(self._h, ptr(out)))
        return out

    def set_w(self, w):
        a = np.ascontiguousarray(w, dtype=np.float64)
        assert a.shape == (self.m, self.dim)
        check(lib.prg_cpd_nonrigid_set_w(self._h, ptr(a)))

    def get_w(self):
        out = np.empty((self.m, self.dim), dtype=np.float64)
        check(lib.prg_cpd_nonrigid_get_w(self._h, ptr(out)))
        return out

    def set_priors(self, p1_tilde, px_tilde, alpha):
        a = np.ascontiguousarray(p1_tilde, dtype=np.float64)
        b = np.ascontiguousarray(px_tilde, dtype=np.float64)
        assert a.shape == (self.m,) and b.shape == (self.m, self.dim)
        check(lib.prg_cpd_nonrigid_set_priors(self._h, ptr(a), ptr(b), float(alpha)))

    def nonrigid_apply(self):
        out = np.empty((self.m, self.dim), dtype=np.float64)
        check(lib.prg_cpd_nonrigid_apply(self._h, ptr(out)))
        return out

    def set_source_weights(self, log_weights, uniform_ratio=0.0):
        if log_weights is None:
            check(lib.prg_cpd_set_source_weights(self._h, None, float(uniform_ratio)))
            return
        a = np.ascontiguousarray(log_weights, dtype=np.float64)
        assert a.shape == (self.m,)
        check(lib.prg_cpd_set_source_weights(self._h, ptr(a), float(uniform_ratio)))

    def bcpd_build_g(self, c=1.0):
        check(lib.prg_cpd_bcpd_build_g(self._h, float(c)))

    def bcpd_solve(self, lmd, cfac, resid, nu=None):
        r = np.ascontiguousarray(resid, dtype=np.float64)
        assert r.shape == (self.m, self.dim)
        v = np.empty((self.m, self.dim), dtype=np.float64)
        d = np.empty(self.m, dtype=np.float64)
        nu_a = None if nu is None else np.ascontiguousarray(nu, dtype=np.float64)
        assert nu_a is None or nu_a.shape == (self.m,)
        check(lib.prg_cpd_bcpd_solve(self._h, float(lmd), float(cfac), None if nu_a is None else ptr(nu_a), ptr(r),
                                     ptr(v), ptr(d)))
        return v, d

    def synchronize(self):
        self.get_params()
```

Measured before the change: 10070 EM iterations/s.

## Add per-wave culled fused E-step kernel with work-filling part split

Adds a new fused column-pass kernel in which each wavefront independently walks only the source chunk groups that survive its own box-distance cull. It double-buffers staged tiles in per-wave LDS using wave-level fences instead of block barriers. The grid's second dimension is a 'parts' count chosen to fill the stream slots. This path is enabled by default (mode 1) once the engine predicts the column pass is sparse enough (r_col below 0.9·M). The goal is to skip culled work and block-synchronisation stalls in the late sparse phase, at the cost of more partial planes to reduce and fixed 3-waves-per-EU occupancy.

After: 9966 EM iterations/s. 0.99x the previous value.

```diff
diff --git a/include/probreg_hip.h b/include/probreg_hip.h
--- a/include/probreg_hip.h
+++ b/include/probreg_hip.h
@@ -67,6 +67,9 @@
 int prg_cpd_set_moments_only(prg_cpd* h, int mode);
 int prg_cpd_last_estep_fused(prg_cpd* h, int* fused);
 int prg_cpd_set_fused_factor(prg_cpd* h, double factor);
+int prg_cpd_set_fused_wave(prg_cpd* h, int mode);
+int prg_cpd_last_estep_fused_wave(prg_cpd* h, int* wave);
+int prg_cpd_fused_wave_parts(int64_t m, int64_t n_local, int* parts, int* parts_cap);
 int prg_cpd_set_resid_sweep(prg_cpd* h, int on);
 
 int prg_cpd_init_sums(prg_cpd* h);
diff --git a/probreg_amd/_lib.py b/probreg_amd/_lib.py
--- a/probreg_amd/_lib.py
+++ b/probreg_amd/_lib.py
@@ -76,6 +76,9 @@
     "prg_cpd_iterate": [_vp, _i, _i, _d, _i],
     "prg_cpd_set_moments_only": [_vp, _i],
     "prg_cpd_last_estep_fused": [_vp, _c.POINTER(_i)],
+    "prg_cpd_set_fused_wave": [_vp, _i],
+    "prg_cpd_last_estep_fused_wave": [_vp, _c.POINTER(_i)],
+    "prg_cpd_fused_wave_parts": [_i64, _i64, _c.POINTER(_i), _c.POINTER(_i)],
     "prg_cpd_set_fused_factor": [_vp, _d],
     "prg_cpd_set_resid_sweep": [_vp, _i],
     "prg_cpd_init_sums": [_vp],
diff --git a/probreg_amd/csrc/cpd.hip b/probreg_amd/csrc/cpd.hip
--- a/probreg_amd/csrc/cpd.hip
+++ b/probreg_amd/csrc/cpd.hip
@@ -424,6 +424,7 @@
         e.r_col = num("PRG_ENGINE_RCOL", 0.0);
         e.r_row = num("PRG_ENGINE_RROW", 0.0);
         e.fused_rcol_scale = num("PRG_FUSED_RCOL_SCALE", -1.0);
+        e.fused_wave_below = num("PRG_FUSED_WAVE_BELOW", -1.0);
         e.lean_factor = num("PRG_LEAN_FACTOR", -1.0);
         e.fused_factor = num("PRG_FUSED_FACTOR", -1.0);
         e.owner_off = is_zero("PRG_OWNER_SWEEP");
@@ -727,6 +728,26 @@
     return PRG_OK;
 }
 
+int prg_cpd_set_fused_wave(prg_cpd* h, int mode) {
+    PRG_REQUIRE(h, PRG_ERR_INVALID, "prg_cpd_set_fused_wave: NULL handle");
+    PRG_REQUIRE(mode >= 0 && mode <= 2, PRG_ERR_INVALID, "prg_cpd_set_fused_wave: mode must be 0, 1 or 2");
+    h->fused_wave = mode;
+    return PRG_OK;
+}
+
+int prg_cpd_last_estep_fused_wave(prg_cpd* h, int* wave) {
+    PRG_REQUIRE(h && wave, PRG_ERR_INVALID, "prg_cpd_last_estep_fused_wave: NULL argument");
+    *wave = h->last_estep_fused_wave ? 1 : 0;
+    return PRG_OK;
+}
+
+int prg_cpd_fused_wave_parts(int64_t m, int64_t n_local, int* parts, int* parts_cap) {
+    PRG_REQUIRE(m > 0 && n_local > 0 && parts && parts_cap, PRG_ERR_INVALID, "prg_cpd_fused_wave_parts: need m, n_local > 0 and an output");
+    *parts = prg::fused_wave_parts(n_local, m);
+    *parts_cap = prg::kFusedWaveMaxParts;
+    return PRG_OK;
+}
+
 int prg_cpd_set_stream_mode(prg_cpd* h, int on) {
     PRG_REQUIRE(h, PRG_ERR_INVALID, "prg_cpd_set_stream_mode: NULL handle");
     h->mfma_stream = on != 0;
@@ -1014,6 +1035,7 @@
     PRG_HIP(hipStreamSynchronize(h->stream));
     h->have_estep = true;
     h->last_estep_fused = false;
+    h->last_estep_fused_wave = false;
     h->rowacc_valid = true;
     return PRG_OK;
 }
diff --git a/probreg_amd/csrc/cpd_estep.h b/probreg_amd/csrc/cpd_estep.h
--- a/probreg_amd/csrc/cpd_estep.h
+++ b/probreg_amd/csrc/cpd_estep.h
@@ -10,6 +10,7 @@
     int SA, segA, PA;
     int SB, segB, PB;
     bool mfma_possible;
+    int fused_wave_parts;
     int seg_col_fine, seg_row_fine;
     int PAm, PBm;
     bool use_queue;
diff --git a/probreg_amd/csrc/cpd_estep.hip b/probreg_amd/csrc/cpd_estep.hip
--- a/probreg_amd/csrc/cpd_estep.hip
+++ b/probreg_amd/csrc/cpd_estep.hip
@@ -771,6 +771,11 @@
     return env > 0.0 ? env : allow_resid ? 1.0 : 0.5;
 }
 
+double fused_wave_below() {
+    const double env = prg::cpd_env().fused_wave_below;
+    return env > 0.0 ? env : 0.9;
+}
+
 constexpr double kLeanFactor = 64.0;
 
 int first_queue_unit(double bound, int64_t owned, int64_t streamed) {
@@ -830,11 +835,13 @@
     L.seg_row_fine = L.mfma_possible ? mfma_fine_segments(h.M, h.N, 64) : 0;
     const int col_grid_planes = L.mfma_possible ? std::max(mfma_planes(h.N, h.M, env.mfma_seg), mfma_planes(h.N, h.M, L.seg_col_fine)) : 0;
     const int row_grid_planes = L.mfma_possible ? std::max(mfma_planes(h.M, h.N, env.mfma_seg), mfma_planes(h.M, h.N, L.seg_row_fine)) : 0;
-    L.PAm = L.mfma_possible ? std::max(col_grid_planes, mfma_stream_planes(h.N, h.M)) : 0;
+    L.fused_wave_parts = L.mfma_possible && !env.mfma_seg ? fused_wave_parts(h.N, h.M) : 0;
+    L.PAm = L.mfma_possible ? std::max({col_grid_planes, mfma_stream_planes(h.N, h.M), L.fused_wave_parts}) : 0;
     L.PBm = L.mfma_possible ? std::max(row_grid_planes, mfma_stream_planes(h.M, h.N)) : 0;
     L.use_queue = L.use_cull && (h.sparse_engine == 2 || ((h.sparse_engine == 1 || h.sparse_engine == 3) && h.M >= 32768 && h.N >= 32768));
     const bool single_ok = h.moments_only && !h.nonrigid && !h.bcpd && h.init_rot_orthonormal;
     L.allow_fused = L.mfma_possible && single_ok;
+    if (!L.allow_fused) L.fused_wave_parts = 0;
     L.allow_resid = L.use_cull && h.resid_sweep && single_ok && !h.srcw;
     L.use_owner = L.allow_resid && h.sparse_engine == 1 && !env.owner_off;
     L.PO = L.use_owner ? owner_planes(h.N, h.M) : 0;
@@ -842,7 +849,7 @@
     const int64_t col_grid = (int64_t)L.PA * h.Ncap;
     const int64_t col_mfma = (int64_t)L.PAm * h.Ncap;
     const int64_t col_queue = L.use_queue ? queue_max_units(h.N, h.M) * 128 : 0;
-    const int64_t col_fused = L.allow_fused ? (int64_t)3 * col_grid_planes * h.Ncap : 0;
+    const int64_t col_fused = L.allow_fused ? (int64_t)3 * std::max(col_grid_planes, L.fused_wave_parts) * h.Ncap : 0;
     const int64_t col_resid = !L.allow_resid ? 0 : L.use_owner ? resid_plane_elems(h, L.PO, 64)
                               : L.use_queue ? 3 * col_queue : resid_plane_elems(h, L.PA, 128);
     L.colpart_elems = std::max({col_grid, col_mfma, col_queue, col_fused, col_resid});
@@ -939,10 +946,11 @@
     prg::launch_chunk_meta_bbox(h, &ea);
     if (ev) PRG_HIP(hipEventRecord(ev[1], h->stream));
     auto seg_col = [&]() { return h->eng.grid_fine && L.seg_col_fine ? L.seg_col_fine : prg::cpd_env().mfma_seg; };
+    auto wave_parts = [&]() { return h->fused_wave == 2 || (h->fused_wave == 1 && h->eng.fused_wave) ? L.fused_wave_parts : 0; };
     const bool pred = h->eng.pred_col != 0, pred_fused = L.allow_fused && h->eng.pred_fused != 0;
     const bool vector_grid = !L.use_queue && !L.use_owner;
     if (pred_fused)
-        prg::launch_fused_mfma(h, seg_col(), !h->have_colmin, false, h->eng_dev);
+        prg::launch_fused_mfma(h, seg_col(), !h->have_colmin, false, h->eng_dev, wave_parts());
     else if (pred)
         prg::launch_colpass_mfma(h, seg_col(), !h->have_colmin, false, h->eng_dev, h->mfma_stream && h->eng.pred_fine == 0 && !h->eng.grid_fine);
     else if (vector_grid)
@@ -961,6 +969,7 @@
     d.fused = L.allow_fused && mb->fused != 0;
     if (!mb->dense) h->eng.mfma_off = true;
     h->eng.grid_fine = !d.first && (double)mb->r_col < 0.9 * (double)h->M;
+    h->eng.fused_wave = !d.first && (double)mb->r_col < fused_wave_below() * (double)h->M;
     if (prg::cpd_env().debug_engine)
         fprintf(stderr, "[engine] sigma2 %.4e nk*ext2 %.1f pairs per owned point col %.0f (bound %.0f) row %.0f (bound %.0f) motion %.3e cmax %.3e nk*width %.1f "
                         "nk*far2 %.1f have_colmin %d -> col %d (first %d, launched ahead: %s) row %d fine %d\n",
@@ -978,7 +987,7 @@
     h->eng.pred_fine = d.fine ? 1 : 0;
     h->eng.pred_fused = d.fused ? 1 : 0;
     if (!d.col_launched && d.fused) {
-        prg::launch_fused_mfma(h, seg_col(), d.first, d.fine, h->eng_dev);
+        prg::launch_fused_mfma(h, seg_col(), d.first, d.fine, h->eng_dev, wave_parts());
         d.col_launched = true;
     } else if (!d.col_launched && d.use_mfma) {
         prg::launch_colpass_mfma(h, seg_col(), d.first, d.fine, h->eng_dev, h->mfma_stream && !d.fine && !h->eng.grid_fine);
@@ -1111,6 +1120,7 @@
     const bool single = d.fused || resid;
     h->last_estep_mfma = d.use_mfma;
     h->last_estep_fused = single;
+    h->last_estep_fused_wave = d.fused && h->fused_wave_launched;
     h->last_estep_row_mfma = d.row_mfma && !single;
     h->last_estep_row_lean = d.row_lean && !single;
     ColumnPass cp;
diff --git a/probreg_amd/csrc/cpd_plan.h b/probreg_amd/csrc/cpd_plan.h
--- a/probreg_amd/csrc/cpd_plan.h
+++ b/probreg_amd/csrc/cpd_plan.h
@@ -46,6 +46,7 @@
     int pred_fine = 0;
     int pred_fused = 0;
     bool grid_fine = false;
+    bool fused_wave = false;
 };
 
 struct CpdEnv {
@@ -53,6 +54,7 @@
     bool fine_grid_off = false;
     double r_col = 0.0, r_row = 0.0;
     double fused_rcol_scale = -1.0;
+    double fused_wave_below = -1.0;
     double lean_factor = -1.0, fused_factor = -1.0;
     bool owner_off = false;
     bool debug_engine = false;
@@ -120,6 +122,9 @@
     bool init_rot_orthonormal = true;
     bool resid_sweep = true;
     bool last_estep_fused = false;
+    int fused_wave = 1;
+    bool fused_wave_launched = false;
+    bool last_estep_fused_wave = false;
     bool rowacc_valid = false;
     float* zchunk = nullptr;
     float* tchunk = nullptr;
diff --git a/probreg_amd/csrc/cpd_sweeps.h b/probreg_amd/csrc/cpd_sweeps.h
--- a/probreg_amd/csrc/cpd_sweeps.h
+++ b/probreg_amd/csrc/cpd_sweeps.h
@@ -25,7 +25,9 @@
 void launch_colpass_mfma(prg_cpd* h, int S, bool first, bool fine, const EngineDecision* guard, bool stream);
 int mfma_stream_planes(int64_t owned_points, int64_t streamed_points);
 void launch_chunk_meta_bbox(prg_cpd* h, const EngineArgs* eng);
-void launch_fused_mfma(prg_cpd* h, int S, bool first, bool fine, const EngineDecision* guard);
+void launch_fused_mfma(prg_cpd* h, int S, bool first, bool fine, const EngineDecision* guard, int wave_parts);
+constexpr int kFusedWaveMaxParts = 32;
+int fused_wave_parts(int64_t owned_points, int64_t streamed_points);
 void launch_rowpass_mfma(prg_cpd* h, int S, bool fine, bool lean, bool stream);
 int mfma_planes(int64_t owned_points, int64_t streamed_points, int S);
 int mfma_chunks_per_seg(int64_t owned_points, int64_t streamed_points, int S);
diff --git a/probreg_amd/csrc/cpd_sweeps_mfma.hip b/probreg_amd/csrc/cpd_sweeps_mfma.hip
--- a/probreg_amd/csrc/cpd_sweeps_mfma.hip
+++ b/probreg_amd/csrc/cpd_sweeps_mfma.hip
@@ -149,6 +149,34 @@
     const unsigned wf = x < big ? x / (sc.base + 1u) : sc.rem + (x - big) / sc.base;
     it.plane = (int)(w - wf);
     return it;
+}
+
+template <bool FUSED>
+__device__ __forceinline__ void tile_step(f32x4& d, const float* __restrict__ tb, const bf16x8 a1, const f32x4 cz, const bf16x8 a1n,
+                                          const f32x4 czn, const int k, const bf16x8 (&bx)[kOwn], float (&s)[kOwn], float (&tm)[kOwn],
+                                          f32x2 (&uxy)[FUSED ? kOwn : 1], f32x2 (&uze)[FUSED ? kOwn : 1]) {
+    f32x2 xy0, xy1, xy2, xy3, zs0, zs1, zs2, zs3;
+    if constexpr (FUSED) {
+        const f32x4 a01 = *reinterpret_cast<const f32x4*>(tb + 272 + 8 * k), a23 = *reinterpret_cast<const f32x4*>(tb + 276 + 8 * k),
+                    b01 = *reinterpret_cast<const f32x4*>(tb + 304 + 8 * k), b23 = *reinterpret_cast<const f32x4*>(tb + 308 + 8 * k);
+        xy0 = (f32x2){a01[0], a01[1]}; xy1 = (f32x2){a01[2], a01[3]}; xy2 = (f32x2){a23[0], a23[1]}; xy3 = (f32x2){a23[2], a23[3]};
+        zs0 = (f32x2){b01[0], b01[1]}; zs1 = (f32x2){b01[2], b01[3]}; zs2 = (f32x2){b23[0], b23[1]}; zs3 = (f32x2){b23[2], b23[3]};
+    }
+#pragma unroll
+    for (int u = 0; u < kOwn; ++u) {
+        const f32x4 dn = u + 1 < kOwn ? __builtin_amdgcn_mfma_f32_16x16x32_bf16(a1, bx[u + 1], cz, 0, 0, 0)
+                                      : __builtin_amdgcn_mfma_f32_16x16x32_bf16(a1n, bx[0], czn, 0, 0, 0);
+        tm[u] = fmaxf(fmaxf(tm[u], d[0]), d[1]);
+        tm[u] = fmaxf(fmaxf(tm[u], d[2]), d[3]);
+        const float q0 = exp2r(d[0]), q1 = exp2r(d[1]), q2 = exp2r(d[2]), q3 = exp2r(d[3]);
+        s[u] += (q0 + q1) + (q2 + q3);
+        if constexpr (FUSED) {
+            const f32x2 s0 = {q0, q0}, s1 = {q1, q1}, s2 = {q2, q2}, s3 = {q3, q3};
+            uxy[u] = __builtin_elementwise_fma(s3, xy3, __builtin_elementwise_fma(s2, xy2, __builtin_elementwise_fma(s1, xy1, __builtin_elementwise_fma(s0, xy0, uxy[u]))));
+            uze[u] = __builtin_elementwise_fma(s3, zs3, __builtin_elementwise_fma(s2, zs2, __builtin_elementwise_fma(s1, zs1, __builtin_elementwise_fma(s0, zs0, uze[u]))));
+        }
+        d = dn;
+    }
 }
 
 template <bool FUSED>
@@ -261,31 +289,6 @@
                 if (wave_cull) gm = zmeta[(c0 + nxt) * 8 + (lane & 7)];
             }
             tiles_done += __popc(tmask);
-            auto tile_step = [&](f32x4& d, const float* __restrict__ tb, const bf16x8 a1, const f32x4 cz, const bf16x8 a1n,
-                                 const f32x4 czn) {
-                f32x2 xy0, xy1, xy2, xy3, zs0, zs1, zs2, zs3;
-                if (FUSED) {
-                    const f32x4 a01 = *reinterpret_cast<const f32x4*>(tb + 272 + 8 * k), a23 = *reinterpret_cast<const f32x4*>(tb + 276 + 8 * k),
-                                b01 = *reinterpret_cast<const f32x4*>(tb + 304 + 8 * k), b23 = *reinterpret_cast<const f32x4*>(tb + 308 + 8 * k);
-                    xy0 = (f32x2){a01[0], a01[1]}; xy1 = (f32x2){a01[2], a01[3]}; xy2 = (f32x2){a23[0], a23[1]}; xy3 = (f32x2){a23[2], a23[3]};
-                    zs0 = (f32x2){b01[0], b01[1]}; zs1 = (f32x2){b01[2], b01[3]}; zs2 = (f32x2){b23[0], b23[1]}; zs3 = (f32x2){b23[2], b23[3]};
-                }
-#pragma unroll
-                for (int u = 0; u < kOwn; ++u) {
-                    const f32x4 dn = u + 1 < kOwn ? __builtin_amdgcn_mfma_f32_16x16x32_bf16(a1, bx[u + 1], cz, 0, 0, 0)
-                                                  : __builtin_amdgcn_mfma_f32_16x16x32_bf16(a1n, bx[0], czn, 0, 0, 0);
-                    tm[u] = fmaxf(fmaxf(tm[u], d[0]), d[1]);
-                    tm[u] = fmaxf(fmaxf(tm[u], d[2]), d[3]);
-                    const float q0 = exp2r(d[0]), q1 = exp2r(d[1]), q2 = exp2r(d[2]), q3 = exp2r(d[3]);
-                    s[u] += (q0 + q1) + (q2 + q3);
-                    if (FUSED) {
-                        const f32x2 s0 = {q0, q0}, s1 = {q1, q1}, s2 = {q2, q2}, s3 = {q3, q3};
-                        uxy[u] = __builtin_elementwise_fma(s3, xy3, __builtin_elementwise_fma(s2, xy2, __builtin_elementwise_fma(s1, xy1, __builtin_elementwise_fma(s0, xy0, uxy[u]))));
-                        uze[u] = __builtin_elementwise_fma(s3, zs3, __builtin_elementwise_fma(s2, zs2, __builtin_elementwise_fma(s1, zs1, __builtin_elementwise_fma(s0, zs0, uze[u]))));
-                    }
-                    d = dn;
-                }
-            };
             if (tmask == 0xFFFFu) {
                 bf16x8 a1 = reinterpret_cast<const bf16x8*>(buf)[lane];
                 f32x4 cz = *reinterpret_cast<const f32x4*>(buf + 256 + 4 * k);
@@ -294,7 +297,7 @@
                     const float* __restrict__ tn = buf + (t + 1 < kChunkTiles ? t + 1 : t) * kTileFloats;
                     const bf16x8 a1n = reinterpret_cast<const bf16x8*>(tn)[lane];
                     const f32x4 czn = *reinterpret_cast<const f32x4*>(tn + 256 + 4 * k);
-                    tile_step(d, buf + t * kTileFloats, a1, cz, a1n, czn);
+                    tile_step<FUSED>(d, buf + t * kTileFloats, a1, cz, a1n, czn, k, bx, s, tm, uxy, uze);
                     a1 = a1n;
                     cz = czn;
                 }
@@ -311,7 +314,7 @@
                     const float* __restrict__ tn = buf + t2 * kTileFloats;
                     const bf16x8 a1n = reinterpret_cast<const bf16x8*>(tn)[lane];
                     const f32x4 czn = *reinterpret_cast<const f32x4*>(tn + 256 + 4 * k);
-                    tile_step(d, buf + t * kTileFloats, a1, cz, a1n, czn);
+                    tile_step<FUSED>(d, buf + t * kTileFloats, a1, cz, a1n, czn, k, bx, s, tm, uxy, uze);
                     if (!more) break;
                     t = t2;
                     a1 = a1n;
@@ -374,6 +377,181 @@
     if (unit >= unit_end) break;
     __syncthreads();
     }
+}
+
+__device__ __forceinline__ void wave_lds_fence() {
+    __builtin_amdgcn_fence(__ATOMIC_RELEASE, "wavefront");
+    __builtin_amdgcn_wave_barrier();
+    __builtin_amdgcn_fence(__ATOMIC_ACQUIRE, "wavefront");
+}
+
+__global__ __launch_bounds__(kBlock) __attribute__((amdgpu_waves_per_eu(3, 3))) void k_fused_wave(
+                                                         const float4* __restrict__ tgt4, const float4* __restrict__ z4,
+                                                         const BoxMeta* __restrict__ tmeta,
+                                                         const BoxMeta* __restrict__ zmeta,
+                                                         const BoxMeta* __restrict__ zchunk,
+                                                         const float* __restrict__ colmin_prev,
+                                                         const float* __restrict__ colmin_g,
+                                                         const unsigned* __restrict__ motion, int parts,
+                                                         int64_t m_total, int64_t n_total,
+                                                         const double* __restrict__ params,
+                                                         float* __restrict__ fpart, int64_t ncap,
+                                                         unsigned* __restrict__ wgcount, unsigned long long* __restrict__ work,
+                                                         int first, int fine,
+                                                         const EngineDecision* __restrict__ guard,
+                                                         float4* __restrict__ corig) {
+    __shared__ __attribute__((aligned(16))) float stage[2 * kChunkTiles * kTileFloats];
+    __shared__ unsigned wave_tiles[kBlock / 64];
+    if (guard) {
+        if (!(guard->col == 1 && guard->fused == 1)) return;
+        fine = guard->fine;
+    }
+    const int lane = threadIdx.x & 63, wv = __builtin_amdgcn_readfirstlane((int)(threadIdx.x >> 6));
+    const float kk = (float)(-kLog2e / (2.0 * params[13]));
+    const float mo = __uint_as_float(*motion);
+    const int nchunks = (int)((m_total + kChunk - 1) / kChunk), nblocks = (int)((n_total + kWgPoints - 1) / kWgPoints);
+    const int blk = (int)blockIdx.x, part = (int)blockIdx.y;
+    const int64_t n0wg = (int64_t)blk * kWgPoints, n0 = n0wg + wv * (16 * kOwn);
+    float lo[3], hi[3];
+    float4 o;
+    float thr = INFINITY, thr_w = INFINITY;
+    WaveBox wb;
+    bool wave_cull = wave_box(tmeta, n0, n_total, lane, wb) && !first && fine;
+    if (n0wg + kWgPoints <= n_total && wg_box(tmeta, n0wg, n_total, lane, lo, hi)) {
+        o = make_float4(0.5f * (lo[0] + hi[0]), 0.5f * (lo[1] + hi[1]), 0.5f * (lo[2] + hi[2]), 0.f);
+        if (!first) {
+            float cm = colmin_g[n0wg / 32 + (lane & 15)];
+            float cw = __shfl(cm, 4 * wv + (lane & 3), 64);
+            cw = fmaxf(cw, __shfl_xor(cw, 1, 64));
+            cw = fmaxf(cw, __shfl_xor(cw, 2, 64));
+#pragma unroll
+            for (int sh = 1; sh < 16; sh <<= 1) cm = fmaxf(cm, __shfl_xor(cm, sh, 64));
+            const float r = sqrtf(cm) + mo, rw = sqrtf(cw) + mo;
+            thr = r * r * 1.00001f + (-prg::kCullExp) / kk;
+            thr_w = rw * rw * 1.00001f + (-prg::kCullExp) / kk;
+        }
+    } else {
+        o = tgt4[n0wg];
+        o.w = 0.f;
+        wave_cull = false;
+#pragma unroll
+        for (int q = 0; q < 3; ++q) { lo[q] = -INFINITY; hi[q] = INFINITY; }
+    }
+    const int k = lane >> 4, j = lane & 15;
+    bf16x8 bx[kOwn];
+    float s[kOwn], tm[kOwn];
+    f32x2 uxy[kOwn], uze[kOwn];
+#pragma unroll
+    for (int t = 0; t < kOwn; ++t) {
+        const float4 x = tgt4[n0 + 16 * t + j];
+        const float xx = x.x - o.x, xy = x.y - o.y, xz = x.z - o.z;
+        const float xsq = fmaf(xz, xz, fmaf(xy, xy, xx * xx));
+        const float offt = first ? 0.f : prg::col_seed_offset(kk, colmin_prev[n0 + 16 * t + j], mo);
+        bx[t] = owned_operand(k, kk, xx, xy, xz, fmaf(kk, xsq, offt));
+        s[t] = 0.f;
+        tm[t] = -INFINITY;
+        uxy[t] = uze[t] = (f32x2){0.f, 0.f};
+    }
+    const int ncp = part < nchunks ? (nchunks - part + parts - 1) / parts : 0;
+    unsigned long long cmask = 0ull;
+    if (ncp > 0) {
+        const BoxMeta cm = zchunk[part + (lane < ncp ? lane : ncp - 1) * parts];
+        if (wave_cull)
+            cmask = __ballot(lane < ncp && !(box_gap2(wb.lo, wb.hi, cm) > thr_w));
+        else
+            cmask = __ballot(lane < ncp && !(box_gap2(lo, hi, cm) > thr));
+    }
+    unsigned long long gmask = 0ull;
+    int mygroup = 0;
+    auto refill = [&]() {
+        while (!gmask && cmask) {
+            int ci = -1;
+#pragma unroll
+            for (int q = 0; q < 8; ++q) {
+                if (cmask) {
+                    const int c = __builtin_ctzll(cmask);
+                    cmask &= cmask - 1;
+                    if ((lane >> 3) == q) ci = c;
+                }
+            }
+            mygroup = (part + (ci < 0 ? 0 : ci) * parts) * 8 + (lane & 7);
+            bool need = ci >= 0;
+            if (wave_cull) {
+                const BoxMeta gm = zmeta[mygroup];
+                need = need && !(box_gap2(wb.lo, wb.hi, gm) > thr_w);
+            }
+            gmask = __ballot(need);
+        }
+    };
+    auto next_group = [&]() -> int {
+        if (!gmask) refill();
+        if (!gmask) return -1;
+        const int b = __builtin_ctzll(gmask);
+        gmask &= gmask - 1;
+        return __builtin_amdgcn_readlane(mygroup, b);
+    };
+    float* const wbuf = stage + wv * (8 * kTileFloats);
+    const int half = lane >> 5, idx = lane & 31;
+    auto load_pair = [&](int ga, int gb) -> float4 {
+        float4 v = z4[(int64_t)(half && gb >= 0 ? gb : ga) * 32 + idx];
+        v.w = 0.f;
+        return v;
+    };
+    unsigned tiles_done = 0;
+    const int g0 = next_group();
+    int g1 = g0 >= 0 ? next_group() : -1;
+    if (g0 >= 0) {
+        float4 ra = load_pair(g0, g1);
+        if (!half || g1 >= 0) stage_point(wbuf, lane, ra, o, kk);
+        wave_lds_fence();
+        for (int bsel = 0;; bsel ^= 1) {
+            const float* __restrict__ buf = wbuf + bsel * (4 * kTileFloats);
+            const int nt = g1 >= 0 ? 4 : 2;
+            const int h0 = next_group(), h1 = h0 >= 0 ? next_group() : -1;
+            if (h0 >= 0) ra = load_pair(h0, h1);
+            tiles_done += (unsigned)nt;
+            bf16x8 a1 = reinterpret_cast<const bf16x8*>(buf)[lane];
+            f32x4 cz = *reinterpret_cast<const f32x4*>(buf + 256 + 4 * k);
+            f32x4 d = __builtin_amdgcn_mfma_f32_16x16x32_bf16(a1, bx[0], cz, 0, 0, 0);
+            for (int t = 0; t < nt; ++t) {
+                const float* __restrict__ tn = buf + (t + 1 < nt ? t + 1 : t) * kTileFloats;
+                const bf16x8 a1n = reinterpret_cast<const bf16x8*>(tn)[lane];
+                const f32x4 czn = *reinterpret_cast<const f32x4*>(tn + 256 + 4 * k);
+                tile_step<true>(d, buf + t * kTileFloats, a1, cz, a1n, czn, k, bx, s, tm, uxy, uze);
+                a1 = a1n;
+                cz = czn;
+            }
+            if (h0 < 0) break;
+            if (!half || h1 >= 0) stage_point(wbuf + (bsel ^ 1) * (4 * kTileFloats), lane, ra, o, kk);
+            wave_lds_fence();
+            g1 = h1;
+        }
+    }
+    if (lane == 0) wave_tiles[wv] = tiles_done;
+    __syncthreads();
+    if (threadIdx.x == 0) {
+        const unsigned tiles = wave_tiles[0] + wave_tiles[1] + wave_tiles[2] + wave_tiles[3];
+        wgcount[(int64_t)part * nblocks + blk] = tiles;
+        if (tiles) atomicAdd(work, (unsigned long long)tiles);
+    }
+    float* __restrict__ fout = fpart + (int64_t)part * 6 * ncap + n0;
+#pragma unroll
+    for (int u2 = 0; u2 < kOwn; ++u2) {
+        const float st = xor_sum(s[u2]), tt = xor_max(tm[u2]);
+        const float bxs = xor_sum(uxy[u2][0]), bys = xor_sum(uxy[u2][1]), bzs = xor_sum(uze[u2][0]), es = xor_sum(uze[u2][1]);
+        if (lane < 16) {
+            const float offt = first ? 0.f : prg::col_seed_offset(kk, colmin_prev[n0 + 16 * u2 + lane], mo);
+            float dmin = fmaxf((tt - offt) / kk, 0.f);
+            dmin = fmaf(dmin, 2.0e-4f, dmin) + 1.0e-12f;
+            fout[16 * u2 + lane] = tt == -INFINITY ? INFINITY : dmin;
+            fout[ncap + 16 * u2 + lane] = st;
+            fout[2 * ncap + 16 * u2 + lane] = bxs;
+            fout[3 * ncap + 16 * u2 + lane] = bys;
+            fout[4 * ncap + 16 * u2 + lane] = bzs;
+            fout[5 * ncap + 16 * u2 + lane] = es;
+        }
+    }
+    if (part == 0 && threadIdx.x == 0) corig[blk] = o;
 }
 
 template <bool LEAN, bool STREAM>
@@ -827,18 +1005,48 @@
     h->dense_pairs_col = 0.0;
 }
 
-void launch_fused_mfma(prg_cpd* h, int S, bool first, bool fine, const EngineDecision* guard) {
-    const int cps = mfma_chunks_per_seg(h->N, h->M, S);
+int fused_wave_parts(int64_t owned_points, int64_t streamed_points) {
+    const int64_t blocks = ceil_div(owned_points, kWgPoints), chunks = ceil_div(streamed_points, kChunk);
+    const int64_t lowest = ceil_div(chunks, (int64_t)64), cap = std::min<int64_t>(kFusedWaveMaxParts, chunks);
+    if (lowest > cap) return 0;
+    const int64_t want = std::max(ceil_div((int64_t)3 * kStreamSlots, blocks), lowest);
+    if (want <= cap) return (int)want;
+    int64_t best = cap;
+    double best_fill = 0.0;
+    for (int64_t s = lowest; s <= cap; ++s) {
+        const double fill = (double)(blocks * s) / (double)(kStreamSlots * ceil_div(blocks * s, (int64_t)kStreamSlots));
+        if (fill >= best_fill) {
+            best_fill = fill;
+            best = s;
+        }
+    }
+    return (int)best;
+}
+
+void launch_fused_mfma(prg_cpd* h, int S, bool first, bool fine, const EngineDecision* guard, int wave_parts) {
     const int64_t nblocks = ceil_div(h->N, kWgPoints);
-    dim3 grid((unsigned)nblocks, (unsigned)ceil_div(ceil_div(h->M, kChunk), cps));
-    h->mfma_col_planes = (int)grid.y;
-    const StreamCut none = {0, 0, 0u, 0u};
-    k_colpass_mfma<true><<<grid, kBlock, 0, h->stream>>>(h->tgt4, h->z4, reinterpret_cast<const BoxMeta*>(h->tmeta),
-                                                         reinterpret_cast<const BoxMeta*>(h->zmeta),
-                                                         reinterpret_cast<const BoxMeta*>(h->zchunk), h->colmin, h->colmin + h->Ncap,
-                                                         h->motion + ((h->estep_count - 1) & 1), cps, h->M, h->N, h->params,
-                                                         h->colpart, h->Ncap, h->wgcount, h->eng_work, first ? 1 : 0, fine ? 1 : 0, guard,
-                                                         none, h->corig);
+    if (wave_parts > 0) {
+        dim3 grid((unsigned)nblocks, (unsigned)wave_parts);
+        h->mfma_col_planes = wave_parts;
+        k_fused_wave<<<grid, kBlock, 0, h->stream>>>(h->tgt4, h->z4, reinterpret_cast<const BoxMeta*>(h->tmeta),
+                                                     reinterpret_cast<const BoxMeta*>(h->zmeta),
+                                                     reinterpret_cast<const BoxMeta*>(h->zchunk), h->colmin, h->colmin + h->Ncap,
+                                                     h->motion + ((h->estep_count - 1) & 1), wave_parts, h->M, h->N, h->params,
+                                                     reinterpret_cast<float*>(h->colpart), h->Ncap, h->wgcount, h->eng_work,
+                                                     first ? 1 : 0, fine ? 1 : 0, guard, h->corig);
+    } else {
+        const int cps = mfma_chunks_per_seg(h->N, h->M, S);
+        dim3 grid((unsigned)nblocks, (unsigned)ceil_div(ceil_div(h->M, kChunk), cps));
+        h->mfma_col_planes = (int)grid.y;
+        const StreamCut none = {0, 0, 0u, 0u};
+        k_colpass_mfma<true><<<grid, kBlock, 0, h->stream>>>(h->tgt4, h->z4, reinterpret_cast<const BoxMeta*>(h->tmeta),
+                                                             reinterpret_cast<const BoxMeta*>(h->zmeta),
+                                                             reinterpret_cast<const BoxMeta*>(h->zchunk), h->colmin, h->colmin + h->Ncap,
+                                                             h->motion + ((h->estep_count - 1) & 1), cps, h->M, h->N, h->params,
+                                                             h->colpart, h->Ncap, h->wgcount, h->eng_work, first ? 1 : 0, fine ? 1 : 0, guard,
+                                                             none, h->corig);
+    }
+    h->fused_wave_launched = wave_parts > 0;
     h->wg_col = nblocks * h->mfma_col_planes;
     h->wg_col_pairs = 128.0 * 16.0;
     h->dense_pairs_col = 0.0;
diff --git a/probreg_amd/engine.py b/probreg_amd/engine.py
--- a/probreg_amd/engine.py
+++ b/probreg_amd/engine.py
@@ -32,6 +32,12 @@
     a, b = ctypes.c_double(0.0), ctypes.c_double(0.0)
     check(lib.prg_cpd_engine_bounds(int(m), int(n_local), ctypes.byref(a), ctypes.byref(b)))
     return float(a.value), float(b.value)
+
+
+def fused_wave_parts(m, n_local):
+    a, b = ctypes.c_int(0), ctypes.c_int(0)
+    check(lib.prg_cpd_fused_wave_parts(int(m), int(n_local), ctypes.byref(a), ctypes.byref(b)))
+    return int(a.value), int(b.value)
 
 
 class CpdPlan(object):
@@ -133,6 +139,14 @@
     def set_fused_factor(self, factor=256.0):
         check(lib.prg_cpd_set_fused_factor(self._h, float(factor)))
 
+    def set_fused_wave(self, mode=1):
+        check(lib.prg_cpd_set_fused_wave(self._h, int(mode)))
+
+    def last_estep_fused_wave(self):
+        v = ctypes.c_int(0)
+        check(lib.prg_cpd_last_estep_fused_wave(self._h, ctypes.byref(v)))
+        return int(v.value)
+
     def last_estep_fused(self):
         v = ctypes.c_int(0)
         check(lib.prg_cpd_last_estep_fused(self._h, ctypes.byref(v)))
```
